# vgl-hub/kreeq

Measured on AMD Instinct MI355X. Metric: distinct+total k-mers/sec at k=21 (count path), higher is better.
Workload: dtype u64

## Files before the change

### include/kreeq_amd.h

```cpp
#ifndef KREEQ_AMD_H
#define KREEQ_AMD_H

#include <stdint.h>

#ifdef __cplusplus
extern "C" {
#endif

#define KQ_ABI_VERSION 4

typedef enum {
    KQ_OK = 0,
    KQ_ERR_INVALID = -1,
    KQ_ERR_NO_DEVICE = -2,
    KQ_ERR_HIP = -3,
    KQ_ERR_NOMEM = -4,
    KQ_ERR_TABLE_FULL = -5,
    KQ_ERR_CAPACITY = -6,
    KQ_ERR_MISMATCH = -7
} kq_status;

typedef struct kq_handle kq_handle;

typedef struct {
    uint64_t key;
    uint32_t fw[4], bw[4], cov;
    uint32_t hc;
} kq_entry;

typedef struct {
    uint32_t fw, bw, cov;
    uint8_t  isFw;
    uint8_t  pad[3];
} kq_dbgbase;

typedef struct {
    uint64_t total;
    uint64_t unique;
    uint64_t distinct;
    uint64_t missing;
    uint64_t edges;
} kq_stats;

typedef struct {
    uint64_t kmers_counted;
    uint64_t slots_used;
    uint64_t slots_total;
    uint64_t hc_used;
    uint64_t hc_total;
    uint64_t table_bytes;
    uint64_t table_passes;
} kq_info;


int  kq_create(kq_handle** out, int device, int k, int map_count, uint64_t capacity_hint);
void kq_destroy(kq_handle* h);
int  kq_clear(kq_handle* h);
int  kq_set_stream(kq_handle* h, void* hip_stream);
void* kq_get_stream(kq_handle* h);
enum { KQ_OPT_TRUST_CAPACITY = 1, KQ_OPT_COUNT_PATH = 2, KQ_OPT_SLICE_KMERS = 3, KQ_OPT_COUNT_MAP_RANGE = 4, KQ_OPT_PROFILE = 5,
       KQ_OPT_LOOKUP_PATH = 6, KQ_OPT_MERGE_PATH = 7, KQ_OPT_NARROW_MID = 8, KQ_OPT_PENDING_BYTES = 9, KQ_OPT_BUCKET_WINDOW = 10, KQ_OPT_OVERLAP = 11, KQ_OPT_COUNT_MAP_PASSES = 12, KQ_OPT_KERNEL_SET = 13,
       KQ_OPT_TEST_FAIL_PLAN = 100  };
int  kq_set_option(kq_handle* h, int option, int64_t value);
int  kq_get_profile(kq_handle* h, char* buf, uint64_t cap);
int  kq_sync(kq_handle* h);
int  kq_flush(kq_handle* h);
int  kq_get_info(kq_handle* h, kq_info* out);
const char* kq_last_error(void);
int  kq_abi_version(void);
int  kq_device_available(void);
int  kq_device_memory(int device, uint64_t* free_bytes, uint64_t* total_bytes);


int  kq_count_batch(kq_handle* h, const char* bases, uint64_t len);
int  kq_count_batch_dev(kq_handle* h, const char* d_bases, uint64_t len);

void* kq_host_alloc(uint64_t bytes);
void  kq_host_free(void* p);
int  kq_count_batch_async(kq_handle* h, const char* bases, uint64_t len, uint64_t* ticket);
int  kq_host_wait(kq_handle* h, uint64_t ticket);

void kq_pack_bases(const char* bases, uint64_t len, uint32_t* codes, uint16_t* inv);
int  kq_count_packed_dev(kq_handle* h, const uint32_t* d_codes, const uint16_t* d_inv, uint64_t n_bases);
int  kq_count_packed_async(kq_handle* h, const uint32_t* codes, const uint16_t* inv, uint64_t n_bases, uint64_t* ticket);

int  kq_pack_bases_dev(kq_handle* h, const char* d_bases, uint64_t len, uint32_t* d_codes, uint16_t* d_inv);

enum { KQ_FASTX_FASTQ = 1, KQ_FASTX_FASTA = 2 };
int  kq_parse_fastx_dev(kq_handle* h, const char* d_text, uint64_t len, int format, char* d_bases, uint64_t cap, uint64_t* n_bases);
int  kq_count_fastx_dev(kq_handle* h, const char* d_text, uint64_t len, int format);
int  kq_count_fastx_async(kq_handle* h, const char* text, uint64_t len, int format, uint64_t* ticket);

int  kq_emit_records(kq_handle* h, const char* bases, uint64_t len,
                     uint64_t* keys, uint8_t* edges, uint64_t cap, uint64_t* n_out);
int  kq_emit_partitioned_dev(kq_handle* h, const char* d_bases, uint64_t len, int n_parts,
                             uint64_t* d_keys, uint8_t* d_edges, uint64_t cap,
                             uint64_t* part_counts);

int  kq_emit_packed_dev(kq_handle* h, const char* d_bases, uint64_t len, int n_parts,
                        uint64_t* d_recs, uint64_t cap, uint64_t* part_counts);
int  kq_insert_packed_dev(kq_handle* h, const uint64_t* d_recs, uint64_t n);

int  kq_emit_sharded_dev(kq_handle* h, const char* d_bases, uint64_t len, int n_parts, uint32_t* d_recs, uint8_t* d_aux, uint64_t cap,
                         uint64_t* d_bucket_counts, uint64_t* part_counts);
int  kq_insert_sharded_dev(kq_handle* h, const uint32_t* d_recs, const uint8_t* d_aux, uint64_t n, int n_peers, const uint64_t* d_bucket_counts);

int  kq_insert_records(kq_handle* h, const uint64_t* keys, const uint8_t* edges, uint64_t n);
int  kq_insert_records_dev(kq_handle* h, const uint64_t* d_keys, const uint8_t* d_edges, uint64_t n);


int  kq_summary(kq_handle* h, kq_stats* out);
int  kq_histogram(kq_handle* h, uint64_t* cov, uint64_t* cnt, uint64_t cap, uint64_t* n_out);


int  kq_lookup_sequence(kq_handle* h, const char* bases, uint64_t len, uint32_t cov_cutoff,
                        uint16_t map_lo, uint16_t map_hi, kq_dbgbase* per_base,
                        uint64_t counters[3]);
int  kq_lookup_sequence_dev(kq_handle* h, const char* d_bases, uint64_t len, uint32_t cov_cutoff,
                            uint16_t map_lo, uint16_t map_hi, kq_dbgbase* d_per_base,
                            uint64_t* d_counters);


int  kq_lookup_keys(kq_handle* h, const uint64_t* keys, uint64_t n, kq_entry* out);

int  kq_branch_scan(kq_handle* h, const char* bases, uint64_t len, uint32_t cov_cutoff, uint8_t* flags);


int  kq_merge(kq_handle* dst, kq_handle* src);

int  kq_import(kq_handle* h, const kq_entry* entries, uint64_t n);
int  kq_export(kq_handle* h, uint16_t map_lo, uint16_t map_hi, kq_entry* out, uint64_t cap,
               uint64_t* n_out);

#ifdef __cplusplus
}
#endif
#endif
```

### kreeq_amd/build.py

```python
import os
import shutil
import subprocess

PKG = os.path.dirname(os.path.abspath(__file__))
ROOT = os.path.dirname(PKG)
LIB = os.path.join(PKG, "lib", "libkreeq_amd.so")
CLI = os.path.join(PKG, "bin", "kreeq")
HOSTLIB = os.path.join(PKG, "lib", "libkreeq_host.so")

HIP_SOURCES = [os.path.join(PKG, "csrc", "kreeq_amd.hip")]
HIP_DEPS = HIP_SOURCES + [os.path.join(PKG, "csrc", f) for f in ("kq_device.h", "kq_partition.h", "kq_kernels.h", "kq_fastx.h")] + [os.path.join(ROOT, "include", "kreeq_amd.h")]
HOST_DIR = os.path.join(PKG, "host")


def _stale(target, deps):
    if not os.path.exists(target):
        return True
    t = os.path.getmtime(target)
    return any(os.path.getmtime(d) > t for d in deps if os.path.exists(d))


def hipcc():
    for c in (shutil.which("hipcc"), "/opt/rocm/bin/hipcc"):
        if c and os.path.exists(c):
            return c
    raise RuntimeError("hipcc not found: the HIP library cannot be built (there is no CPU fallback)")


def build_lib(force=False, verbose=False, out=None, defines=()):
    target = out or LIB
    if force or _stale(target, HIP_DEPS):
        os.makedirs(os.path.dirname(target), exist_ok=True)
        cmd = [hipcc(), "-O3", "-std=c++17", "--offload-arch=gfx950", "-fPIC", "-shared", "-Wall", "-Wextra",
               "-o", target] + ["-D" + d for d in defines] + HIP_SOURCES
        if verbose:
            print(" ".join(cmd))
        subprocess.check_call(cmd)
    return target


def host_sources():
    if not os.path.isdir(HOST_DIR):
        return []
    return sorted(os.path.join(HOST_DIR, f) for f in os.listdir(HOST_DIR) if f.endswith(".cpp") and f != "hostlib.cpp")


def build_hostlib(force=False, verbose=False):
    srcs = [os.path.join(HOST_DIR, f) for f in ("hostlib.cpp", "kreeq_db.cpp")]
    deps = srcs + [os.path.join(HOST_DIR, "kreeq_db.h"), os.path.join(ROOT, "include", "kreeq_amd.h")]
    if force or _stale(HOSTLIB, deps):
        os.makedirs(os.path.dirname(HOSTLIB), exist_ok=True)
        cmd = ["g++", "-O2", "-std=c++17", "-Wall", "-Wextra", "-fPIC", "-shared", "-pthread", "-I", os.path.join(ROOT, "include"), "-o", HOSTLIB] + srcs
        if verbose:
            print(" ".join(cmd))
        subprocess.check_call(cmd)
    return HOSTLIB


def build_cli(force=False, verbose=False):
    srcs = host_sources()
    if not srcs:
        return None
    deps = srcs + [os.path.join(HOST_DIR, f) for f in os.listdir(HOST_DIR) if f.endswith(".h")] + [LIB]
    if force or _stale(CLI, deps):
        os.makedirs(os.path.dirname(CLI), exist_ok=True)
        cmd = ["g++", "-O2", "-std=c++17", "-Wall", "-Wextra", "-pthread", "-I", os.path.join(ROOT, "include"), "-o", CLI] + srcs + \
              ["-L", os.path.dirname(LIB), "-lkreeq_amd", "-lz", "-Wl,-rpath,$ORIGIN/../lib"]
        if verbose:
            print(" ".join(cmd))
        subprocess.check_call(cmd)
    return CLI


def build_all(force=False, verbose=False):
    build_lib(force, verbose)
    build_cli(force, verbose)
    build_hostlib(force, verbose)
```

### kreeq_amd/capi.py

```python
import ctypes as C
import os

import numpy as np

from . import build as _build

ENTRY_DTYPE = np.dtype([("key", "<u8"), ("fw", "<u4", 4), ("bw", "<u4", 4), ("cov", "<u4"), ("hc", "<u4")])
DBGBASE_DTYPE = np.dtype([("fw", "<u4"), ("bw", "<u4"), ("cov", "<u4"), ("isFw", "u1"), ("pad", "u1", 3)])

SYMBOLS = ["kq_create", "kq_destroy", "kq_clear", "kq_set_option", "kq_get_profile", "kq_set_stream", "kq_get_stream", "kq_sync", "kq_flush", "kq_get_info", "kq_last_error",
           "kq_abi_version", "kq_device_available", "kq_device_memory", "kq_count_batch", "kq_count_batch_dev", "kq_host_alloc", "kq_host_free", "kq_count_batch_async", "kq_host_wait", "kq_pack_bases", "kq_count_packed_dev", "kq_count_packed_async",
           "kq_pack_bases_dev", "kq_parse_fastx_dev", "kq_count_fastx_dev", "kq_count_fastx_async", "kq_emit_records",
           "kq_emit_partitioned_dev", "kq_emit_packed_dev", "kq_insert_packed_dev", "kq_emit_sharded_dev", "kq_insert_sharded_dev", "kq_insert_records", "kq_insert_records_dev", "kq_summary", "kq_histogram",
           "kq_lookup_sequence", "kq_lookup_sequence_dev", "kq_lookup_keys", "kq_branch_scan", "kq_merge", "kq_import", "kq_export"]

FASTX_FASTQ, FASTX_FASTA = 1, 2


class KqError(RuntimeError):
    def __init__(self, code, msg):
        super().__init__(f"kreeq_amd error {code}: {msg}")
        self.code = code


class Stats(C.Structure):
    _fields_ = [("total", C.c_uint64), ("unique", C.c_uint64), ("distinct", C.c_uint64), ("missing", C.c_uint64),
                ("edges", C.c_uint64)]


class Info(C.Structure):
    _fields_ = [("kmers_counted", C.c_uint64), ("slots_used", C.c_uint64), ("slots_total", C.c_uint64), ("hc_used", C.c_uint64),
                ("hc_total", C.c_uint64), ("table_bytes", C.c_uint64), ("table_passes", C.c_uint64)]


_lib = None


def lib_path():
    return _build.LIB


def _preload_process_hip_runtime():
    import importlib.util

    try:
        spec = importlib.util.find_spec("torch")
    except (ImportError, ValueError):
        spec = None
    if not spec or not spec.origin:
        return
    d = os.path.join(os.path.dirname(spec.origin), "lib")
    for name in ("libhsa-runtime64.so", "libamdhip64.so"):
        p = os.path.join(d, name)
        if os.path.exists(p):
            try:
                C.CDLL(p, mode=C.RTLD_GLOBAL)
            except OSError:
                return


def load():
    global _lib
    if _lib is not None:
        return _lib
    path = os.environ.get("KQ_LIB") or _build.LIB
    if not os.path.exists(path):
        raise KqError(-2, f"{path} is missing: build it with `python -c 'import __graft_entry__ as g; g.build()'` "
                          "(the product has no CPU fallback)")
    _preload_process_hip_runtime()
    L = C.CDLL(path)
    vp, u64, u32, u16, ci = C.c_void_p, C.c_uint64, C.c_uint32, C.c_uint16, C.c_int
    L.kq_create.argtypes = [C.POINTER(vp), ci, ci, ci, u64]
    L.kq_destroy.argtypes = [vp]
    L.kq_destroy.restype = None
    L.kq_clear.argtypes = [vp]
    L.kq_set_stream.argtypes = [vp, vp]
    L.kq_set_option.argtypes = [vp, ci, C.c_int64]
    L.kq_get_profile.argtypes = [vp, C.c_char_p, u64]
    L.kq_get_stream.argtypes = [vp]
    L.kq_get_stream.restype = vp
    L.kq_sync.argtypes = [vp]
    L.kq_flush.argtypes = [vp]
    L.kq_get_info.argtypes = [vp, C.POINTER(Info)]
    L.kq_last_error.restype = C.c_char_p
    L.kq_device_memory.argtypes = [ci, C.POINTER(u64), C.POINTER(u64)]
    L.kq_count_batch.argtypes = [vp, vp, u64]
    L.kq_count_batch_dev.argtypes = [vp, vp, u64]
    L.kq_host_alloc.argtypes = [u64]
    L.kq_host_alloc.restype = vp
    L.kq_host_free.argtypes = [vp]
    L.kq_host_free.restype = None
    L.kq_count_batch_async.argtypes = [vp, vp, u64, C.POINTER(u64)]
    L.kq_host_wait.argtypes = [vp, u64]
    L.kq_pack_bases.argtypes = [vp, u64, vp, vp]
    L.kq_pack_bases.restype = None
    L.kq_count_packed_dev.argtypes = [vp, vp, vp, u64]
    L.kq_count_packed_async.argtypes = [vp, vp, vp, u64, C.POINTER(u64)]
    L.kq_pack_bases_dev.argtypes = [vp, vp, u64, vp, vp]
    L.kq_parse_fastx_dev.argtypes = [vp, vp, u64, ci, vp, u64, C.POINTER(u64)]
    L.kq_count_fastx_dev.argtypes = [vp, vp, u64, ci]
    L.kq_count_fastx_async.argtypes = [vp, vp, u64, ci, C.POINTER(u64)]
    L.kq_emit_records.argtypes = [vp, vp, u64, vp, vp, u64, C.POINTER(u64)]
    L.kq_emit_partitioned_dev.argtypes = [vp, vp, u64, ci, vp, vp, u64, vp]
    L.kq_emit_packed_dev.argtypes = [vp, vp, u64, ci, vp, u64, vp]
    L.kq_insert_packed_dev.argtypes = [vp, vp, u64]
    L.kq_emit_sharded_dev.argtypes = [vp, vp, u64, ci, vp, vp, u64, vp, vp]
    L.kq_insert_sharded_dev.argtypes = [vp, vp, vp, u64, ci, vp]
    L.kq_insert_records.argtypes = [vp, vp, vp, u64]
    L.kq_insert_records_dev.argtypes = [vp, vp, vp, u64]
    L.kq_summary.argtypes = [vp, C.POINTER(Stats)]
    L.kq_histogram.argtypes = [vp, vp, vp, u64, C.POINTER(u64)]
    L.kq_lookup_sequence.argtypes = [vp, vp, u64, u32, u16, u16, vp, vp]
    L.kq_lookup_sequence_dev.argtypes = [vp, vp, u64, u32, u16, u16, vp, vp]
    L.kq_lookup_keys.argtypes = [vp, vp, u64, vp]
    L.kq_branch_scan.argtypes = [vp, vp, u64, u32, vp]
    L.kq_merge.argtypes = [vp, vp]
    L.kq_import.argtypes = [vp, vp, u64]
    L.kq_export.argtypes = [vp, u16, u16, vp, u64, C.POINTER(u64)]
    _lib = L
    return L


def _check(rc):
    if rc != 0:
        raise KqError(rc, load().kq_last_error().decode(errors="replace"))


def _p(a):
    return a.ctypes.data_as(C.c_void_p) if a is not None else None


def pack_bases(bases: bytes):
    buf = np.frombuffer(bases, dtype=np.uint8)
    units = (len(buf) + 15) // 16
    codes, inv = np.zeros(max(units, 1), dtype=np.uint32), np.zeros(max(units, 1), dtype=np.uint16)
    load().kq_pack_bases(_p(buf) if len(buf) else None, len(buf), _p(codes), _p(inv))
    return codes[:units], inv[:units]


def device_available():
    return bool(load().kq_device_available())


def device_memory(device=0):
    f, t = C.c_uint64(0), C.c_uint64(0)
    _check(load().kq_device_memory(device, C.byref(f), C.byref(t)))
    return f.value, t.value


class KreeqDB:

    def __init__(self, k=21, map_count=128, device=0, capacity_hint=0):
        self.k, self.map_count, self.device = k, map_count, device
        self._h = C.c_void_p()
        _check(load().kq_create(C.byref(self._h), device, k, map_count, capacity_hint))

    def close(self, _load=load):
        if getattr(self, "_h", None):
            _load().kq_destroy(self._h)
            self._h = None

    __del__ = close

    @property
    def handle(self):
        return self._h

    def set_stream(self, hip_stream_ptr):
        _check(load().kq_set_stream(self._h, C.c_void_p(hip_stream_ptr)))

    def sync(self):
        _check(load().kq_sync(self._h))

    def flush(self):
        _check(load().kq_flush(self._h))

    def set_option(self, option, value):
        opt = {"trust_capacity": 1, "count_path": 2, "slice_kmers": 3, "count_map_range": 4, "profile": 5, "lookup_path": 6, "merge_path": 7, "narrow_mid": 8, "pending_bytes": 9, "bucket_window": 10, "overlap": 11, "count_map_passes": 12, "kernel_set": 13, "test_fail_plan": 100}[option]
        if option == "count_map_range":
            value = int(value[0]) | (int(value[1]) << 16)
        if option in ("count_path", "lookup_path", "merge_path"):
            value = {"auto": 0, "direct": 1, "partitioned": 2}[value]
        _check(load().kq_set_option(self._h, opt, int(value)))

    def clear(self):
        _check(load().kq_clear(self._h))

    def profile(self):
        buf = C.create_string_buffer(1024)
        _check(load().kq_get_profile(self._h, buf, 1024))
        return {k: float(v) for k, v in (kv.split("=") for kv in buf.value.decode().split(";") if kv)}

    def info(self):
        i = Info()
        _check(load().kq_get_info(self._h, C.byref(i)))
        return {f: getattr(i, f) for f, _ in Info._fields_}

    def count_batch(self, bases: bytes):
        buf = np.frombuffer(bases, dtype=np.uint8)
        _check(load().kq_count_batch(self._h, _p(buf), len(buf)))

    def count_batch_async(self, host_ptr, n):
        t = C.c_uint64(0)
        _check(load().kq_count_batch_async(self._h, C.c_void_p(host_ptr), n, C.byref(t)))
        return t.value

    def count_packed_dev(self, codes_ptr, inv_ptr, n_bases):
        _check(load().kq_count_packed_dev(self._h, C.c_void_p(codes_ptr), C.c_void_p(inv_ptr), n_bases))

    def count_packed_async(self, codes_ptr, inv_ptr, n_bases):
        t = C.c_uint64(0)
        _check(load().kq_count_packed_async(self._h, C.c_void_p(codes_ptr), C.c_void_p(inv_ptr), n_bases, C.byref(t)))
        return t.value

    def pack_bases_dev(self, bases_ptr, n, codes_ptr, inv_ptr):
        _check(load().kq_pack_bases_dev(self._h, C.c_void_p(bases_ptr), n, C.c_void_p(codes_ptr), C.c_void_p(inv_ptr)))

    def parse_fastx_dev(self, text_ptr, n, fmt, out_ptr, cap):
        nb = C.c_uint64(0)
        rc = load().kq_parse_fastx_dev(self._h, C.c_void_p(text_ptr), n, fmt, C.c_void_p(out_ptr) if out_ptr else None, cap, C.byref(nb))
        if rc != 0:
            e = KqError(rc, load().kq_last_error().decode(errors="replace"))
            e.needed = nb.value
            raise e
        return nb.value

    def count_fastx_dev(self, text_ptr, n, fmt):
        _check(load().kq_count_fastx_dev(self._h, C.c_void_p(text_ptr), n, fmt))

    def count_fastx_async(self, host_ptr, n, fmt):
        t = C.c_uint64(0)
        _check(load().kq_count_fastx_async(self._h, C.c_void_p(host_ptr), n, fmt, C.byref(t)))
        return t.value

    def host_wait(self, ticket):
        _check(load().kq_host_wait(self._h, ticket))

    def count_batch_dev(self, ptr, n):
        _check(load().kq_count_batch_dev(self._h, C.c_void_p(ptr), n))

    def emit_records(self, bases: bytes):
        buf = np.frombuffer(bases, dtype=np.uint8)
        n = C.c_uint64(0)
        _check(load().kq_emit_records(self._h, _p(buf), len(buf), None, None, 0, C.byref(n)))
        keys = np.empty(n.value, dtype=np.uint64)
        edges = np.empty(n.value, dtype=np.uint8)
        if n.value:
            _check(load().kq_emit_records(self._h, _p(buf), len(buf), _p(keys), _p(edges), n.value, C.byref(n)))
        return keys, edges

    def emit_partitioned_dev(self, bases_ptr, n, n_parts, keys_ptr, edges_ptr, cap):
        counts = np.zeros(n_parts, dtype=np.uint64)
        _check(load().kq_emit_partitioned_dev(self._h, C.c_void_p(bases_ptr), n, n_parts, C.c_void_p(keys_ptr), C.c_void_p(edges_ptr),
                                              cap, _p(counts)))
        return counts

    def emit_packed_dev(self, bases_ptr, n, n_parts, recs_ptr, cap):
        counts = np.zeros(n_parts, dtype=np.uint64)
        _check(load().kq_emit_packed_dev(self._h, C.c_void_p(bases_ptr), n, n_parts, C.c_void_p(recs_ptr), cap, _p(counts)))
        return counts

    def insert_packed_dev(self, recs_ptr, n):
        _check(load().kq_insert_packed_dev(self._h, C.c_void_p(recs_ptr), n))

    def emit_sharded_dev(self, bases_ptr, n, n_parts, recs_ptr, aux_ptr, cap, bucket_counts_ptr, sync=True):
        counts = np.zeros(n_parts, dtype=np.uint64) if sync else None
        _check(load().kq_emit_sharded_dev(self._h, C.c_void_p(bases_ptr), n, n_parts, C.c_void_p(recs_ptr), C.c_void_p(aux_ptr), cap,
                                          C.c_void_p(bucket_counts_ptr), _p(counts)))
        return counts

    def insert_sharded_dev(self, recs_ptr, aux_ptr, n, n_peers, bucket_counts_ptr):
        _check(load().kq_insert_sharded_dev(self._h, C.c_void_p(recs_ptr), C.c_void_p(aux_ptr), n, n_peers, C.c_void_p(bucket_counts_ptr)))

    def insert_records(self, keys, edges):
        keys = np.ascontiguousarray(keys, dtype=np.uint64)
        edges = np.ascontiguousarray(edges, dtype=np.uint8)
        assert len(keys) == len(edges)
        _check(load().kq_insert_records(self._h, _p(keys), _p(edges), len(keys)))

    def insert_records_dev(self, keys_ptr, edges_ptr, n):
        _check(load().kq_insert_records_dev(self._h, C.c_void_p(keys_ptr), C.c_void_p(edges_ptr), n))

    def summary(self, with_hist=False):
        st = Stats()
        _check(load().kq_summary(self._h, C.byref(st)))
        d = {f: getattr(st, f) for f, _ in Stats._fields_}
        if with_hist:
            n = C.c_uint64(0)
            _check(load().kq_histogram(self._h, None, None, 0, C.byref(n)))
            cov = np.zeros(n.value, dtype=np.uint64)
            cnt = np.zeros(n.value, dtype=np.uint64)
            _check(load().kq_histogram(self._h, _p(cov), _p(cnt), n.value, C.byref(n)))
            d["hist"] = dict(zip(cov.tolist(), cnt.tolist()))
        return d

    def lookup_sequence(self, bases: bytes, cov_cutoff=0, map_lo=0, map_hi=None, per_base=False, per_base_buf=None):
        if map_hi is None:
            map_hi = self.map_count
        buf = np.frombuffer(bases, dtype=np.uint8)
        ctr = np.zeros(3, dtype=np.uint64)
        pb = per_base_buf if per_base_buf is not None else (np.zeros(len(buf), dtype=DBGBASE_DTYPE) if per_base else None)
        _check(load().kq_lookup_sequence(self._h, _p(buf), len(buf), cov_cutoff, map_lo, map_hi, _p(pb), _p(ctr)))
        return ctr, pb

    def lookup_sequence_dev(self, bases_ptr, n, counters_ptr, cov_cutoff=0, map_lo=0, map_hi=None, per_base_ptr=None):
        if map_hi is None:
            map_hi = self.map_count
        _check(load().kq_lookup_sequence_dev(self._h, C.c_void_p(bases_ptr), n, cov_cutoff, map_lo, map_hi,
                                             C.c_void_p(per_base_ptr) if per_base_ptr else None, C.c_void_p(counters_ptr)))

    def lookup_keys(self, keys):
        keys = np.ascontiguousarray(keys, dtype=np.uint64)
        out = np.zeros(len(keys), dtype=ENTRY_DTYPE)
        _check(load().kq_lookup_keys(self._h, _p(keys), len(keys), _p(out)))
        return out

    def branch_scan(self, bases: bytes, cov_cutoff=0):
        buf = np.frombuffer(bases, dtype=np.uint8)
        flags = np.zeros(len(buf), dtype=np.uint8)
        _check(load().kq_branch_scan(self._h, _p(buf), len(buf), cov_cutoff, _p(flags)))
        return flags

    def merge(self, other):
        _check(load().kq_merge(self._h, other._h))

    def import_entries(self, entries):
        entries = np.ascontiguousarray(entries, dtype=ENTRY_DTYPE)
        _check(load().kq_import(self._h, _p(entries), len(entries)))

    def export(self, map_lo=0, map_hi=None):
        if map_hi is None:
# ... 8 lines not shown
```

### kreeq_amd/csrc/kq_kernels.h

```cpp
#pragma once

#include <hip/hip_runtime.h>

#include <type_traits>

#include "../../include/kreeq_amd.h"
#include "kq_device.h"
#include "kq_partition.h"

using namespace kq;


__global__ __launch_bounds__(TILE_THREADS) void k_count_direct(TableView t, const uint8_t* __restrict__ ab,
                                                                uint64_t lead, uint64_t len, int k, EmitRange er, PartCfg filt,
                                                                const uint16_t* __restrict__ pinv ) {
    uint32_t n_new = 0;
    uint64_t n_kmers = 0;
    scan_tiles(ab, lead, len, k, [&](uint64_t pos, uint64_t fw, uint64_t rv, uint32_t prev, uint32_t next) {
        if (pos < er.lo || pos >= er.hi) return;
        const bool is_fw = fw < rv;
        const uint64_t key = is_fw ? fw : rv;
        if (filt.filt_lo != 0 || filt.filt_hi != filt.map_count) {
            const uint32_t m = map_index(key, filt.map_count, filt.map_mask);
            if (m < filt.filt_lo || m >= filt.filt_hi) return;
// ... 240 lines not shown
        for (int it = 0; it < 16; ++it) { const uint32_t b = TOP8 ? wb[TOP8 ? it : 0] : narrow_word_bin(w[it]); pl[it] = b != NB ? atomicAdd(&s_hist[b], 1u) : ~0u; }
#pragma unroll
        for (int it = 0; it < 16; ++it) if (pl[it] != ~0u) { s_buf[pl[it]] = w[it]; if (TOP8) s_bin[pl[it]] = (uint16_t)wb[TOP8 ? it : 0]; }
        __syncthreads();
        const uint32_t total = s_loff[NB];
        uint64_t cv[16];
        uint32_t cg[16];
#pragma unroll
        for (int it = 0; it < 16; ++it) cv[it] = s_buf[tid + it * THREADS];
#pragma unroll
        for (int it = 0; it < 16; ++it) cg[it] = s_grel[(uint32_t)(tid + it * THREADS) < total ? (TOP8 ? (uint32_t)s_bin[TOP8 ? tid + it * THREADS : 0] : narrow_word_bin(cv[it])) : 0u] + (tid + it * THREADS);
        if (bin_owner) s_hist[tid] = 0;
        landed(nxt.x); landed(nxt.y); landed(nxt.z); landed(nxt.w);
#pragma unroll
        for (int it = 0; it < 16; ++it) {
            if ((uint32_t)(tid + it * THREADS) < total) {
                if (TOP8) reinterpret_cast<uint64_t*>(recs)[cg[it]] = cv[it];
                else { recs[cg[it]] = (uint32_t)cv[it]; recs_aux[cg[it]] = (uint8_t)(cv[it] >> 48); }
            }
        }
    }
}

__global__ __launch_bounds__(1024) void k_lv_units(const unsigned long long* __restrict__ seg_off, const unsigned long long* __restrict__ seg_hi, LevelCfg lv,
                                                   unsigned long long* __restrict__ unit_base) {
    __shared__ unsigned long long s_part[1024];
    const uint32_t tid = threadIdx.x, per = (lv.n_seg + 1023) / 1024;
    const uint32_t lo = min(tid * per, lv.n_seg), hi = min(lo + per, lv.n_seg);
    unsigned long long sum = 0;
    for (uint32_t b = lo; b < hi; ++b) sum += (seg_hi[b] - seg_off[b] + P2_UNIT - 1) / P2_UNIT;
    s_part[tid] = sum;
    __syncthreads();
    if (tid < 64) {
        unsigned long long loc[16], tot = 0;
#pragma unroll
        for (int j = 0; j < 16; ++j) { loc[j] = s_part[tid * 16 + j]; tot += loc[j]; }
        unsigned long long incl = tot;
#pragma unroll
        for (int o = 1; o < 64; o <<= 1) { unsigned long long nn = __shfl_up(incl, o, 64); if ((int)tid >= o) incl += nn; }
        unsigned long long run = incl - tot;
#pragma unroll
        for (int j = 0; j < 16; ++j) { s_part[tid * 16 + j] = run; run += loc[j]; }
        if (tid == 63) unit_base[lv.n_seg] = incl;
    }
    __syncthreads();
    unsigned long long run = s_part[tid];
    for (uint32_t b = lo; b < hi; ++b) { unit_base[b] = run; run += (seg_hi[b] - seg_off[b] + P2_UNIT - 1) / P2_UNIT; }
}
__device__ __forceinline__ uint32_t seg_of_unit(const unsigned long long* unit_base, uint32_t n_seg, uint64_t u) {
    uint32_t lo = 0, hi = n_seg;
    while (hi - lo > 1) { uint32_t mid = (lo + hi) >> 1; if (unit_base[mid] <= u) lo = mid; else hi = mid; }
    return lo;
}
template <int FMT>
__global__ __launch_bounds__(MS_THREADS) void k_lv_hist(const uint64_t* __restrict__ recs, const uint8_t* __restrict__ , LevelCfg lv,
                                                        const unsigned long long* __restrict__ seg_off, const unsigned long long* __restrict__ seg_hi,
                                                        const unsigned long long* __restrict__ unit_base, uint32_t* __restrict__ m2) {
    __shared__ uint32_t s_hist[NB_MAX];
    const uint64_t n_units = unit_base[lv.n_seg];
    for (uint64_t u = blockIdx.x; u < n_units; u += gridDim.x) {
        const uint32_t b_in = seg_of_unit(unit_base, lv.n_seg, u);
        const uint32_t b = lv.spb > 1 ? b_in / lv.spb : b_in;
        const uint64_t lo = seg_off[b_in] + (u - unit_base[b_in]) * P2_UNIT;
        const uint64_t hi = lo + P2_UNIT < seg_hi[b_in] ? lo + P2_UNIT : seg_hi[b_in];
        for (uint32_t i = threadIdx.x; i < lv.nb; i += MS_THREADS) s_hist[i] = 0;
        __syncthreads();
        const uint64_t last = hi - 1;
        if (FMT == FMT_NARROW) {
            const uint4* v4 = reinterpret_cast<const uint4*>(recs);
            const uint64_t q0 = lo >> 2, q1 = (hi + 3) >> 2;
            for (uint64_t qb = q0; qb < q1; qb += 4ull * MS_THREADS) {
                uint4 q[4];
#pragma unroll
                for (int j = 0; j < 4; ++j) q[j] = v4[min(qb + (uint64_t)j * MS_THREADS + threadIdx.x, q1 - 1)];
#pragma unroll
                for (int j = 0; j < 4; ++j) {
                    const uint64_t qi = qb + (uint64_t)j * MS_THREADS + threadIdx.x;
                    const uint32_t e[4] = {q[j].x, q[j].y, q[j].z, q[j].w};
#pragma unroll
                    for (int c = 0; c < 4; ++c) {
                        const uint64_t ri = 4 * qi + c;
                        if (qi < q1 && ri >= lo && ri < hi) atomicAdd(&s_hist[narrow_bin(lv, b, e[c])], 1u);
                    }
                }
            }
        } else
        for (uint64_t base = lo; base < hi; base += 8ull * MS_THREADS) {
            uint64_t r[8];
#pragma unroll
            for (int j = 0; j < 8; ++j) {
                const uint64_t i = min(base + (uint64_t)j * MS_THREADS + threadIdx.x, last);
                r[j] = FMT == FMT_NARROW ? (uint64_t)reinterpret_cast<const uint32_t*>(recs)[i] : recs[i];
            }
#pragma unroll
            for (int j = 0; j < 8; ++j)
                if (base + (uint64_t)j * MS_THREADS + threadIdx.x < hi) {
                    const uint32_t bin = FMT == FMT_NARROW ? narrow_bin(lv, b, (uint32_t)r[j])
                        : FMT == FMT_TOP8 ? narrow_bin(lv, b, (uint32_t)(r[j] >> 32))
                        : (FMT == FMT_PACK8 && lv.top8) ? (uint32_t)(rec_hash<false>(r[j]) >> (64 - NARROW_CBITS))
                        : level_bin(lv, b, hash_region(lv.in_raw ? table_hash(r[j], lv.k) : rec_hash<FMT == FMT_WIDE>(r[j]), lv.n_regions));
                    atomicAdd(&s_hist[bin], 1u);
                }
        }
        __syncthreads();
        for (uint32_t i = threadIdx.x; i < lv.nb; i += MS_THREADS) m2[u * lv.nb + i] = s_hist[i];
        __syncthreads();
    }
}
__global__ __launch_bounds__(256) void k_lv_offsets(uint32_t* __restrict__ m2, LevelCfg lv, const unsigned long long* __restrict__ unit_base,
                                                    unsigned long long* __restrict__ group_count) {
    const uint64_t r = ((uint64_t)blockIdx.x * blockDim.x + threadIdx.x) >> 6;
    const uint32_t lane = threadIdx.x & 63;
    const uint32_t n_lseg = lv.n_seg / lv.spb;
    if (r >= (uint64_t)n_lseg * lv.nb) return;
    const uint32_t b = (uint32_t)(r / lv.nb), bin = (uint32_t)(r % lv.nb);
    const uint64_t u0 = unit_base[b * lv.spb], u1 = unit_base[(b + 1) * lv.spb];
    unsigned long long run = 0;
    for (uint64_t base = u0; base < u1; base += 64) {
        const uint64_t u = base + lane;
        const uint32_t c = u < u1 ? m2[u * lv.nb + bin] : 0u;
        unsigned long long incl = c;
#pragma unroll
        for (int o = 1; o < 64; o <<= 1) { const unsigned long long n = __shfl_up(incl, o, 64); if ((int)lane >= o) incl += n; }
        if (u < u1) m2[u * lv.nb + bin] = (uint32_t)(run + incl - c);
        run += __shfl(incl, 63, 64);
    }
    if (lane == 0) group_count[r] = run;
}
__global__ __launch_bounds__(256) void k_lv_offsets_thread(uint32_t* __restrict__ m2, LevelCfg lv, const unsigned long long* __restrict__ unit_base,
                                                           unsigned long long* __restrict__ group_count) {
    const uint64_t r = (uint64_t)blockIdx.x * blockDim.x + threadIdx.x;
    const uint32_t n_lseg = lv.n_seg / lv.spb;
    if (r >= (uint64_t)n_lseg * lv.nb) return;
    const uint32_t b = (uint32_t)(r / lv.nb), bin = (uint32_t)(r % lv.nb);
    const uint64_t u0 = unit_base[b * lv.spb], u1 = unit_base[(b + 1) * lv.spb];
    unsigned long long run = 0;
    for (uint64_t u = u0; u < u1; ++u) {
        const uint32_t c = m2[u * lv.nb + bin];
        m2[u * lv.nb + bin] = (uint32_t)run;
        run += c;
    }
    group_count[r] = run;
}
#ifndef KQ_LV_THREADS
#define KQ_LV_THREADS 512
#define KQ_LV_ITEMS 8
#define KQ_LV_OCC 4
#endif
constexpr int LV_THREADS = KQ_LV_THREADS, LV_ITEMS = KQ_LV_ITEMS, LV_TILE = LV_THREADS * LV_ITEMS;
template <int FMT, int NBC>
__global__ __launch_bounds__(LV_THREADS, KQ_LV_OCC) void k_lv_scatter(const uint64_t* __restrict__ recs, const uint8_t* __restrict__ recs_aux, LevelCfg lv,
                                                           const unsigned long long* __restrict__ seg_off, const unsigned long long* __restrict__ seg_hi,
                                                           const unsigned long long* __restrict__ unit_base, const uint32_t* __restrict__ m2,
                                                           const unsigned long long* __restrict__ group_base, uint64_t* __restrict__ out,
                                                           uint8_t* __restrict__ out_aux) {
    constexpr bool WIDE = FMT == FMT_WIDE, TIGHT = FMT == FMT_NARROW_TO_TIGHT, NARROW = FMT == FMT_NARROW || TIGHT, CONVERT = FMT == FMT_PACK8_TO_NARROW,
                   TOP8 = FMT == FMT_TOP8, HAS_AUX = WIDE || NARROW;
    constexpr int MS_FMT = (CONVERT || TIGHT) ? FMT_NARROW : TOP8 ? FMT_PACK8 : FMT;
    const uint32_t* recs32 = reinterpret_cast<const uint32_t*>(recs);
    __shared__ MsShared<NBC, MS_FMT, LV_TILE> s;
    __shared__ uint32_t s_rst[TIGHT ? NBC : 1];
    const uint32_t nb = lv.nb;
    const uint64_t n_units = unit_base[lv.n_seg];
    for (uint64_t u = blockIdx.x; u < n_units; u += gridDim.x) {
        const uint32_t b_in = seg_of_unit(unit_base, lv.n_seg, u);
        const uint32_t b = lv.spb > 1 ? b_in / lv.spb : b_in;
        const uint64_t lo = seg_off[b_in] + (u - unit_base[b_in]) * P2_UNIT;
        const uint64_t hi = lo + P2_UNIT < seg_hi[b_in] ? lo + P2_UNIT : seg_hi[b_in];
        for (uint32_t i = threadIdx.x; i < nb; i += LV_THREADS)
            s.gbase[i] = (uint32_t)(group_base[(uint64_t)b * nb + i] + m2[u * nb + i]);
        if (TIGHT) {
            const uint32_t first = (b >> lv.nr_shift) * lv.nr_rps + (b & ((1u << lv.nr_shift) - 1u)) * lv.nr_sub;
            for (uint32_t i = threadIdx.x; i < nb; i += LV_THREADS) s_rst[i] = lv.rstart[first + i];
        }
        __syncthreads();
        uint64_t nxt[LV_ITEMS];
        uint32_t nxt_aux[LV_ITEMS];
        const uint64_t last = hi - 1;
#pragma unroll
        for (int j = 0; j < LV_ITEMS; ++j) {
            const uint64_t i = min(lo + (uint64_t)j * LV_THREADS + threadIdx.x, last);
            nxt[j] = NARROW ? (uint64_t)recs32[i] : recs[i];
            nxt_aux[j] = HAS_AUX ? recs_aux[i] : 0;
        }
#pragma unroll
        for (int j = 0; j < LV_ITEMS; ++j) { landed(nxt[j]); if (HAS_AUX) landed(nxt_aux[j]); }
        for (uint64_t pos = lo; pos < hi; pos += LV_TILE) {
            uint64_t rec[LV_ITEMS];
            uint32_t aux[LV_ITEMS], bin[LV_ITEMS];
#pragma unroll
            for (int j = 0; j < LV_ITEMS; ++j) {
                const uint64_t i = pos + (uint64_t)j * LV_THREADS + threadIdx.x;
                rec[j] = (WIDE && lv.in_raw) ? table_hash(nxt[j], lv.k) : nxt[j];
                aux[j] = nxt_aux[j];
                if (TIGHT) {
                    const uint32_t bn = i >= hi ? nb : narrow_bin(lv, b, (uint32_t)rec[j]);
                    rec[j] = narrow_word(tight_rec(b >> lv.nr_shift, (uint32_t)rec[j], aux[j], s_rst[bn < nb ? bn : 0u]), 0u, bn);
                }
                else if (NARROW) rec[j] = narrow_word((uint32_t)rec[j], aux[j], i >= hi ? nb : narrow_bin(lv, b, (uint32_t)rec[j]));
                else if (CONVERT) {
                    const uint64_t hh = rec_hash<false>(rec[j]);
                    rec[j] = narrow_word(narrow_main(hh), narrow_aux(hh, (uint32_t)(rec[j] >> REC_EDGE_SHIFT) & 63u), i >= hi ? nb : (uint32_t)(hh >> (64 - NARROW_CBITS)));
                }
                else if (TOP8) bin[j] = i >= hi ? nb : narrow_bin(lv, b, (uint32_t)(rec[j] >> 32));
                else bin[j] = i >= hi ? nb : level_bin(lv, b, hash_region(rec_hash<WIDE>(rec[j]), lv.n_regions));
            }
#pragma unroll
            for (int j = 0; j < LV_ITEMS; ++j) {
                const uint64_t i = min(pos + LV_TILE + (uint64_t)j * LV_THREADS + threadIdx.x, last);
                nxt[j] = NARROW ? (uint64_t)recs32[i] : recs[i];
                nxt_aux[j] = HAS_AUX ? recs_aux[i] : 0;
            }
            block_multisplit<MS_FMT, LV_THREADS, LV_ITEMS>(s, rec, aux, bin, nb, out, out_aux, [&] {
#pragma unroll
                for (int j = 0; j < LV_ITEMS; ++j) { landed(nxt[j]); if (HAS_AUX) landed(nxt_aux[j]); }
            }, NBC <= 512 ? lv.rep_shift : 0u);
        }
    }
}
#ifndef KQ_LVS_OCC
#define KQ_LVS_OCC 4
#define KQ_LVS_OCC_TIGHT 4
#endif
template <bool TIGHT>
__global__ __launch_bounds__(LV_THREADS, TIGHT ? KQ_LVS_OCC_TIGHT : KQ_LVS_OCC) void k_lv_scatter_s(const uint32_t* __restrict__ recs32, const uint8_t* __restrict__ recs_aux, LevelCfg lv,
                                                           const unsigned long long* __restrict__ seg_off, const unsigned long long* __restrict__ seg_hi,
                                                           const unsigned long long* __restrict__ unit_base, const uint32_t* __restrict__ m2,
                                                           const unsigned long long* __restrict__ group_base, uint32_t* __restrict__ out,
                                                           uint8_t* __restrict__ out_aux) {
    constexpr int NC = 512;
    static_assert(LV_THREADS == NC && LV_ITEMS == 8, "one counter per thread");
    __shared__ uint64_t s_buf[LV_TILE];
    __shared__ uint32_t s_hist[2][NC], s_loff[NC + 1], s_grel[NC], s_wave[LV_THREADS / 64];
    __shared__ uint32_t s_rst[TIGHT ? NC : 1];
    const int tid = threadIdx.x;
    const uint32_t nb = lv.nb, rs = lv.rep_shift, n_ctr = (nb + 1) << rs;
    const uint32_t sub = (uint32_t)tid & ((1u << rs) - 1u), my_bin = (uint32_t)tid >> rs;
    const bool own_bin = sub == 0 && my_bin < nb;
    const uint64_t n_units = unit_base[lv.n_seg];
    for (uint64_t u = blockIdx.x; u < n_units; u += gridDim.x) {
        const uint32_t b_in = seg_of_unit(unit_base, lv.n_seg, u);
        const uint32_t b = lv.spb > 1 ? b_in / lv.spb : b_in;
        const uint64_t lo = seg_off[b_in] + (u - unit_base[b_in]) * P2_UNIT;
        const uint64_t hi = lo + P2_UNIT < seg_hi[b_in] ? lo + P2_UNIT : seg_hi[b_in];
        uint32_t gabs = own_bin ? (uint32_t)(group_base[(uint64_t)b * nb + my_bin] + m2[u * nb + my_bin]) : 0u;
        if (TIGHT) {
            const uint32_t first = (b >> lv.nr_shift) * lv.nr_rps + (b & ((1u << lv.nr_shift) - 1u)) * lv.nr_sub;
            if ((uint32_t)tid < nb) s_rst[tid] = lv.rstart[first + tid];
        }
        s_hist[0][tid] = 0;
        __syncthreads();
        uint32_t nxt[LV_ITEMS], nxt_aux[LV_ITEMS];
        const uint64_t last = hi - 1;
#pragma unroll
        for (int j = 0; j < LV_ITEMS; ++j) {
            const uint64_t i = min(lo + (uint64_t)j * LV_THREADS + tid, last);
            nxt[j] = recs32[i];
            nxt_aux[j] = recs_aux[i];
        }
#pragma unroll
        for (int j = 0; j < LV_ITEMS; ++j) { landed(nxt[j]); landed(nxt_aux[j]); }
        uint32_t par = 0;
        for (uint64_t pos = lo; pos < hi; pos += LV_TILE, par ^= 1u) {
            uint32_t* hist = s_hist[par];
            uint64_t w[LV_ITEMS];
#pragma unroll
            for (int j = 0; j < LV_ITEMS; ++j) {
                const uint64_t i = pos + (uint64_t)j * LV_THREADS + tid;
                const uint32_t bn = i >= hi ? nb : narrow_bin(lv, b, nxt[j]);
                w[j] = TIGHT ? narrow_word(tight_rec(b >> lv.nr_shift, nxt[j], nxt_aux[j], s_rst[bn < nb ? bn : 0u]), 0u, bn) : narrow_word(nxt[j], nxt_aux[j], bn);
                if (bn != nb) atomicAdd(&hist[(bn << rs) | sub], 1u);
            }
#pragma unroll
            for (int j = 0; j < LV_ITEMS; ++j) {
                const uint64_t i = min(pos + LV_TILE + (uint64_t)j * LV_THREADS + tid, last);
                nxt[j] = recs32[i];
                nxt_aux[j] = recs_aux[i];
            }
            __syncthreads();
            const uint32_t cnt = (uint32_t)tid < n_ctr ? hist[tid] : 0u;
            uint32_t incl = cnt;
#pragma unroll
            for (int o = 1; o < 64; o <<= 1) { const uint32_t n = __shfl_up(incl, o, 64); if ((tid & 63) >= o) incl += n; }
            if ((tid & 63) == 63) s_wave[tid >> 6] = incl;
            s_hist[par ^ 1u][tid] = 0;
            __syncthreads();
            uint32_t excl = incl - cnt;
            for (int v = 0; v < (tid >> 6); ++v) excl += s_wave[v];
            s_loff[tid] = excl;
            hist[tid] = excl;
            if (own_bin) s_grel[my_bin] = gabs - excl;
            __syncthreads();
            if (own_bin) gabs += s_loff[(my_bin + 1) << rs] - excl;
#pragma unroll
            for (int j = 0; j < LV_ITEMS; ++j) {
                const uint32_t bn = narrow_word_bin(w[j]);
                if (bn != nb) s_buf[atomicAdd(&hist[(bn << rs) | sub], 1u)] = w[j];
            }
            __syncthreads();
            const uint32_t total = s_loff[nb << rs];
            uint64_t cv[LV_ITEMS];
            uint32_t cg[LV_ITEMS];
#pragma unroll
            for (int it = 0; it < LV_ITEMS; ++it) cv[it] = s_buf[tid + it * LV_THREADS];
#pragma unroll
            for (int it = 0; it < LV_ITEMS; ++it) cg[it] = s_grel[(uint32_t)(tid + it * LV_THREADS) < total ? narrow_word_bin(cv[it]) : 0u] + (tid + it * LV_THREADS);
#pragma unroll
            for (int j = 0; j < LV_ITEMS; ++j) { landed(nxt[j]); landed(nxt_aux[j]); }
#pragma unroll
            for (int it = 0; it < LV_ITEMS; ++it) {
                if ((uint32_t)(tid + it * LV_THREADS) < total) {
                    out[cg[it]] = (uint32_t)cv[it];
                    if (!TIGHT) out_aux[cg[it]] = (uint8_t)(cv[it] >> 48);
                }
            }
        }
    }
}
__global__ void k_set2(unsigned long long* p, unsigned long long a, unsigned long long b) { p[0] = a; p[1] = b; }

constexpr uint32_t SCAN_CHUNK = 16384;
__global__ __launch_bounds__(1024) void k_scan_sums(const unsigned long long* __restrict__ a, uint64_t n, unsigned long long* __restrict__ sums) {
    const uint64_t lo = (uint64_t)blockIdx.x * SCAN_CHUNK, hi = lo + SCAN_CHUNK < n ? lo + SCAN_CHUNK : n;
    unsigned long long v = 0;
    for (uint64_t i = lo + threadIdx.x; i < hi; i += 1024) v += a[i];
    uint64_t t = block_sum(v);
    if (threadIdx.x == 0) sums[blockIdx.x] = t;
}
__global__ __launch_bounds__(1024) void k_scan_apply(unsigned long long* __restrict__ a, uint64_t n, const unsigned long long* __restrict__ sums) {
    __shared__ unsigned long long s_part[1024];
    const uint64_t lo = (uint64_t)blockIdx.x * SCAN_CHUNK + (uint64_t)threadIdx.x * (SCAN_CHUNK / 1024);
    unsigned long long v[SCAN_CHUNK / 1024], sum = 0;
#pragma unroll
    for (uint32_t j = 0; j < SCAN_CHUNK / 1024; ++j) { v[j] = lo + j < n ? a[lo + j] : 0; sum += v[j]; }
    s_part[threadIdx.x] = sum;
    __syncthreads();
    if (threadIdx.x < 64) {
        unsigned long long loc[16], tot = 0;
#pragma unroll
        for (int j = 0; j < 16; ++j) { loc[j] = s_part[threadIdx.x * 16 + j]; tot += loc[j]; }
        unsigned long long incl = tot;
#pragma unroll
        for (int o = 1; o < 64; o <<= 1) { unsigned long long nn = __shfl_up(incl, o, 64); if ((int)threadIdx.x >= o) incl += nn; }
        unsigned long long run = incl - tot;
#pragma unroll
        for (int j = 0; j < 16; ++j) { s_part[threadIdx.x * 16 + j] = run; run += loc[j]; }
    }
    __syncthreads();
    unsigned long long run = sums[blockIdx.x] + s_part[threadIdx.x];
#pragma unroll
    for (uint32_t j = 0; j < SCAN_CHUNK / 1024; ++j) { if (lo + j < n) a[lo + j] = run; run += v[j]; }
}


template <class T> __device__ __forceinline__ T ld_global(const T* p) { return *(const __attribute__((address_space(1))) T*)p; }

template <uint32_t GRP>
struct SetTickets {
    uint64_t lo; uint32_t cnt, first, n_grp;
    __device__ __forceinline__ void build(const P3Set* __restrict__ sets, uint32_t n_sets, uint64_t r, uint32_t lane) {
        lo = 0; cnt = 0;
        if (lane < n_sets) { const unsigned long long* b = ld_global(&sets[lane].base); lo = ld_global(b + r); cnt = (uint32_t)(ld_global(b + r + 1) - lo); }
        const uint32_t mine = (cnt + GRP - 1) / GRP;
        uint32_t incl = mine;
#pragma unroll
        for (int o = 1; o < P3_MAX_SETS; o <<= 1) { const uint32_t v = __shfl_up(incl, o, 64); if ((int)lane >= o) incl += v; }
        first = incl - mine;
        n_grp = __builtin_amdgcn_readlane(incl, 63);
    }
    __device__ __forceinline__ void locate(uint32_t g, uint32_t& q, uint32_t& off, uint32_t& q_cnt, uint64_t& q_lo) const {
        const uint64_t nonempty = __ballot(cnt != 0);
        const uint64_t m = __ballot(cnt != 0 && first <= g);
        q = (g < n_grp && m) ? 63u - (uint32_t)__clzll((unsigned long long)m) : (uint32_t)__ffsll((unsigned long long)nonempty) - 1u;
        const uint32_t f = __builtin_amdgcn_readlane(first, q);
        q_cnt = __builtin_amdgcn_readlane(cnt, q);
        q_lo = ((uint64_t)__builtin_amdgcn_readlane((uint32_t)(lo >> 32), q) << 32) | __builtin_amdgcn_readlane((uint32_t)lo, q);
        off = (g < n_grp ? g - f : 0u) * GRP;
    }
};

template <int THREADS, bool HOT, uint32_t GRP>
__device__ __forceinline__ bool region_gate(SetTickets<GRP>& tk, const TableView& t, const P3Set* __restrict__ sets, uint32_t n_sets, uint64_t r,
                                            int table_is_empty, unsigned long long* __restrict__ hot_list ) {
    const int tid = threadIdx.x;
    tk.build(sets, n_sets, r, (uint32_t)tid & 63u);
    uint64_t n_recs = tk.cnt;
#pragma unroll
    for (int o = 32; o > 0; o >>= 1) n_recs += __shfl_xor(n_recs, o, 64);
    if (n_recs == 0) {
        if (!HOT && table_is_empty == 2) {
            ulonglong2* g2 = reinterpret_cast<ulonglong2*>(t.slots + (r << REGION_SHIFT));
            for (int i = tid; i < (int)REGION_SLOTS; i += THREADS) g2[i] = make_ulonglong2(0ull, 0ull);
        }
        return false;
    }
    if (!HOT && n_recs > 32ull * REGION_SLOTS) {
        if (tid == 0) hot_list[1 + atomicAdd(&hot_list[0], 1ull)] = r;
        return false;
    }
    return true;
}
constexpr int HC_LDS = 64;
__device__ __forceinline__ void hc_lds_reset(uint64_t (&hckey)[HC_LDS], uint32_t (&hccnt)[HC_LDS][8]) {
    const int tid = threadIdx.x;
    if (tid < HC_LDS) {
        hckey[tid] = EMPTY_KEY;
#pragma unroll
        for (int e = 0; e < 8; ++e) hccnt[tid][e] = 0;
    }
}
__device__ __forceinline__ void hc_lds_add(const TableView& t, uint64_t (&hckey)[HC_LDS], uint32_t (&hccnt)[HC_LDS][8], uint64_t h, const uint32_t (&e)[8]) {
    const uint64_t key = key_of_hash(h, t.k);
    int hslot = -1;
    uint32_t hp = (uint32_t)(h >> 40) & (HC_LDS - 1);
    for (int probe = 0; probe < HC_LDS; ++probe, hp = (hp + 1) & (HC_LDS - 1)) {
        uint64_t cur = __hip_atomic_load(&hckey[hp], __ATOMIC_RELAXED, __HIP_MEMORY_SCOPE_WORKGROUP);
        if (cur == EMPTY_KEY) cur = atomicCAS((unsigned long long*)&hckey[hp], (unsigned long long)EMPTY_KEY, (unsigned long long)key);
        if (cur == EMPTY_KEY || cur == key) { hslot = (int)hp; break; }
    }
    if (hslot >= 0) {
#pragma unroll
        for (int w = 0; w < 8; ++w) if (e[w]) atomicAdd(&hccnt[hslot][w], e[w]);
    } else {
        hc_add(t, h, 0, 0, e);
    }
}
__device__ __forceinline__ void hc_lds_flush(const TableView& t, uint64_t (&hckey)[HC_LDS], uint32_t (&hccnt)[HC_LDS][8]) {
    const int tid = threadIdx.x;
    if (tid < HC_LDS && hckey[tid] != EMPTY_KEY) {
        HcSlot* hs = hc_upsert(t, hckey[tid]);
        if (!hs) atomicOr(&t.st->err_hc_full, 1u);
        else {
#pragma unroll
            for (int e = 0; e < 8; ++e) if (hccnt[tid][e]) atomicAdd((unsigned long long*)&hs->cnt[e], (unsigned long long)hccnt[tid][e]);
        }
    }
}
template <class C>
__device__ __forceinline__ void region_totals_wave(uint32_t n_new, uint32_t n_ok, C& s_new, C& s_kmers) {
#pragma unroll
    for (int o = 32; o > 0; o >>= 1) { n_new += __shfl_down(n_new, o, 64); n_ok += __shfl_down(n_ok, o, 64); }
    if ((threadIdx.x & 63) == 0) { if (n_new) atomicAdd(&s_new, (C)n_new); if (n_ok) atomicAdd(&s_kmers, (C)n_ok); }
}
template <class C>
__device__ __forceinline__ void region_totals_store(const TableView& t, const C& s_new, const C& s_kmers) {
    if (threadIdx.x == 0) {
        if (s_new) atomicAdd(&t.st->slots_used, (unsigned long long)s_new);
        if (s_kmers) atomicAdd(&t.st->kmers_added, (unsigned long long)s_kmers);
    }
}

#ifndef KQ_P3_THREADS
#define KQ_P3_THREADS 512
#define KQ_P3_OCC 6
#define KQ_P3_PF 2
#endif
constexpr int P3_THREADS = KQ_P3_THREADS;
template <int FMT, bool HOT>
__global__ __launch_bounds__(P3_THREADS, HOT ? 4 : KQ_P3_OCC) void k_count_regions(TableView t, const P3Set* __restrict__ sets, uint32_t n_sets,
                                                              int aux_fmt, int table_is_empty,
                                                              unsigned long long* __restrict__ hot_list ,
                                                              uint32_t narrow_rps ) {
    constexpr bool WIDE = FMT == FMT_WIDE, NARROW = FMT == FMT_NARROW, TOP8 = FMT == FMT_TOP8, HAS_AUX = WIDE || NARROW;
    constexpr int PF = KQ_P3_PF;
    constexpr uint64_t GRP = 64ull * PF;
    __shared__ uint64_t s_img[REGION_SLOTS * 3];
    __shared__ uint64_t s_lut[64];
    if (threadIdx.x < 64) s_lut[threadIdx.x] = idx6_to_pack(threadIdx.x);
    __shared__ unsigned long long s_new, s_kmers;
    __shared__ unsigned int s_grp;
    __shared__ uint64_t s_hckey[HC_LDS];
    __shared__ uint32_t s_hccnt[HC_LDS][8];
// ... 837 lines not shown
```

### kreeq_amd/csrc/kq_partition.h

```cpp
#pragma once
#include "kq_device.h"

namespace kq {

constexpr int MS_THREADS = 256;
constexpr int MS_ITEMS = 16;
constexpr int MS_TILE = MS_THREADS * MS_ITEMS;
constexpr int NB_MAX = 2048;
constexpr int SEG_MAX = 65536;
constexpr uint32_t SUB_BITS_MAX = 8;
constexpr int REC_EDGE_SHIFT = 56;
constexpr int PART_MAX_K = 28;
constexpr int AUX_IDX6 = 0, AUX_EDGE_BYTE = 1, AUX_TIGHT = 2;

struct PartCfg {
    uint64_t n_regions;
    uint32_t g_shift;
    uint32_t n_coarse;
    uint32_t mode;
    uint32_t map_count;
    uint32_t map_mask;
    uint32_t filt_lo, filt_hi;
    uint32_t raw_out;
    uint32_t narrow;
    uint32_t owner_sub;
    uint32_t sub_bits;
    uint32_t win_lo, win_hi;
    uint32_t n_rng;
};

constexpr int P3_MAX_SETS = 64;
struct P3Set { const uint64_t* recs; const uint8_t* aux; const unsigned long long* base; uint64_t n_max; };

struct LevelCfg {
    uint64_t n_regions;
    uint32_t n_seg, nb, seg_shift, out_shift;
    uint32_t in_raw;
    uint32_t k;
    uint32_t narrow;
    uint32_t top8;
    uint32_t nr_shift, nr_rps, nr_sub, nr_div, nr_inv;
    uint32_t nr_mid, nr_fshift, nr_fmask, nr_f24;
    uint32_t spb;
    uint32_t rep_shift;
    const uint32_t* rstart = nullptr;
};
__device__ __forceinline__ uint32_t level_bin(const LevelCfg& lv, uint32_t b, uint64_t region) {
    return (uint32_t)(region >> lv.out_shift) - (lv.seg_shift >= 32 ? 0u : (b << (lv.seg_shift - lv.out_shift)));
}

__device__ __forceinline__ uint32_t edge_idx6(bool is_fw, uint32_t prev, uint32_t next) {
    uint32_t f, b;
    if (is_fw) { f = next < 4 ? next : 7u; b = prev < 4 ? prev : 7u; }
    else       { f = prev < 4 ? 3u - prev : 7u; b = next < 4 ? 3u - next : 7u; }
    return f | (b << 3);
}
__device__ __forceinline__ uint32_t edge_idx6_any(bool is_fw, uint32_t prev, uint32_t next) {
    const uint32_t f = is_fw ? next : prev, b = is_fw ? prev : next, m = is_fw ? 0u : 0x1Bu;
    return (f | (b << 3)) ^ m;
}
__device__ __forceinline__ uint64_t rec_pack(uint64_t key, bool is_fw, uint32_t prev, uint32_t next) {
    return key | ((uint64_t)edge_idx6(is_fw, prev, next) << REC_EDGE_SHIFT);
}
__device__ __forceinline__ uint64_t idx6_to_pack(uint32_t v) {
    const uint32_t f = v & 7u, b = (v >> 3) & 7u;
    return (f < 4 ? 1ull << (8 * f) : 0ull) | (b < 4 ? 1ull << (8 * (4 + b)) : 0ull);
}
__device__ __forceinline__ uint32_t idx6_to_edge_byte(uint32_t v) {
    const uint32_t f = v & 7u, b = (v >> 3) & 7u;
    return (f < 4 ? 1u << (7 - f) : 0u) | (b < 4 ? 1u << (7 - (4 + b)) : 0u);
}
__device__ __forceinline__ uint64_t rec_key(uint64_t rec) { return rec & ((1ull << REC_EDGE_SHIFT) - 1); }
__device__ __forceinline__ uint64_t rec_edge_pack(uint64_t rec) {
    const uint32_t f = (uint32_t)(rec >> REC_EDGE_SHIFT) & 7u, b = (uint32_t)(rec >> (REC_EDGE_SHIFT + 3)) & 7u;
    return (f < 4 ? 1ull << (8 * f) : 0ull) | (b < 4 ? 1ull << (8 * (4 + b)) : 0ull);
}
template <bool WIDE>
__device__ __forceinline__ uint64_t rec_hash(uint64_t rec) { return WIDE ? rec : rec << 8; }
__device__ __forceinline__ uint64_t rec_pack_hash(uint64_t h, bool is_fw, uint32_t prev, uint32_t next) {
    return (h >> 8) | ((uint64_t)edge_idx6(is_fw, prev, next) << REC_EDGE_SHIFT);
}

constexpr int FMT_PACK8 = 0, FMT_WIDE = 1, FMT_NARROW = 2;
constexpr int FMT_PACK8_TO_NARROW = 3;
constexpr uint32_t NARROW_CBITS = 8, NARROW_MAX_K = 21;
constexpr int FMT_TOP8 = 4;
constexpr int FMT_TIGHT = 5;
constexpr int FMT_NARROW_TO_TIGHT = 6;
constexpr uint64_t TIGHT_MIN_REGIONS = 1ull << 16;
__device__ __forceinline__ uint32_t tight_rec(uint32_t bucket, uint32_t main32, uint32_t aux, uint32_t rstart_r) {
    const uint32_t d = ((bucket << (32 - NARROW_CBITS)) | (main32 >> NARROW_CBITS)) - rstart_r;
    return (d << 16) | ((main32 & 0xFFu) << 8) | ((aux & 3u) << 6) | (aux >> 2);
}
__device__ __forceinline__ uint64_t tight_hash(uint32_t t, uint32_t rstart_r) { return ((uint64_t)((t >> 16) + rstart_r) << 32) | ((uint64_t)((t >> 6) & 1023u) << 22); }
__device__ __forceinline__ uint64_t top8_rec(uint64_t h, uint32_t idx6) { return ((h << NARROW_CBITS) & ~63ull) | idx6; }
__device__ __forceinline__ uint64_t top8_hash(uint32_t bucket, uint64_t rec) { return ((uint64_t)bucket << (64 - NARROW_CBITS)) | ((rec & ~63ull) >> NARROW_CBITS); }
__device__ __forceinline__ uint32_t narrow_main(uint64_t h) { return (uint32_t)(h >> (32 - NARROW_CBITS)); }
__device__ __forceinline__ uint32_t narrow_aux(uint64_t h, uint32_t idx6) { return ((uint32_t)(h >> (30 - NARROW_CBITS)) & 3u) | (idx6 << 2); }
__device__ __forceinline__ uint64_t narrow_hash(uint32_t bucket, uint32_t main32, uint32_t aux) {
    return ((uint64_t)bucket << (64 - NARROW_CBITS)) | ((uint64_t)main32 << (32 - NARROW_CBITS)) | ((uint64_t)(aux & 3u) << (30 - NARROW_CBITS));
}
__device__ __forceinline__ uint64_t narrow_word(uint32_t main32, uint32_t aux, uint32_t bin) { return (uint64_t)main32 | ((uint64_t)(bin | (aux << 16)) << 32); }
__device__ __forceinline__ uint32_t narrow_word_bin(uint64_t w) { return (uint32_t)(w >> 32) & 0xFFFFu; }
__device__ __forceinline__ uint32_t narrow_region(uint32_t bucket, uint32_t main32, uint64_t n_regions) {
    return __umulhi((bucket << (32 - NARROW_CBITS)) | (main32 >> NARROW_CBITS), (uint32_t)n_regions);
}
__device__ __forceinline__ uint32_t narrow_bin(const LevelCfg& lv, uint32_t , uint32_t main32) {
    const uint32_t f = main32 >> NARROW_CBITS;
    if (lv.nr_mid) return f >> lv.nr_fshift;
    const uint32_t fs = f & lv.nr_fmask;
    return lv.nr_f24 ? umul24u(fs, lv.nr_sub) >> lv.nr_fshift : (uint32_t)(((uint64_t)fs * lv.nr_sub) >> lv.nr_fshift);
}

template <int NBC, int FMT, int TILE = MS_TILE>
struct MsShared {
    static constexpr int tile = TILE;
    uint64_t stage[TILE];
    uint16_t sbin[FMT != FMT_NARROW ? TILE : 4];
    uint8_t  saux[FMT == FMT_WIDE ? TILE : 8];
    uint32_t hist[NBC];
    uint32_t loff[NBC];
    uint32_t gbase[NBC];
    uint32_t wave_sum[16];
};

template <int THREADS, class S>
__device__ __forceinline__ void ms_scan(S& s, uint32_t nb) {
    constexpr int NBC = (int)(sizeof(s.hist) / sizeof(uint32_t));
    constexpr int MS_BINS_PER_THREAD = (NBC + THREADS - 1) / THREADS;
    const int tid = threadIdx.x;
    uint32_t v[MS_BINS_PER_THREAD], sum = 0;
#pragma unroll
    for (int j = 0; j < MS_BINS_PER_THREAD; ++j) { uint32_t b = MS_BINS_PER_THREAD * tid + j; v[j] = (b < nb) ? s.hist[b] : 0; sum += v[j]; }
    uint32_t incl = sum;
#pragma unroll
    for (int o = 1; o < 64; o <<= 1) { uint32_t n = __shfl_up(incl, o, 64); if ((tid & 63) >= o) incl += n; }
    if ((tid & 63) == 63) s.wave_sum[tid >> 6] = incl;
    __syncthreads();
    uint32_t base = 0;
    for (int w = 0; w < (tid >> 6); ++w) base += s.wave_sum[w];
    uint32_t run = base + incl - sum;
#pragma unroll
    for (int j = 0; j < MS_BINS_PER_THREAD; ++j) { uint32_t b = MS_BINS_PER_THREAD * tid + j; if (b < nb) s.loff[b] = run; run += v[j]; }
    __syncthreads();
}

__device__ __forceinline__ void landed(uint32_t& v) { asm volatile("" : "+v"(v)); }
__device__ __forceinline__ void landed(uint64_t& v) { asm volatile("" : "+v"(v)); }
struct NoHook { __device__ __forceinline__ void operator()() const {} };
template <int FMT, int THREADS = MS_THREADS, int ITEMS = MS_ITEMS, class S, class F = NoHook>
__device__ __forceinline__ void block_multisplit(S& s, const uint64_t (&rec)[ITEMS], const uint32_t (&aux)[ITEMS],
                                                 const uint32_t (&bin)[ITEMS], uint32_t nb,
                                                 uint64_t* __restrict__ out, uint8_t* __restrict__ out_aux, F pre_store = F(), uint32_t rs = 0) {
    const int tid = threadIdx.x;
    const uint32_t sub = (uint32_t)tid & ((1u << rs) - 1u), n_ctr = (nb + 1) << rs;
    for (uint32_t b = tid; b < n_ctr; b += THREADS) s.hist[b] = 0;
    __syncthreads();
    static_assert(THREADS * ITEMS <= S::tile, "round size");
    uint32_t rank[ITEMS];
#pragma unroll
    for (int i = 0; i < ITEMS; ++i) {
        const uint32_t b = FMT == FMT_NARROW ? narrow_word_bin(rec[i]) : bin[i];
        rank[i] = 0;
        if (b != nb) rank[i] = atomicAdd(&s.hist[(b << rs) | sub], 1u);
    }
    __syncthreads();
    ms_scan<THREADS>(s, n_ctr);
    for (uint32_t b = tid; b < nb; b += THREADS) s.gbase[b] -= s.loff[b << rs];
#pragma unroll
    for (int i = 0; i < ITEMS; ++i) {
        const uint32_t b = FMT == FMT_NARROW ? narrow_word_bin(rec[i]) : bin[i];
        if (b == nb) continue;
        const uint32_t p = s.loff[(b << rs) | sub] + rank[i];
        if (FMT == FMT_NARROW) {
            s.stage[p] = rec[i];
        } else {
            s.stage[p] = rec[i];
            s.sbin[p] = (uint16_t)bin[i];
            if (FMT == FMT_WIDE) s.saux[p] = (uint8_t)aux[i];
        }
    }
    __syncthreads();
    const uint32_t total = s.loff[nb << rs];
    uint32_t cb[ITEMS];
    uint32_t cg[ITEMS];
    uint64_t cv[ITEMS];
// ... 46 lines not shown
```

### kreeq_amd/csrc/kreeq_amd.hip

```cpp
#include <hip/hip_runtime.h>
#include <hipcub/hipcub.hpp>

#include <algorithm>
#include <cstdarg>
#include <cstdio>
#include <cstdlib>
#include <cstring>
#include <mutex>
#include <new>
#include <numeric>
#include <string>
#include <thread>
#include <type_traits>
#include <vector>

#include "../../include/kreeq_amd.h"
#include "kq_device.h"
#include "kq_partition.h"

using namespace kq;

#include "kq_kernels.h"
#include "kq_fastx.h"


static thread_local std::string g_err;
static int fail(int code, const char* fmt, ...) {
    char buf[512];
    va_list ap; va_start(ap, fmt); vsnprintf(buf, sizeof buf, fmt, ap); va_end(ap);
    g_err = buf;
    return code;
}
#define HIPC(expr)                                                                                   \
    do {                                                                                             \
        hipError_t e_ = (expr);                                                                      \
        if (e_ != hipSuccess)                                                                        \
            return fail(e_ == hipErrorOutOfMemory ? KQ_ERR_NOMEM : KQ_ERR_HIP, "%s: %s (%s:%d)", #expr, \
                        hipGetErrorString(e_), __FILE__, __LINE__);                                  \
    } while (0)

struct Scrambled {
    void* p = nullptr; size_t bytes = 0, chunk = 0;
    std::vector<hipMemGenericAllocationHandle_t> hs;
    bool vmm = false;
};
static void scr_free(Scrambled& b) {
    if (!b.p) return;
    (void)hipDeviceSynchronize();
    if (b.vmm) {
        (void)hipMemUnmap(b.p, b.hs.size() * b.chunk);
        for (auto& hnd : b.hs) (void)hipMemRelease(hnd);
        (void)hipMemAddressFree(b.p, b.hs.size() * b.chunk);
    } else (void)hipFree(b.p);
    b = Scrambled();
}
static bool scr_try_vmm(Scrambled& b, size_t bytes, int device) {
    static const size_t chunk_mb = getenv("KQ_SCRAMBLE_MB") ? (size_t)atoi(getenv("KQ_SCRAMBLE_MB")) : 2;
    if (!chunk_mb) return false;
    hipMemAllocationProp prop = {};
    prop.type = hipMemAllocationTypePinned; prop.location.type = hipMemLocationTypeDevice; prop.location.id = device;
    size_t gran = 0;
    if (hipMemGetAllocationGranularity(&gran, &prop, hipMemAllocationGranularityMinimum) != hipSuccess || !gran) { (void)hipGetLastError(); return false; }
    const size_t chunk = ((chunk_mb << 20) + gran - 1) / gran * gran, n = (bytes + chunk - 1) / chunk;
    void* base = nullptr;
    if (hipMemAddressReserve(&base, n * chunk, 0, nullptr, 0) != hipSuccess) { (void)hipGetLastError(); return false; }
    std::vector<hipMemGenericAllocationHandle_t> hs;
    hs.reserve(n);
    bool ok = true;
    for (size_t i = 0; i < n && ok; ++i) { hipMemGenericAllocationHandle_t hnd; ok = hipMemCreate(&hnd, chunk, &prop, 0) == hipSuccess; if (ok) hs.push_back(hnd); }
    size_t mapped = 0;
    if (ok) {
        size_t mul = 7919;
        while (std::gcd(mul, n) != 1) ++mul;
        for (; mapped < n && ok; ++mapped) ok = hipMemMap((char*)base + mapped * chunk, chunk, 0, hs[(mapped * mul + 13) % n], 0) == hipSuccess;
        if (!ok) --mapped;
    }
    if (ok) {
        hipMemAccessDesc acc = {};
        acc.location = prop.location; acc.flags = hipMemAccessFlagsProtReadWrite;
        ok = hipMemSetAccess(base, n * chunk, &acc, 1) == hipSuccess;
    }
    if (!ok) {
        (void)hipGetLastError();
        if (mapped) (void)hipMemUnmap(base, mapped * chunk);
        for (auto& hnd : hs) (void)hipMemRelease(hnd);
        (void)hipMemAddressFree(base, n * chunk);
        return false;
    }
    b.p = base; b.bytes = n * chunk; b.chunk = chunk; b.hs.swap(hs); b.vmm = true;
    return true;
}
static int scr_ensure(Scrambled& b, size_t need, int device) {
    if (b.bytes >= need) return KQ_OK;
    scr_free(b);
    const size_t sz = need + std::min<size_t>(need / 4, (size_t)256 << 20) + 4096;
    if (scr_try_vmm(b, sz, device)) return KQ_OK;
    if (hipMalloc(&b.p, sz) != hipSuccess) { (void)hipGetLastError(); b.p = nullptr; return fail(KQ_ERR_NOMEM, "partition scratch allocation failed"); }
    b.bytes = sz; b.vmm = false;
    return KQ_OK;
}

struct kq_handle;
static void arena_release(kq_handle* h);
struct kq_handle {
    int device = 0, k = 0, map_count = 0;
    hipStream_t own_stream = nullptr, stream = nullptr;
    int n_cu = 256;
    Slot* slots = nullptr;
    uint64_t n_regions = 0;
    uint32_t win_lo = 0, win_hi = 256;
    bool windowed = false;
    HcSlot* hc = nullptr;
    uint64_t hc_cap = 0;
    uint32_t* rstart = nullptr;
    DevState* st = nullptr;
    DevState* st_host = nullptr;
    void* scratch = nullptr; size_t scratch_bytes = 0;
    void* stage = nullptr; size_t stage_bytes = 0;
    uint64_t kmers_bound = 0;
    uint64_t used_bound = 0;
    uint64_t hc_check_at = 0;
    bool table_empty = true;
    uint32_t mid_rps = 2048;
    int merge_path = 0;
    int lookup_path = 0;
    bool slots_dirty = false;
    bool trust_capacity = false;
    int count_path = 0;
    uint64_t slice_kmers = 1ull << 28;
    bool slice_user = false;
    uint32_t filt_lo = 0, filt_hi = 0;
    bool profile = false;
    std::vector<std::pair<const char*, hipEvent_t>> marks;
    void* part = nullptr; size_t part_bytes = 0;
    Scrambled part2, fork_part2;
    hipStream_t base = nullptr;
    hipStream_t fork_stream[2] = {nullptr, nullptr};
    void* fork_part[2] = {nullptr, nullptr}; size_t fork_part_bytes[2] = {0, 0};
    bool fork_busy[2] = {false, false};
    bool fork_stale[2] = {false, false};
    static constexpr int EV_RING = 64;
    hipEvent_t ev_ring[EV_RING] = {};
    uint64_t ev_next = 0;
    hipEvent_t ev_pass = nullptr;
    int overlap = 1;
    int kernel_set = 0;
    struct HistKey { const void* ab; const void* pinv; uint64_t lead, len, er_lo, er_hi; uint32_t g1, n_rng; int k;
                     bool operator==(const HistKey& o) const { return ab == o.ab && pinv == o.pinv && lead == o.lead && len == o.len && er_lo == o.er_lo && er_hi == o.er_hi && g1 == o.g1 && n_rng == o.n_rng && k == o.k; } };
    struct HistEntry { HistKey key; unsigned long long* m1_all; size_t bytes; };
    std::vector<HistEntry> hist_cache;
    size_t hist_cache_bytes = 0;
    int map_passes = 1;
    void* arena = nullptr; size_t arena_bytes = 0, arena_used = 0;
    Scrambled arena_scr;
    P3Set* d_sets = nullptr;
    int n_pend = 0, pend_fmt = -1, pend_aux_fmt = 0;
    uint64_t pend_records = 0;
    int64_t pend_budget = -1;
    uint64_t table_passes = 0;
    static constexpr int IN_SLOTS = 3, IN_TICKETS = 512;
    hipStream_t copy_stream = nullptr;
    void* in_buf[IN_SLOTS] = {nullptr, nullptr, nullptr}; size_t in_bytes[IN_SLOTS] = {0, 0, 0};
    hipEvent_t in_consumed[IN_SLOTS] = {nullptr, nullptr, nullptr};
    std::vector<hipEvent_t> in_copied;
    uint64_t in_next = 0;
    std::mutex in_m;
    uint8_t in_bad[IN_TICKETS] = {};
    void* fx_units = nullptr; size_t fx_units_bytes = 0;
    void* fx_out = nullptr; size_t fx_out_bytes = 0;
    void* in_cmp[IN_SLOTS] = {nullptr, nullptr, nullptr}; size_t in_cmp_bytes[IN_SLOTS] = {0, 0, 0};
    FxResult* fx_res = nullptr;
    FxResult* fx_res_host = nullptr;
    int fx_bad = 0;
    bool hist_cache_off = false;
    bool test_fail_plan = false;
    void* hot = nullptr; size_t hot_bytes = 0;

    TableView view() const {
        TableView v; v.slots = slots - (reg_lo() << REGION_SHIFT); v.n_regions = n_regions; v.hc = hc; v.hc_mask = hc_cap - 1; v.st = st; v.k = (uint32_t)k;
        v.reg_lo = reg_lo(); v.reg_hi = reg_hi();
        v.rps = k >= HI_K ? (uint32_t)(n_regions >> 8) : 0u;
        v.rstart = rstart;
        return v;
    }
    uint64_t reg_lo() const { return windowed ? (uint64_t)win_lo * (n_regions >> 8) : 0; }
    uint64_t reg_hi() const { return windowed ? (uint64_t)win_hi * (n_regions >> 8) : n_regions; }
    uint64_t n_alloc_regions() const { return reg_hi() - reg_lo(); }
    uint64_t n_slots() const { return n_alloc_regions() << REGION_SHIFT; }
};

static void marks_reset(kq_handle* h);
static int flush_pending(kq_handle* h);

static int ev_get(kq_handle* h, hipEvent_t* out) {
    hipEvent_t& e = h->ev_ring[h->ev_next++ % kq_handle::EV_RING];
    if (!e) HIPC(hipEventCreateWithFlags(&e, hipEventDisableTiming));
    else HIPC(hipEventSynchronize(e));
    *out = e;
    return KQ_OK;
}
static int join_forks(kq_handle* h) {
    for (int w = 0; w < 2; ++w) {
        if (!h->fork_busy[w]) continue;
        hipEvent_t e; int rc = ev_get(h, &e); if (rc) return rc;
        HIPC(hipEventRecord(e, h->fork_stream[w]));
        HIPC(hipStreamWaitEvent(h->base, e, 0));
        h->fork_busy[w] = false;
    }
    return KQ_OK;
}

static int grid_for(const kq_handle* h, uint64_t work_items, int per_block, int per_cu = 8) {
    uint64_t blocks = (work_items + per_block - 1) / per_block;
    uint64_t cap = (uint64_t)h->n_cu * per_cu;
    if (blocks > cap) blocks = cap;
    if (blocks < 1) blocks = 1;
    return (int)blocks;
}

static void arena_release(kq_handle* h) {
    if (!h->arena) return;
    if (h->arena_scr.p) scr_free(h->arena_scr); else (void)hipFree(h->arena);
    h->arena = nullptr; h->arena_bytes = 0;
}
static int ensure_buf(void** p, size_t* have, size_t need) {
    if (*have >= need) return KQ_OK;
    if (*p) { HIPC(hipFree(*p)); *p = nullptr; *have = 0; }
    size_t sz = need + std::min<size_t>(need / 4, (size_t)256 << 20) + 4096;
    HIPC(hipMalloc(p, sz));
    *have = sz;
    return KQ_OK;
}

static void clear_words(kq_handle* h, void* p, uint32_t words_per_slot, uint64_t n_slots) {
    const uint64_t n_pairs = n_slots * words_per_slot / 2;
    hipLaunchKernelGGL(k_clear_slots, dim3(grid_for(h, n_pairs, 256)), dim3(256), 0, h->stream, (ulonglong2*)p, words_per_slot, n_pairs);
}
static void clear_main(kq_handle* h, Slot* p, uint64_t n_slots) { (void)hipMemsetAsync(p, 0, (size_t)n_slots * sizeof(Slot), h->stream); }
static void materialize(kq_handle* h) {
    if (!h->slots_dirty) return;
    clear_main(h, h->slots, h->n_slots());
    h->slots_dirty = false;
}
static int alloc_main(kq_handle* h, uint64_t n_regions, uint64_t alloc_regions, Slot** out, uint32_t** rstart_out) {
    Slot* p = nullptr;
    uint32_t* rs = nullptr;
    size_t bytes = (size_t)(alloc_regions << REGION_SHIFT) * sizeof(Slot);
    HIPC(hipMalloc((void**)&p, bytes));
    if (hipMalloc((void**)&rs, (size_t)(n_regions + 1) * sizeof(uint32_t)) != hipSuccess) { (void)hipFree(p); return fail(KQ_ERR_NOMEM, "region index allocation failed"); }
    clear_main(h, p, alloc_regions << REGION_SHIFT);
    hipLaunchKernelGGL(k_region_starts, dim3(grid_for(h, n_regions + 1, 256)), dim3(256), 0, h->stream, rs, n_regions);
    *out = p; *rstart_out = rs;
    return KQ_OK;
}
static int alloc_hc(kq_handle* h, uint64_t cap, HcSlot** out) {
    HcSlot* p = nullptr;
    size_t bytes = (size_t)cap * sizeof(HcSlot);
    HIPC(hipMalloc((void**)&p, bytes));
    clear_words(h, p, sizeof(HcSlot) / 8, cap);
    *out = p;
    return KQ_OK;
}

static int read_state_raw(kq_handle* h) {
    HIPC(hipMemcpyAsync(h->st_host, h->st, sizeof(DevState), hipMemcpyDeviceToHost, h->stream));
    HIPC(hipStreamSynchronize(h->stream));
    return KQ_OK;
}
static int read_state(kq_handle* h) {
    int frc = flush_pending(h);
    if (frc) return frc;
    return read_state_raw(h);
}
static int check_errors(kq_handle* h) {
    int rc = read_state(h);
    if (rc) return rc;
    if (h->st_host->err_table_full) return fail(KQ_ERR_TABLE_FULL, "k-mer table region overflow (slots %llu / %llu)",
                                                 (unsigned long long)h->st_host->slots_used, (unsigned long long)h->n_slots());
    if (h->st_host->err_hc_full) return fail(KQ_ERR_TABLE_FULL, "high-copy side table overflow (%llu / %llu)",
                                              (unsigned long long)h->st_host->hc_used, (unsigned long long)h->hc_cap);
    return KQ_OK;
}

static int grow_main(kq_handle* h, uint64_t need_slots) {
    int frc = flush_pending(h);
    if (frc) return frc;
    uint64_t want = h->n_slots(), new_regions = h->n_regions;
    while (want < need_slots) { want *= 2; new_regions *= 2; }
    if (new_regions >= (1ull << 32)) return fail(KQ_ERR_TABLE_FULL, "cannot grow k-mer table to %llu slots: region index overflow", (unsigned long long)want);
    Slot* fresh = nullptr;
    uint32_t* fresh_rs = nullptr;
    int rc = alloc_main(h, new_regions, want >> REGION_SHIFT, &fresh, &fresh_rs);
    if (rc) return rc == KQ_ERR_NOMEM ? fail(KQ_ERR_TABLE_FULL, "cannot grow k-mer table to %llu slots: out of device memory",
                                             (unsigned long long)want) : rc;
    Slot* old = h->slots; const uint64_t n_old = h->n_slots();
    const TableView old_view = h->view();
    uint32_t* old_rs = h->rstart;
    h->slots = fresh; h->n_regions = new_regions; h->rstart = fresh_rs;
    if (h->slots_dirty) h->slots_dirty = false;
    else hipLaunchKernelGGL(k_rehash, dim3(grid_for(h, n_old, 256)), dim3(256), 0, h->stream, h->view(), old_view);
    HIPC(hipStreamSynchronize(h->stream));
    HIPC(hipFree(old));
    if (old_rs) HIPC(hipFree(old_rs));
    return KQ_OK;
}
static int grow_hc(kq_handle* h, uint64_t need) {
    uint64_t want = h->hc_cap;
    while (want < need) want *= 2;
    HcSlot* fresh = nullptr;
    int rc = alloc_hc(h, want, &fresh);
    if (rc) return rc;
    HcSlot* old = h->hc; const uint64_t n_old = h->hc_cap;
    h->hc = fresh; h->hc_cap = want;
    HIPC(hipMemsetAsync(&h->st->hc_used, 0, sizeof(unsigned long long), h->stream));
    hipLaunchKernelGGL(k_rehash_hc, dim3(grid_for(h, n_old, 256)), dim3(256), 0, h->stream, h->view(), old, n_old);
    HIPC(hipStreamSynchronize(h->stream));
    HIPC(hipFree(old));
    return KQ_OK;
}

constexpr uint64_t HC_CAP_BIG = 1ull << 25;
static int reserve(kq_handle* h, uint64_t extra, uint64_t extra_instances) {
    int rc;
    bool state_read = false;
    if (!h->trust_capacity) {
        uint64_t need = (uint64_t)((double)(h->used_bound + extra) / 0.85) + REGION_SLOTS;
        if (need > h->n_slots()) {
            rc = read_state(h); if (rc) return rc;
            state_read = true;
            h->used_bound = h->st_host->slots_used;
            need = (uint64_t)((double)(h->used_bound + extra) / 0.85) + REGION_SLOTS;
            if (need > h->n_slots()) { rc = grow_main(h, need); if (rc) return rc; }
        }
    }
    h->used_bound += extra;
    h->kmers_bound += extra_instances;
    const uint64_t bound = h->kmers_bound / 255 + 1;
    uint64_t need_hc = 2 * std::min<uint64_t>(bound, 1ull << 23);
    if (bound > (1ull << 23)) need_hc = HC_CAP_BIG;
    if (bound > (1ull << 23) && h->kmers_bound >= h->hc_check_at && h->n_pend == 0) {
        if (!state_read) { rc = read_state_raw(h); if (rc) return rc; }
        need_hc = std::max<uint64_t>(need_hc, 8 * h->st_host->hc_used);
        h->hc_check_at = 2 * h->kmers_bound;
    }
    if (need_hc > h->hc_cap) { rc = grow_hc(h, need_hc); if (rc) return rc; }
    return KQ_OK;
}

static inline void aligned_view(const char* d, const uint8_t** ab, uint64_t* lead) {
    uintptr_t p = (uintptr_t)d;
    *lead = p & 15;
    *ab = (const uint8_t*)(p - *lead);
}

static int stage_in(kq_handle* h, const void* host, size_t bytes, void** dev) {
    int rc = ensure_buf(&h->stage, &h->stage_bytes, bytes + 64);
    if (rc) return rc;
    if (bytes) HIPC(hipMemcpyAsync(h->stage, host, bytes, hipMemcpyHostToDevice, h->stream));
    *dev = h->stage;
    return KQ_OK;
}

static void parallel_sort_entries(kq_entry* a, uint64_t n) {
    auto less = [](const kq_entry& x, const kq_entry& y) { return x.key < y.key; };
    unsigned hw = std::thread::hardware_concurrency();
    unsigned t = std::max(1u, std::min(16u, hw ? hw : 1u));
    while (t > 1 && n / t < (1u << 16)) t /= 2;
    if (t <= 1) { std::sort(a, a + n, less); return; }
    std::vector<uint64_t> cut(t + 1);
    for (unsigned i = 0; i <= t; ++i) cut[i] = n * i / t;
    {
        std::vector<std::thread> th;
        for (unsigned i = 0; i < t; ++i) th.emplace_back([&, i] { std::sort(a + cut[i], a + cut[i + 1], less); });
        for (auto& x : th) x.join();
    }
    for (unsigned width = 1; width < t; width *= 2) {
        std::vector<std::thread> th;
        for (unsigned i = 0; i + width < t; i += 2 * width) {
            const uint64_t lo = cut[i], mid = cut[i + width], hi = cut[std::min(i + 2 * width, t)];
            th.emplace_back([=] { std::inplace_merge(a + lo, a + mid, a + hi, less); });
        }
        for (auto& x : th) x.join();
    }
}

extern "C" {

const char* kq_last_error(void) { return g_err.c_str(); }
int kq_abi_version(void) { return KQ_ABI_VERSION; }

int kq_device_available(void) {
    int n = 0;
    if (hipGetDeviceCount(&n) != hipSuccess || n <= 0) return 0;
    hipDeviceProp_t p;
    if (hipGetDeviceProperties(&p, 0) != hipSuccess) return 0;
    return strncmp(p.gcnArchName, "gfx950", 6) == 0 ? 1 : 0;
}

int kq_device_memory(int device, uint64_t* free_bytes, uint64_t* total_bytes) {
    if (!free_bytes || !total_bytes) return fail(KQ_ERR_INVALID, "null argument");
    int n = 0;
    if (hipGetDeviceCount(&n) != hipSuccess || n <= 0) return fail(KQ_ERR_NO_DEVICE, "no HIP device visible (this library has no CPU path)");
    if (device < 0 || device >= n) return fail(KQ_ERR_NO_DEVICE, "device %d out of range (%d visible)", device, n);
    HIPC(hipSetDevice(device));
    size_t f = 0, t = 0;
    HIPC(hipMemGetInfo(&f, &t));
    *free_bytes = f; *total_bytes = t;
    return KQ_OK;
}

static uint64_t round_regions(uint64_t regions, int k) {
    if (regions < 16) regions = 16;
    if (regions >= (uint64_t)NB_MAX || k >= HI_K) regions = (regions + 255) / 256 * 256;
    if (regions >= (1ull << 19)) {
        uint32_t sbits = 3;
        while (sbits < SUB_BITS_MAX && (((regions + 255) / 256) >> sbits) > 256) ++sbits;
        const uint64_t unit = 256ull << sbits;
        regions = (regions + unit - 1) / unit * unit;
    }
    return regions;
}
static int set_window(kq_handle* h, uint32_t lo, uint32_t hi) {
    if (lo >= hi || hi > 256) return fail(KQ_ERR_INVALID, "bucket window [%u, %u) is not a range of the 256 hash-prefix buckets", lo, hi);
    if (h->k > (int)NARROW_MAX_K) return fail(KQ_ERR_INVALID, "bucket windows need k <= %u (5-byte records)", NARROW_MAX_K);
    if (!h->table_empty || h->n_pend || h->kmers_bound) return fail(KQ_ERR_INVALID, "the bucket window is chosen before anything is counted");
    if (h->windowed && hi - lo == h->win_hi - h->win_lo && !(lo == 0 && hi == 256)) {
        HIPC(hipStreamSynchronize(h->stream));
        h->win_lo = lo; h->win_hi = hi;
        return KQ_OK;
    }
    const uint64_t nb = hi - lo;
    const uint64_t alloc_now = h->n_alloc_regions();
    uint64_t virt = round_regions(std::max<uint64_t>((alloc_now + nb - 1) / nb * 256, (uint64_t)NB_MAX), h->k);
    if (virt >= (1ull << 32)) return fail(KQ_ERR_INVALID, "bucket window too narrow for a table of %llu regions", (unsigned long long)alloc_now);
    HIPC(hipStreamSynchronize(h->stream));
    const bool windowed = !(lo == 0 && hi == 256);
    const uint64_t alloc_new = windowed ? (uint64_t)(hi - lo) * (virt >> 8) : virt;
    Slot* fresh = nullptr;
    uint32_t* fresh_rs = nullptr;
    int rc = alloc_main(h, virt, alloc_new, &fresh, &fresh_rs);
    if (rc) return rc;
    HIPC(hipStreamSynchronize(h->stream));
    if (h->slots) (void)hipFree(h->slots);
    if (h->rstart) (void)hipFree(h->rstart);
    h->slots = fresh; h->rstart = fresh_rs;
    h->n_regions = virt; h->win_lo = lo; h->win_hi = hi; h->windowed = windowed;
    h->slots_dirty = false;
    return KQ_OK;
}

int kq_create(kq_handle** out, int device, int k, int map_count, uint64_t capacity_hint) {
    if (!out) return fail(KQ_ERR_INVALID, "out is null");
    *out = nullptr;
    if (k < 2 || k > 32) return fail(KQ_ERR_INVALID, "k must be in 2..32 (got %d)", k);
    if (map_count < 1 || map_count > 65535) return fail(KQ_ERR_INVALID, "map_count must be in 1..65535 (got %d)", map_count);
    int n = 0;
    if (hipGetDeviceCount(&n) != hipSuccess || n <= 0) return fail(KQ_ERR_NO_DEVICE, "no HIP device visible (this library has no CPU path)");
    if (device < 0 || device >= n) return fail(KQ_ERR_NO_DEVICE, "device %d out of range (%d visible)", device, n);
    HIPC(hipSetDevice(device));
    hipDeviceProp_t prop;
    HIPC(hipGetDeviceProperties(&prop, device));
    if (strncmp(prop.gcnArchName, "gfx950", 6) != 0)
        return fail(KQ_ERR_NO_DEVICE, "device %d is %s; this library carries gfx950 code only", device, prop.gcnArchName);
    kq_handle* h = new (std::nothrow) kq_handle();
    if (!h) return fail(KQ_ERR_NOMEM, "host allocation failed");
    h->device = device; h->k = k; h->map_count = map_count; h->n_cu = prop.multiProcessorCount;
    h->filt_hi = (uint32_t)map_count;
    hipError_t e = hipStreamCreateWithFlags(&h->own_stream, hipStreamNonBlocking);
    if (e != hipSuccess) { delete h; return fail(KQ_ERR_HIP, "hipStreamCreate: %s", hipGetErrorString(e)); }
    h->stream = h->base = h->own_stream;
    int rc = KQ_OK;
    do {
        if (hipMalloc((void**)&h->st, sizeof(DevState)) != hipSuccess || hipHostMalloc((void**)&h->st_host, sizeof(DevState)) != hipSuccess) {
            rc = fail(KQ_ERR_NOMEM, "state allocation failed"); break;
        }
        (void)hipMemsetAsync(h->st, 0, sizeof(DevState), h->stream);
        uint64_t slots = (uint64_t)((double)(capacity_hint ? capacity_hint : (1u << 20)) / 0.7);
        const uint64_t regions = round_regions((slots + REGION_SLOTS - 1) >> REGION_SHIFT, k);
        rc = alloc_main(h, regions, regions, &h->slots, &h->rstart); if (rc) break;
        h->n_regions = regions;
        uint64_t hc = 1u << 16;
        rc = alloc_hc(h, hc, &h->hc); if (rc) break;
        h->hc_cap = hc;
        if (hipStreamSynchronize(h->stream) != hipSuccess) { rc = fail(KQ_ERR_HIP, "table initialisation failed"); break; }
    } while (0);
    if (rc) { kq_destroy(h); return rc; }
    *out = h;
    return KQ_OK;
}

void kq_destroy(kq_handle* h) {
    if (!h) return;
    (void)hipSetDevice(h->device);
    if (h->stream) (void)hipStreamSynchronize(h->stream);
    if (h->slots) (void)hipFree(h->slots);
    if (h->rstart) (void)hipFree(h->rstart);
    if (h->hc) (void)hipFree(h->hc);
    if (h->st) (void)hipFree(h->st);
    if (h->st_host) (void)hipHostFree(h->st_host);
    if (h->scratch) (void)hipFree(h->scratch);
    if (h->stage) (void)hipFree(h->stage);
    if (h->part) (void)hipFree(h->part);
    scr_free(h->part2); scr_free(h->fork_part2);
    for (auto& e : h->hist_cache) (void)hipFree(e.m1_all);
    for (int w = 0; w < 2; ++w) { if (h->fork_stream[w]) { (void)hipStreamSynchronize(h->fork_stream[w]); (void)hipStreamDestroy(h->fork_stream[w]); } }
    if (h->fork_part[1]) (void)hipFree(h->fork_part[1]);
    for (auto e : h->ev_ring) if (e) (void)hipEventDestroy(e);
    if (h->ev_pass) (void)hipEventDestroy(h->ev_pass);
    for (int i = 0; i < kq_handle::IN_SLOTS; ++i) { if (h->in_buf[i]) (void)hipFree(h->in_buf[i]); if (h->in_consumed[i]) (void)hipEventDestroy(h->in_consumed[i]); }
    for (auto e : h->in_copied) (void)hipEventDestroy(e);
    for (int i = 0; i < kq_handle::IN_SLOTS; ++i) if (h->in_cmp[i]) (void)hipFree(h->in_cmp[i]);
    if (h->fx_units) (void)hipFree(h->fx_units);
    if (h->fx_out) (void)hipFree(h->fx_out);
    if (h->fx_res) (void)hipFree(h->fx_res);
    if (h->fx_res_host) (void)hipHostFree(h->fx_res_host);
    if (h->copy_stream) (void)hipStreamDestroy(h->copy_stream);
    arena_release(h);
    if (h->d_sets) (void)hipFree(h->d_sets);
    if (h->hot) (void)hipFree(h->hot);
    marks_reset(h);
    if (h->own_stream) (void)hipStreamDestroy(h->own_stream);
    delete h;
}

int kq_clear(kq_handle* h) {
    if (!h) return fail(KQ_ERR_INVALID, "null handle");
    HIPC(hipSetDevice(h->device));
    h->slots_dirty = true;
    clear_words(h, h->hc, sizeof(HcSlot) / 8, h->hc_cap);
    HIPC(hipMemsetAsync(h->st, 0, sizeof(DevState), h->stream));
    h->kmers_bound = 0;
    h->used_bound = 0;
    h->hc_check_at = 0;
    h->table_empty = true;
    h->n_pend = 0; h->arena_used = 0; h->pend_records = 0;
    h->fx_bad = 0;
    return KQ_OK;
}

int kq_set_stream(kq_handle* h, void* s) {
    if (!h) return fail(KQ_ERR_INVALID, "null handle");
    HIPC(hipStreamSynchronize(h->stream));
    h->stream = h->base = s ? (hipStream_t)s : h->own_stream;
    return KQ_OK;
}
int kq_set_option(kq_handle* h, int option, int64_t value) {
    if (!h) return fail(KQ_ERR_INVALID, "null handle");
    switch (option) {
        case KQ_OPT_TRUST_CAPACITY: h->trust_capacity = value != 0; return KQ_OK;
        case KQ_OPT_COUNT_PATH:
            if (value < 0 || value > 2) return fail(KQ_ERR_INVALID, "KQ_OPT_COUNT_PATH must be 0, 1 or 2");
            h->count_path = (int)value; return KQ_OK;
        case KQ_OPT_COUNT_MAP_RANGE: {
            const int64_t lo = value & 0xFFFF, hi = (value >> 16) & 0xFFFF;
            if (lo >= hi || hi > h->map_count) return fail(KQ_ERR_INVALID, "map range [%lld,%lld) outside [0,%d]", (long long)lo, (long long)hi, h->map_count);
            h->filt_lo = (uint32_t)lo; h->filt_hi = (uint32_t)hi; return KQ_OK;
        }
        case KQ_OPT_NARROW_MID:
            if (value < 2 || value > (1 << 14)) return fail(KQ_ERR_INVALID, "KQ_OPT_NARROW_MID must be in [2, 16384]");
            h->mid_rps = (uint32_t)value; return KQ_OK;
        case KQ_OPT_MERGE_PATH:
            if (value < 0 || value > 2) return fail(KQ_ERR_INVALID, "KQ_OPT_MERGE_PATH must be 0, 1 or 2");
            h->merge_path = (int)value; return KQ_OK;
        case KQ_OPT_LOOKUP_PATH:
            if (value < 0 || value > 2) return fail(KQ_ERR_INVALID, "KQ_OPT_LOOKUP_PATH must be 0, 1 or 2");
            h->lookup_path = (int)value; return KQ_OK;
        case KQ_OPT_PROFILE: h->profile = value != 0; if (!h->profile) marks_reset(h); return KQ_OK;
        case KQ_OPT_TEST_FAIL_PLAN: h->test_fail_plan = value != 0; return KQ_OK;
        case KQ_OPT_COUNT_MAP_PASSES: {
            if (value != 1 && value != 2 && value != 4 && value != 8) return fail(KQ_ERR_INVALID, "KQ_OPT_COUNT_MAP_PASSES must be 1, 2, 4 or 8");
            if ((h->map_count & (h->map_count - 1)) != 0 || value > h->map_count) return fail(KQ_ERR_INVALID, "KQ_OPT_COUNT_MAP_PASSES needs a power-of-two map count");
            HIPC(hipStreamSynchronize(h->stream));
            for (auto& e : h->hist_cache) (void)hipFree(e.m1_all);
            h->hist_cache.clear(); h->hist_cache_bytes = 0;
            h->map_passes = (int)value; return KQ_OK;
        }
        case KQ_OPT_KERNEL_SET:
            if (value < 0 || value > 7) return fail(KQ_ERR_INVALID, "KQ_OPT_KERNEL_SET is a mask of bits 1, 2, 4");
            h->kernel_set = (int)value; return KQ_OK;
        case KQ_OPT_OVERLAP:
            if (value < 0 || value > 2) return fail(KQ_ERR_INVALID, "KQ_OPT_OVERLAP must be 0, 1 or 2");
            h->overlap = (int)value; return KQ_OK;
        case KQ_OPT_PENDING_BYTES: {
            if (value < -1) return fail(KQ_ERR_INVALID, "KQ_OPT_PENDING_BYTES must be -1 (auto), 0 (off) or a byte count");
            int rc = flush_pending(h);
            if (rc) return rc;
            if (h->arena && value != h->pend_budget) { HIPC(hipStreamSynchronize(h->stream)); arena_release(h); }
            h->pend_budget = value; return KQ_OK;
        }
        case KQ_OPT_BUCKET_WINDOW:
            HIPC(hipSetDevice(h->device));
            return set_window(h, (uint32_t)(value & 0xFFFF), (uint32_t)((value >> 16) & 0xFFFF));
        case KQ_OPT_SLICE_KMERS:
            if (value < 1) return fail(KQ_ERR_INVALID, "KQ_OPT_SLICE_KMERS must be positive");
            h->slice_kmers = (uint64_t)value; h->slice_user = true; return KQ_OK;
        default: return fail(KQ_ERR_INVALID, "unknown option %d", option);
    }
}
int kq_get_profile(kq_handle* h, char* buf, uint64_t cap) {
    if (!h || !buf || !cap) return fail(KQ_ERR_INVALID, "null argument");
    HIPC(hipSetDevice(h->device));
    HIPC(hipStreamSynchronize(h->stream));
    std::string out;
    for (size_t i = 1; i < h->marks.size(); ++i) {
        float ms = 0;
        HIPC(hipEventElapsedTime(&ms, h->marks[i - 1].second, h->marks[i].second));
        char tmp[96];
        snprintf(tmp, sizeof tmp, "%s%s=%.4f", out.empty() ? "" : ";", h->marks[i].first, ms);
        out += tmp;
    }
    if (out.size() + 1 > cap) return fail(KQ_ERR_CAPACITY, "profile buffer too small: need %zu", out.size() + 1);
    memcpy(buf, out.c_str(), out.size() + 1);
    return KQ_OK;
}
void* kq_get_stream(kq_handle* h) { return h ? (void*)h->stream : nullptr; }
int kq_sync(kq_handle* h) {
    if (!h) return fail(KQ_ERR_INVALID, "null handle");
    HIPC(hipSetDevice(h->device));
    HIPC(hipStreamSynchronize(h->stream));
    const int rc = check_errors(h);
    if (h->fx_bad) return fail(KQ_ERR_INVALID, "malformed %s text was submitted for counting and skipped (kq_clear resets this)", h->fx_bad == KQ_FASTX_FASTQ ? "FASTQ" : "FASTA");
    return rc;
}
int kq_flush(kq_handle* h) {
    if (!h) return fail(KQ_ERR_INVALID, "null handle");
    HIPC(hipSetDevice(h->device));
    return flush_pending(h);
}
int kq_get_info(kq_handle* h, kq_info* out) {
    if (!h || !out) return fail(KQ_ERR_INVALID, "null argument");
    HIPC(hipSetDevice(h->device));
    int rc = read_state(h);
    if (rc) return rc;
    out->kmers_counted = h->st_host->kmers_added;
    out->slots_used = h->st_host->slots_used;
    out->slots_total = h->n_slots();
    out->hc_used = h->st_host->hc_used;
    out->hc_total = h->hc_cap;
    out->table_bytes = h->n_slots() * sizeof(Slot) + h->hc_cap * sizeof(HcSlot);
    out->table_passes = h->table_passes;
    return KQ_OK;
}

struct PartPlan {
    PartCfg cfg;
    bool two_level;
    int fmt;
    uint64_t n_max, R;
    uint32_t g1;
    uint64_t m1_n, m2_n, sums_n, groups_n;
    uint64_t *recs1, *recs2;
    uint8_t *aux1, *aux2;
    unsigned long long *m1, *seg_off, *unit_base, *group_base, *sums, *total, *hot;
    uint32_t* m2;
};
static void plan_cfg(const kq_handle* h, PartCfg* cfg, bool allow_narrow = false) {
    cfg->n_regions = h->n_regions;
    uint32_t g = 1;
    while (((cfg->n_regions + (1ull << g) - 1) >> g) > 512 && g < 10) ++g;
    while (((cfg->n_regions + (1ull << g) - 1) >> g) >= (uint64_t)NB_MAX) ++g;
    cfg->g_shift = cfg->n_regions < (uint64_t)NB_MAX ? 0 : g;
    cfg->n_coarse = (uint32_t)((cfg->n_regions + (1ull << cfg->g_shift) - 1) >> cfg->g_shift);
    cfg->mode = 0; cfg->map_count = (uint32_t)h->map_count;
    cfg->map_mask = (h->map_count & (h->map_count - 1)) == 0 ? (uint32_t)h->map_count - 1 : 0;
    cfg->filt_lo = 0; cfg->filt_hi = (uint32_t)h->map_count;
    cfg->raw_out = 0;
    cfg->narrow = 0; cfg->sub_bits = 0; cfg->owner_sub = 0; cfg->n_rng = 0; cfg->win_lo = 0; cfg->win_hi = 1u << NARROW_CBITS;
    if (allow_narrow && (h->k <= (int)NARROW_MAX_K || h->k > PART_MAX_K) && cfg->n_regions >= (uint64_t)NB_MAX && cfg->n_regions % (1u << NARROW_CBITS) == 0) {
        const uint64_t rps = cfg->n_regions >> NARROW_CBITS;
        uint32_t sb = 0;
        if (rps >= h->mid_rps) {
            const uint64_t target_nb = std::max<uint64_t>(1, std::min<uint64_t>(256, h->mid_rps / 8));
            while ((rps >> sb) > target_nb && sb < SUB_BITS_MAX && rps % (2ull << sb) == 0) ++sb;
        }
        if ((rps >> sb) < (uint64_t)NB_MAX && (sb > 0 || rps < (uint64_t)NB_MAX)) { cfg->narrow = 1; cfg->sub_bits = sb; }
    }
    if (cfg->narrow) { cfg->n_coarse = 1u << NARROW_CBITS; if (cfg->g_shift == 0) cfg->g_shift = 1; }
}
static int plan_alloc(kq_handle* h, PartPlan* p, uint64_t n_max, uint64_t n_tiles, uint32_t p1_bins, bool allow_narrow = false,
                      uint64_t min_segs = 0 ) {
    if (h->test_fail_plan) { h->test_fail_plan = false; return fail(KQ_ERR_NOMEM, "partition scratch allocation failed (injected by KQ_OPT_TEST_FAIL_PLAN)"); }
    if (n_max >= (1ull << 32) - 16) return fail(KQ_ERR_INVALID, "a partition pass handles fewer than 2^32 records (got %llu): slice the input", (unsigned long long)n_max);
    plan_cfg(h, &p->cfg, allow_narrow);
    n_max = (n_max + 7) & ~7ull;
    p->two_level = p->cfg.g_shift != 0;
    p->fmt = !p->cfg.narrow ? FMT_PACK8 : h->k > PART_MAX_K ? FMT_TOP8 : FMT_NARROW;
    p->n_max = n_max; p->R = p->cfg.n_regions;
    p->g1 = (uint32_t)std::max<uint64_t>(1, std::min<uint64_t>(n_tiles, (uint64_t)h->n_cu * (p1_bins < 512 ? 18 : 12)));
    p->m1_n = (uint64_t)p1_bins * p->g1 * P1_F;
    const uint64_t nb_max = std::max<uint64_t>(std::max<uint64_t>(1ull << p->cfg.g_shift, p->cfg.n_coarse), p->cfg.narrow ? (p->cfg.n_regions >> NARROW_CBITS) >> p->cfg.sub_bits : 0);
    const uint64_t seg_max = std::max<uint64_t>(min_segs, p->cfg.narrow ? ((uint64_t)1 << NARROW_CBITS) << p->cfg.sub_bits : (uint64_t)NB_MAX);
    p->m2_n = (n_max / P2_UNIT + seg_max + 2) * nb_max;
    p->groups_n = std::max<uint64_t>(std::max<uint64_t>(p->R, (uint64_t)p->cfg.n_coarse << p->cfg.g_shift), min_segs) + 2;
    p->sums_n = std::max(p->m1_n, p->groups_n) / SCAN_CHUNK + 2;
    const uint64_t aux_words = (n_max + 7) / 8 + 1;
    const uint64_t rec_words = p->fmt == FMT_NARROW ? n_max / 2 + 2 : n_max;
    const bool split2 = (rec_words + aux_words) * 8 >= ((size_t)512 << 20);
    if (split2) { int rc2 = scr_ensure(h->part2, (size_t)(rec_words + aux_words) * 8, h->device); if (rc2) return rc2; }
    const size_t words = (size_t)((split2 ? 1 : 2) * (rec_words + aux_words) + p->m1_n + 2 * (seg_max + 2) + p->groups_n + p->sums_n + 4 + (p->R + 2) + (p->m2_n + 1) / 2);
    int rc = ensure_buf(&h->part, &h->part_bytes, words * 8);
    if (rc) return rc;
    p->recs1 = (uint64_t*)h->part;
    p->aux1 = (uint8_t*)(p->recs1 + rec_words);
    uint64_t* rest = (uint64_t*)(p->aux1 + aux_words * 8);
    if (split2) { p->recs2 = (uint64_t*)h->part2.p; p->aux2 = (uint8_t*)(p->recs2 + rec_words); }
    else { p->recs2 = rest; p->aux2 = (uint8_t*)(p->recs2 + rec_words); rest = (uint64_t*)(p->aux2 + aux_words * 8); }
    p->m1 = (unsigned long long*)rest;
    p->seg_off = p->m1 + p->m1_n;
    p->unit_base = p->seg_off + seg_max + 2;
    p->group_base = p->unit_base + seg_max + 2;
    p->sums = p->group_base + p->groups_n;
    p->total = p->sums + p->sums_n;
    p->hot = p->total + 4;
    p->m2 = (uint32_t*)(p->hot + p->R + 2);
    return KQ_OK;
}
static void scan_u64(kq_handle* h, unsigned long long* a, uint64_t n, unsigned long long* sums_scratch, unsigned long long* total) {
    if (n <= 2 * SCAN_CHUNK) {
        hipLaunchKernelGGL(k_exclusive_scan, dim3(1), dim3(1024), 0, h->stream, a, n, total);
        return;
    }
    const uint64_t chunks = (n + SCAN_CHUNK - 1) / SCAN_CHUNK;
    hipLaunchKernelGGL(k_scan_sums, dim3((unsigned)chunks), dim3(1024), 0, h->stream, a, n, sums_scratch);
    hipLaunchKernelGGL(k_exclusive_scan, dim3(1), dim3(1024), 0, h->stream, sums_scratch, chunks, total);
    hipLaunchKernelGGL(k_scan_apply, dim3((unsigned)chunks), dim3(1024), 0, h->stream, a, n, sums_scratch);
}
static void mark(kq_handle* h, const char* name) {
    if (!h->profile) return;
    hipEvent_t e;
    if (hipEventCreate(&e) != hipSuccess) return;
    (void)hipEventRecord(e, h->stream);
    h->marks.emplace_back(name, e);
}
static void marks_reset(kq_handle* h) {
    for (auto& m : h->marks) (void)hipEventDestroy(m.second);
    h->marks.clear();
}

static void run_p1(kq_handle* h, PartPlan* p, const PartCfg& cfg, const uint8_t* ab, uint64_t lead, uint64_t len, EmitRange er, uint64_t* out,
                   uint8_t* out_aux, int aux_fmt, const uint16_t* pinv = nullptr ) {
    const bool plain = cfg.mode == 0 && cfg.filt_lo == 0 && cfg.filt_hi == cfg.map_count;
    const bool owner_plain = cfg.mode == 1 && cfg.map_mask != 0 && cfg.filt_lo == 0 && cfg.filt_hi == cfg.map_count;
    const bool narrow_filt = cfg.mode == 0 && cfg.narrow && !plain && cfg.map_mask != 0 && h->k <= (int)NARROW_MAX_K;
    const bool narrow_win = plain && cfg.narrow && h->k <= (int)NARROW_MAX_K && (cfg.win_lo != 0 || cfg.win_hi != (1u << NARROW_CBITS));
    const int binmode = owner_plain ? 3 : narrow_filt ? 4 : narrow_win ? 6 : !plain ? 0 : cfg.narrow ? 2 : 1;
    auto cached_hist = [&](const kq_handle::HistKey& key, size_t bytes, auto launch) -> kq_handle::HistEntry* {
        for (auto& e : h->hist_cache) if (e.key == key) return &e;
        if (h->hist_cache_bytes + bytes > ((size_t)4 << 30)) return nullptr;
        unsigned long long* buf = nullptr;
        if (hipMalloc((void**)&buf, bytes) != hipSuccess) { (void)hipGetLastError(); return nullptr; }
        launch(buf);
        h->hist_cache.push_back(kq_handle::HistEntry{key, buf, bytes});
        h->hist_cache_bytes += bytes;
        return &h->hist_cache.back();
    };
    bool have_hist = false;
    const size_t row = (size_t)p->g1 * sizeof(unsigned long long), block = row << NARROW_CBITS;
    if (narrow_filt && h->map_passes > 1 && P1_F == 1 && !h->hist_cache_off) {
        const uint32_t n = (uint32_t)h->map_passes, per = cfg.map_count / n, rr = cfg.filt_lo / per;
        if (cfg.filt_lo == rr * per && cfg.filt_hi == (rr + 1) * per) {
            const auto* ent = cached_hist({ab, pinv, lead, len, er.lo, er.hi, p->g1, n, h->k}, n * block, [&](unsigned long long* buf) {
                PartCfg all = cfg;
                all.n_rng = n; all.n_coarse = n << NARROW_CBITS;
                if (h->k == 21) hipLaunchKernelGGL((k_p1_hist<5, 21>), dim3(p->g1), dim3(TILE_THREADS), 0, h->stream, ab, lead, len, h->k, all, er, p->g1, buf, pinv);
                else hipLaunchKernelGGL((k_p1_hist<5, 0>), dim3(p->g1), dim3(TILE_THREADS), 0, h->stream, ab, lead, len, h->k, all, er, p->g1, buf, pinv);
            });
            if (ent) {
                (void)hipMemcpyAsync(p->m1, (const char*)ent->m1_all + rr * block, block, hipMemcpyDeviceToDevice, h->stream);
                have_hist = true;
            }
        }
    }
    if (narrow_win && h->map_passes > 1 && P1_F == 1 && !h->hist_cache_off) {
        const auto* ent = cached_hist({ab, pinv, lead, len, er.lo, er.hi, p->g1, 0xB0C4E7u, h->k}, block, [&](unsigned long long* buf) {
            PartCfg all = cfg;
            all.win_lo = 0; all.win_hi = 1u << NARROW_CBITS;
            if (h->k == 21) hipLaunchKernelGGL((k_p1_hist<2, 21>), dim3(p->g1), dim3(TILE_THREADS), 0, h->stream, ab, lead, len, h->k, all, er, p->g1, buf, pinv);
            else hipLaunchKernelGGL((k_p1_hist<2, 0>), dim3(p->g1), dim3(TILE_THREADS), 0, h->stream, ab, lead, len, h->k, all, er, p->g1, buf, pinv);
        });
        if (ent) {
            (void)hipMemcpyAsync(p->m1, ent->m1_all, block, hipMemcpyDeviceToDevice, h->stream);
            if (cfg.win_lo) (void)hipMemsetAsync(p->m1, 0, (size_t)cfg.win_lo * row, h->stream);
            if (cfg.win_hi < (1u << NARROW_CBITS)) (void)hipMemsetAsync((char*)p->m1 + (size_t)cfg.win_hi * row, 0, (size_t)((1u << NARROW_CBITS) - cfg.win_hi) * row, h->stream);
            have_hist = true;
        }
    }
#define KQ_P1H(B, K) hipLaunchKernelGGL((k_p1_hist<B, K>), dim3(p->g1 * P1_F), dim3(TILE_THREADS), 0, h->stream, ab, lead, len, h->k, cfg, er, p->g1, p->m1, pinv)
    if (have_hist) { }
    else if (binmode == 6) { if (h->k == 21) KQ_P1H(6, 21); else KQ_P1H(6, 0); }
    else if (binmode == 2) { if (h->k == 21) KQ_P1H(2, 21); else KQ_P1H(2, 0); }
    else if (binmode == 1) { if (h->k == 31) KQ_P1H(1, 31); else KQ_P1H(1, 0); }
    else if (binmode == 3) { if (h->k == 21) KQ_P1H(3, 21); else KQ_P1H(3, 0); }
    else if (binmode == 4) { if (h->k == 21) KQ_P1H(4, 21); else KQ_P1H(4, 0); }
    else KQ_P1H(0, 0);
#undef KQ_P1H
    scan_u64(h, p->m1, (uint64_t)cfg.n_coarse * p->g1 * P1_F, p->sums, p->total);
    hipLaunchKernelGGL(k_p1_offsets, dim3((cfg.n_coarse + 256) / 256), dim3(256), 0, h->stream, p->m1, p->total, cfg, p->g1, p->seg_off);
    mark(h, "k_p1_hist+scan");
    const bool small = cfg.n_coarse < 512;
#define KQ_P1S(W, N, B, K) hipLaunchKernelGGL((k_p1_scatter<W, N, B, K>), dim3(p->g1), dim3(TILE_THREADS), 0, h->stream, ab, lead, len, h->k, cfg, er, p->m1, out, out_aux, aux_fmt, pinv)
#define KQ_P1T(B, K) do { if (h->kernel_set & 1) KQ_P1S(FMT_TOP8, 512, B, K); else \
        hipLaunchKernelGGL((k_p1_scatter_s<B, K, 1, true>), dim3(p->g1), dim3(TILE_THREADS), 0, h->stream, ab, lead, len, h->k, cfg, er, p->m1, (uint32_t*)out, out_aux, pinv); } while (0)
    if (cfg.narrow && h->k > PART_MAX_K) { if (plain && h->k == 31) KQ_P1T(2, 31); else if (plain) KQ_P1T(2, 0); else KQ_P1T(0, 0); }
#define KQ_P1N(B, K, T) do { if (h->kernel_set & 1) KQ_P1S(FMT_NARROW, 512, B, K); else \
        hipLaunchKernelGGL((k_p1_scatter_s<B, K, T>), dim3(p->g1), dim3(TILE_THREADS * T), 0, h->stream, ab, lead, len, h->k, cfg, er, p->m1, (uint32_t*)out, out_aux, pinv); } while (0)
    else if (narrow_filt)  { if (h->k == 21) KQ_P1N(4, 21, 1); else KQ_P1N(4, 0, 1); }
    else if (narrow_win)   { if (h->k == 21) KQ_P1N(6, 21, 1); else KQ_P1N(6, 0, 1); }
    else if (cfg.narrow)   { if (plain && h->k == 21) KQ_P1N(2, 21, KQ_P1S_TPR); else if (plain) KQ_P1N(2, 0, KQ_P1S_TPR); else KQ_P1N(0, 0, 1); }
    else if (out_aux && plain && h->k == 31) { if (small) KQ_P1S(FMT_WIDE, 512, 1, 31); else KQ_P1S(FMT_WIDE, NB_MAX, 1, 31); }
    else if (out_aux) { if (small) KQ_P1S(FMT_WIDE, 512, 0, 0); else KQ_P1S(FMT_WIDE, NB_MAX, 0, 0); }
    else if (owner_plain && !out_aux && small) { if (h->k == 21) KQ_P1S(FMT_PACK8, 512, 3, 21); else KQ_P1S(FMT_PACK8, 512, 3, 0); }
    else if (plain)   { if (small) KQ_P1S(FMT_PACK8, 512, 1, 0); else KQ_P1S(FMT_PACK8, NB_MAX, 1, 0); }
    else              { if (small) KQ_P1S(FMT_PACK8, 512, 0, 0); else KQ_P1S(FMT_PACK8, NB_MAX, 0, 0); }
#undef KQ_P1S
#undef KQ_P1N
#undef KQ_P1T
    mark(h, "k_p1_scatter");
}
static void run_level(kq_handle* h, PartPlan* p, const LevelCfg& lv, const uint64_t* in, const uint8_t* in_aux, uint64_t* out, uint8_t* out_aux,
                      unsigned long long* gb = nullptr ,
                      const unsigned long long* seg_hi = nullptr ) {
    if (!gb) gb = p->group_base;
    if (!seg_hi) seg_hi = p->seg_off + 1;
    LevelCfg lvr = lv;
    lvr.rep_shift = 0;
    while (lvr.rep_shift < 6 && (((uint64_t)lv.nb + 1) << (lvr.rep_shift + 1)) <= 512) ++lvr.rep_shift;
    const LevelCfg& lv_ = lvr;
    const int fmt = lv.narrow == 2 ? FMT_TOP8 : lv.narrow ? FMT_NARROW : in_aux != nullptr ? FMT_WIDE : FMT_PACK8;
    const uint64_t groups = (uint64_t)(lv.n_seg / lv.spb) * lv.nb;
    hipLaunchKernelGGL(k_lv_units, dim3(1), dim3(1024), 0, h->stream, p->seg_off, seg_hi, lv_, p->unit_base);
    const unsigned unit_grid = (unsigned)std::min<uint64_t>(p->n_max / P2_UNIT + lv.n_seg + 1, 1u << 30);
    if (fmt == FMT_TOP8) hipLaunchKernelGGL(k_lv_hist<FMT_TOP8>, dim3(unit_grid), dim3(MS_THREADS), 0, h->stream, in, in_aux, lv_, p->seg_off, seg_hi, p->unit_base, p->m2);
    else if (fmt == FMT_NARROW) hipLaunchKernelGGL(k_lv_hist<FMT_NARROW>, dim3(unit_grid), dim3(MS_THREADS), 0, h->stream, in, in_aux, lv_, p->seg_off, seg_hi, p->unit_base, p->m2);
    else if (fmt == FMT_WIDE) hipLaunchKernelGGL(k_lv_hist<FMT_WIDE>, dim3(unit_grid), dim3(MS_THREADS), 0, h->stream, in, in_aux, lv_, p->seg_off, seg_hi, p->unit_base, p->m2);
    else hipLaunchKernelGGL(k_lv_hist<FMT_PACK8>, dim3(unit_grid), dim3(MS_THREADS), 0, h->stream, in, in_aux, lv_, p->seg_off, seg_hi, p->unit_base, p->m2);
    if (p->n_max / P2_UNIT + 1 <= 8 * (uint64_t)(lv.n_seg / lv.spb))
        hipLaunchKernelGGL(k_lv_offsets_thread, dim3((unsigned)((groups + 255) / 256)), dim3(256), 0, h->stream, p->m2, lv_, p->unit_base, gb);
    else
        hipLaunchKernelGGL(k_lv_offsets, dim3((unsigned)((groups * 64 + 255) / 256)), dim3(256), 0, h->stream, p->m2, lv_, p->unit_base, gb);
    (void)hipMemsetAsync(gb + groups, 0, 8, h->stream);
    scan_u64(h, gb, groups + 1, p->sums, p->total + 1);
    mark(h, "k_lv_hist+offsets+scan");
    const bool small = lv.nb < 512;
#define KQ_LVS(W, N) hipLaunchKernelGGL((k_lv_scatter<W, N>), dim3(unit_grid), dim3(LV_THREADS), 0, h->stream, in, in_aux, lv_, \
                                        p->seg_off, seg_hi, p->unit_base, p->m2, gb, out, out_aux)
    if (lv.top8)              { KQ_LVS(FMT_PACK8_TO_NARROW, 512); }
    else if (fmt == FMT_TOP8) { if (small) KQ_LVS(FMT_TOP8, 512); else KQ_LVS(FMT_TOP8, NB_MAX); }
#define KQ_LVN(T) hipLaunchKernelGGL((k_lv_scatter_s<T>), dim3(unit_grid), dim3(LV_THREADS), 0, h->stream, (const uint32_t*)in, in_aux, lv_, \
                                      p->seg_off, seg_hi, p->unit_base, p->m2, gb, (uint32_t*)out, out_aux)
    else if (fmt == FMT_NARROW && small && lv.rstart && !(h->kernel_set & 4)) { KQ_LVN(true); }
    else if (fmt == FMT_NARROW && small && !lv.rstart && (h->kernel_set & 2)) { KQ_LVN(false); }
#undef KQ_LVN
    else if (fmt == FMT_NARROW && lv.rstart) { if (small) KQ_LVS(FMT_NARROW_TO_TIGHT, 512); else KQ_LVS(FMT_NARROW_TO_TIGHT, NB_MAX); }
    else if (fmt == FMT_NARROW) { if (small) KQ_LVS(FMT_NARROW, 512); else KQ_LVS(FMT_NARROW, NB_MAX); }
    else if (fmt == FMT_WIDE) { if (small) KQ_LVS(FMT_WIDE, 512); else KQ_LVS(FMT_WIDE, NB_MAX); }
    else                      { if (small) KQ_LVS(FMT_PACK8, 512); else KQ_LVS(FMT_PACK8, NB_MAX); }
#undef KQ_LVS
    mark(h, "k_lv_scatter");
}
static LevelCfg level_coarse_to_regions(const PartCfg& cfg) {
    LevelCfg lv; lv.n_regions = cfg.n_regions; lv.n_seg = cfg.n_coarse; lv.nb = 1u << cfg.g_shift; lv.seg_shift = cfg.g_shift; lv.out_shift = 0; lv.in_raw = 0; lv.k = 0; lv.narrow = 0; lv.top8 = 0;
    lv.nr_shift = lv.nr_rps = lv.nr_sub = lv.nr_inv = 0; lv.nr_div = 1;
    lv.nr_mid = 0; lv.nr_fshift = 24; lv.nr_fmask = 0xFFFFFFu; lv.nr_f24 = 0;
    lv.spb = 1;
    return lv;
}
static LevelCfg level_narrow(const PartCfg& cfg, uint32_t sub_bits = 0, bool middle = false, bool top8_records = false) {
    LevelCfg lv; lv.n_regions = cfg.n_regions;
    const uint32_t rps = (uint32_t)(cfg.n_regions >> NARROW_CBITS), subsz = rps >> sub_bits;
    lv.seg_shift = 0; lv.out_shift = 0; lv.in_raw = 0; lv.k = 0; lv.narrow = top8_records ? 2 : 1; lv.top8 = 0;
    lv.nr_rps = rps; lv.nr_sub = subsz;
    if (middle) { lv.n_seg = 1u << NARROW_CBITS; lv.nb = 1u << sub_bits; lv.nr_shift = 0; lv.nr_div = subsz; }
    else        { lv.n_seg = (1u << NARROW_CBITS) << sub_bits; lv.nb = subsz; lv.nr_shift = sub_bits; lv.nr_div = 1; }
    lv.nr_inv = lv.nr_div > 1 ? (uint32_t)(((1ull << 32) + lv.nr_div - 1) / lv.nr_div) : 0;
    lv.nr_mid = middle ? 1u : 0u; lv.nr_fshift = 24 - sub_bits; lv.nr_fmask = (1u << (24 - sub_bits)) - 1u;
    lv.nr_f24 = ((uint64_t)subsz << (24 - sub_bits)) <= (1ull << 32) && subsz < (1u << 24) ? 1u : 0u;
    lv.spb = 1;
    return lv;
}
static void run_narrow_levels(kq_handle* h, PartPlan* p, const uint64_t** sorted, const uint8_t** sorted_aux, const P3Set* dst = nullptr, bool tight = false);
static bool tight_ok(const kq_handle* h, const PartPlan& p) { return p.fmt == FMT_NARROW && p.R >= TIGHT_MIN_REGIONS && h->rstart != nullptr; }
static LevelCfg level_flat_to_coarse(const PartCfg& cfg) {
    LevelCfg lv; lv.n_regions = cfg.n_regions; lv.n_seg = 1; lv.nb = cfg.n_coarse; lv.seg_shift = 32; lv.out_shift = cfg.g_shift; lv.in_raw = 0; lv.k = 0; lv.narrow = 0; lv.top8 = 0;
    lv.nr_shift = lv.nr_rps = lv.nr_sub = lv.nr_inv = 0; lv.nr_div = 1;
    lv.nr_mid = 0; lv.nr_fshift = 24; lv.nr_fmask = 0xFFFFFFu; lv.nr_f24 = 0;
    lv.spb = 1;
    return lv;
}
__global__ void k_p3set(P3Set* sets, int i, P3Set v) { sets[i] = v; }

static size_t set_bytes(uint64_t n_max, int fmt, uint64_t R) {
    const size_t rec = (fmt == FMT_NARROW || fmt == FMT_TIGHT) ? 4 : 8;
    const bool aux = fmt == FMT_NARROW || fmt == FMT_WIDE;
    return ((((size_t)n_max * rec + 63) & ~(size_t)63) + (aux ? (((size_t)n_max + 63) & ~(size_t)63) : 0) + (size_t)(R + 2) * 8 + 255) & ~(size_t)255;
}
static int arena_take(kq_handle* h, uint64_t n_max, int fmt, uint64_t R, P3Set* out, bool* ok) {
    *ok = false;
    if (h->pend_budget == 0) return KQ_OK;
    const size_t need = set_bytes(n_max, fmt, R);
    bool was_full = false;
    if (h->n_pend && (h->n_pend >= P3_MAX_SETS || h->pend_fmt != fmt || h->arena_used + need > h->arena_bytes)) {
        was_full = h->pend_fmt == fmt && h->n_pend < P3_MAX_SETS;
        int rc = flush_pending(h);
        if (rc) return rc;
    }
    size_t want = h->arena_bytes;
    if (need > want) want = h->pend_budget > 0 ? (size_t)h->pend_budget : std::max<size_t>(4 * need, (size_t)64 << 20);
    else if (was_full && h->pend_budget < 0) want = 2 * h->arena_bytes;
    if (want > h->arena_bytes) {
        size_t free_b = 0, total_b = 0;
        if (hipMemGetInfo(&free_b, &total_b) != hipSuccess) return KQ_OK;
        size_t budget = want;
        const size_t avail = free_b + h->arena_bytes, reserve = std::max<size_t>(total_b / 8, (size_t)8 << 30);
        const size_t ceiling = avail > 2 * reserve ? avail - reserve : avail / 2;
        if (h->pend_budget < 0) budget = std::min<size_t>(want, std::min<size_t>(ceiling, std::max<size_t>(4 * need, 4 * (size_t)h->n_slots() * sizeof(Slot))));
        if (budget <= h->arena_bytes && need <= h->arena_bytes) budget = 0;
        if (budget && budget < need) return KQ_OK;
        if (budget) {
            if (h->arena) { HIPC(hipStreamSynchronize(h->stream)); HIPC(hipStreamSynchronize(h->base)); arena_release(h); }
            static const bool scramble_arena = !getenv("KQ_SCRAMBLE_ARENA") || atoi(getenv("KQ_SCRAMBLE_ARENA")) != 0;
            if (scramble_arena && budget >= ((size_t)1 << 30) && scr_try_vmm(h->arena_scr, budget, h->device)) h->arena = h->arena_scr.p;
            else
            if (hipMalloc(&h->arena, budget) != hipSuccess) { (void)hipGetLastError(); h->arena = nullptr; return KQ_OK; }
            h->arena_bytes = budget; h->arena_used = 0;
        }
    }
    uint8_t* base = (uint8_t*)h->arena + h->arena_used;
    const size_t rec = (fmt == FMT_NARROW || fmt == FMT_TIGHT) ? 4 : 8;
    const bool aux = fmt == FMT_NARROW || fmt == FMT_WIDE;
    out->recs = (const uint64_t*)base;
    base += ((size_t)n_max * rec + 63) & ~(size_t)63;
    out->aux = aux ? base : nullptr;
    if (aux) base += ((size_t)n_max + 63) & ~(size_t)63;
    out->base = (const unsigned long long*)base;
    out->n_max = n_max;
    h->arena_used += need;
    *ok = true;
    return KQ_OK;
}
static int pend_add(kq_handle* h, const P3Set& set, int fmt, int aux_fmt) {
    if (h->n_pend && (h->n_pend >= P3_MAX_SETS || h->pend_fmt != fmt || h->pend_aux_fmt != aux_fmt)) {
        int rc = flush_pending(h);
        if (rc) return rc;
    }
    if (!h->d_sets) HIPC(hipMalloc((void**)&h->d_sets, sizeof(P3Set) * P3_MAX_SETS));
    hipLaunchKernelGGL(k_p3set, dim3(1), dim3(1), 0, h->stream, h->d_sets, h->n_pend, set);
    h->pend_fmt = fmt; h->pend_aux_fmt = aux_fmt;
    ++h->n_pend;
    h->pend_records += set.n_max;
    return KQ_OK;
}
static int flush_pending_base(kq_handle* h);
static int flush_pending(kq_handle* h) {
    if (!h->n_pend) return KQ_OK;
    hipStream_t work = h->stream;
    h->stream = h->base;
    int rc = join_forks(h);
    if (!rc) rc = flush_pending_base(h);
    if (!rc && h->fork_stream[0]) {
        hipEvent_t e; rc = ev_get(h, &e);
        if (!rc && hipEventRecord(e, h->base) != hipSuccess) rc = fail(KQ_ERR_HIP, "hipEventRecord failed");
        for (int w = 0; w < 2 && !rc; ++w) if (hipStreamWaitEvent(h->fork_stream[w], e, 0) != hipSuccess) rc = fail(KQ_ERR_HIP, "hipStreamWaitEvent failed");
    }
    h->stream = work;
    return rc;
}
static int flush_pending_base(kq_handle* h) {
    const uint64_t R = h->n_regions;
    int rc = ensure_buf(&h->hot, &h->hot_bytes, (size_t)(R + 2) * 8);
    if (rc) return rc;
    if (h->kmers_bound / 255 + 1 > (1ull << 23)) {
        rc = read_state_raw(h); if (rc) return rc;
        const uint64_t need_hc = std::max<uint64_t>(HC_CAP_BIG, 8 * h->st_host->hc_used);
        if (need_hc > h->hc_cap) { rc = grow_hc(h, need_hc); if (rc) return rc; }
    }
    unsigned long long* hot = (unsigned long long*)h->hot;
    HIPC(hipMemsetAsync(hot, 0, 8, h->stream));
    const dim3 grid((unsigned)std::min<uint64_t>(h->n_alloc_regions(), 1u << 30)), grid_hot(h->n_cu), block(P3_THREADS);
    const int empty = h->slots_dirty ? 2 : h->table_empty ? 1 : 0;
    const int fmt = h->pend_fmt;
    const uint32_t rps = (fmt == FMT_NARROW || fmt == FMT_TIGHT || fmt == FMT_TOP8) ? (uint32_t)(R >> NARROW_CBITS) : 1u;
#define KQ_HOT(F) hipLaunchKernelGGL((k_count_regions<F, true>), grid_hot, block, 0, h->stream, h->view(), h->d_sets, (uint32_t)h->n_pend, h->pend_aux_fmt, empty, hot, rps)
#define KQ_P3(F) do { \
        hipLaunchKernelGGL((k_count_regions<F, false>), grid, block, 0, h->stream, h->view(), h->d_sets, (uint32_t)h->n_pend, h->pend_aux_fmt, empty, hot, rps); \
        KQ_HOT(F); } while (0)
#define KQ_Q4(KC, T) do { \
        hipLaunchKernelGGL((k_count_regions_q4<KC, T>), grid, dim3(Q4_THREADS), 0, h->stream, h->view(), h->d_sets, (uint32_t)h->n_pend, empty, hot, rps); \
        KQ_HOT(FMT_NARROW); } while (0)
    if (fmt == FMT_TIGHT)       { if (h->k == 21) KQ_Q4(21, true); else KQ_Q4(0, true); }
    else if (fmt == FMT_NARROW) { if (h->k == 21) KQ_Q4(21, false); else KQ_Q4(0, false); }
    else if (fmt == FMT_TOP8) KQ_P3(FMT_TOP8);
    else if (fmt == FMT_WIDE) KQ_P3(FMT_WIDE);
    else KQ_P3(FMT_PACK8);
#undef KQ_Q4
#undef KQ_P3
#undef KQ_HOT
    h->n_pend = 0; h->arena_used = 0; h->pend_records = 0;
    ++h->table_passes;
    h->slots_dirty = false;
    h->table_empty = false;
    mark(h, "k_count_regions");
    HIPC(hipGetLastError());
    return KQ_OK;
}

static bool part_table_ok(const kq_handle* h, bool narrow_possible) {
    if (h->n_regions <= (1ull << 20)) return true;
    if (!narrow_possible) return false;
    PartCfg c; plan_cfg(h, &c, true);
    return c.narrow != 0;
}
static void run_narrow_levels(kq_handle* h, PartPlan* p, const uint64_t** sorted, const uint8_t** sorted_aux, const P3Set* dst, bool tight) {
    const uint32_t sb = p->cfg.sub_bits;
    const bool t8 = p->fmt == FMT_TOP8;
    uint8_t* a1 = t8 ? nullptr : p->aux1;
    uint8_t* a2 = t8 ? nullptr : p->aux2;
    uint64_t* fin = dst ? const_cast<uint64_t*>(dst->recs) : (sb == 0 ? p->recs2 : p->recs1);
    uint8_t* fin_aux = (t8 || tight) ? nullptr : dst ? const_cast<uint8_t*>(dst->aux) : (sb == 0 ? a2 : a1);
    unsigned long long* fin_base = dst ? const_cast<unsigned long long*>(dst->base) : p->group_base;
    LevelCfg last = level_narrow(p->cfg, sb, false, t8);
    if (tight) last.rstart = h->rstart;
    if (sb == 0) {
        run_level(h, p, last, p->recs1, a1, fin, fin_aux, fin_base);
    } else {
        run_level(h, p, level_narrow(p->cfg, sb, true, t8), p->recs1, a1, p->recs2, a2);
        (void)hipMemcpyAsync(p->seg_off, p->group_base, (size_t)(((1u << NARROW_CBITS) << sb) + 1) * 8, hipMemcpyDeviceToDevice, h->stream);
        run_level(h, p, last, p->recs2, a2, fin, fin_aux, fin_base);
    }
    *sorted = fin; *sorted_aux = fin_aux;
}

static int pend_or_apply(kq_handle* h, const P3Set& set, int fmt, int aux_fmt, bool in_arena) {
    int rc = pend_add(h, set, fmt, aux_fmt);
    if (rc) return rc;
    return in_arena ? KQ_OK : flush_pending(h);
}

static int count_partitioned(kq_handle* h, const uint8_t* ab, uint64_t lead, uint64_t len, EmitRange er, const uint16_t* pinv = nullptr) {
    PartPlan p;
    PartCfg c0; plan_cfg(h, &c0, true);
    int rc = plan_alloc(h, &p, len, n_tiles_of(lead, len), c0.n_coarse, true);
    if (rc) return rc;
    if (h->k > PART_MAX_K && p.fmt != FMT_TOP8) p.fmt = FMT_WIDE;
    const bool has_aux = p.fmt == FMT_WIDE || p.fmt == FMT_NARROW;
    uint8_t* a1 = has_aux ? p.aux1 : nullptr;
    uint8_t* a2 = has_aux ? p.aux2 : nullptr;
    p.cfg.filt_lo = h->filt_lo; p.cfg.filt_hi = h->filt_hi;
    if (h->windowed) { p.cfg.win_lo = h->win_lo; p.cfg.win_hi = h->win_hi; }
    const bool leveled = p.fmt == FMT_NARROW || p.fmt == FMT_TOP8 || p.two_level;
    P3Set set; bool in_arena = false;
    const bool tight = tight_ok(h, p);
    const int set_fmt = tight ? FMT_TIGHT : p.fmt;
    const bool filtered = p.cfg.filt_lo != 0 || p.cfg.filt_hi != p.cfg.map_count || h->windowed;
    if (leveled && !filtered) { rc = arena_take(h, p.n_max, set_fmt, p.R, &set, &in_arena); if (rc) return rc; }
    marks_reset(h);
    mark(h, "start");
    run_p1(h, &p, p.cfg, ab, lead, len, er, p.recs1, a1, AUX_IDX6, pinv);
    if (leveled && filtered) {
        unsigned long long n_recs = 0;
        HIPC(hipMemcpyAsync(&n_recs, p.total, sizeof n_recs, hipMemcpyDeviceToHost, h->stream));
        HIPC(hipStreamSynchronize(h->stream));
        rc = arena_take(h, std::min<uint64_t>(p.n_max, ((uint64_t)n_recs + 15) & ~7ull), set_fmt, p.R, &set, &in_arena); if (rc) return rc;
    }
    if (p.fmt == FMT_NARROW || p.fmt == FMT_TOP8) {
        const uint64_t* sorted; const uint8_t* sorted_aux;
        run_narrow_levels(h, &p, &sorted, &sorted_aux, in_arena ? &set : nullptr, tight);
        if (!in_arena) set = P3Set{sorted, sorted_aux, p.group_base, p.n_max};
    } else if (p.two_level) {
        if (in_arena) run_level(h, &p, level_coarse_to_regions(p.cfg), p.recs1, a1, const_cast<uint64_t*>(set.recs), const_cast<uint8_t*>(set.aux), const_cast<unsigned long long*>(set.base));
        else { run_level(h, &p, level_coarse_to_regions(p.cfg), p.recs1, a1, p.recs2, a2); set = P3Set{p.recs2, a2, p.group_base, p.n_max}; }
    } else {
        set = P3Set{p.recs1, a1, p.seg_off, p.n_max};
    }
    HIPC(hipGetLastError());
    return pend_or_apply(h, set, set_fmt, tight ? AUX_TIGHT : AUX_IDX6, in_arena);
}
static int count_partitioned_records(kq_handle* h, const uint64_t* d_recs, const uint8_t* d_aux, int aux_fmt, uint64_t n, bool raw) {
    PartPlan p;
    int rc = plan_alloc(h, &p, n, 0, 1, !d_aux && !raw);
    if (rc) return rc;
    P3Set set; bool in_arena = false;
    if (p.fmt == FMT_NARROW) {
        const bool tight = tight_ok(h, p);
        rc = arena_take(h, p.n_max, tight ? FMT_TIGHT : p.fmt, p.R, &set, &in_arena); if (rc) return rc;
        hipLaunchKernelGGL(k_set2, dim3(1), dim3(1), 0, h->stream, p.seg_off, 0ull, (unsigned long long)n);
        LevelCfg first = level_flat_to_coarse(p.cfg);
        first.top8 = 1; first.nb = 1u << NARROW_CBITS;
        run_level(h, &p, first, d_recs, nullptr, p.recs1, p.aux1);
        HIPC(hipMemcpyAsync(p.seg_off, p.group_base, (size_t)((1u << NARROW_CBITS) + 1) * 8, hipMemcpyDeviceToDevice, h->stream));
        const uint64_t* sorted; const uint8_t* sorted_aux;
        run_narrow_levels(h, &p, &sorted, &sorted_aux, in_arena ? &set : nullptr, tight);
        if (!in_arena) set = P3Set{sorted, sorted_aux, p.group_base, p.n_max};
        HIPC(hipGetLastError());
        return pend_or_apply(h, set, tight ? FMT_TIGHT : FMT_NARROW, tight ? AUX_TIGHT : AUX_IDX6, in_arena);
    }
    if (d_aux) p.fmt = FMT_WIDE;
    uint8_t* a1 = d_aux ? p.aux1 : nullptr;
    uint8_t* a2 = d_aux ? p.aux2 : nullptr;
    hipLaunchKernelGGL(k_set2, dim3(1), dim3(1), 0, h->stream, p.seg_off, 0ull, (unsigned long long)n);
    LevelCfg first = level_flat_to_coarse(p.cfg);
    first.in_raw = raw ? 1 : 0; first.k = (uint32_t)h->k;
    run_level(h, &p, first, d_recs, d_aux, p.recs1, a1);
    if (p.two_level) {
        HIPC(hipMemcpyAsync(p.seg_off, p.group_base, (size_t)(p.cfg.n_coarse + 1) * 8, hipMemcpyDeviceToDevice, h->stream));
        run_level(h, &p, level_coarse_to_regions(p.cfg), p.recs1, a1, p.recs2, a2);
        set = P3Set{p.recs2, a2, p.group_base, p.n_max};
    } else {
        set = P3Set{p.recs1, a1, p.group_base, p.n_max};
    }
    HIPC(hipGetLastError());
    return pend_or_apply(h, set, p.fmt, aux_fmt, false);
}

static int count_seq_dev(kq_handle* h, const char* d_bases, const uint16_t* d_inv, uint64_t len) {
    if (!h || (!d_bases && len)) return fail(KQ_ERR_INVALID, "null argument");
    HIPC(hipSetDevice(h->device));
    if (len < (uint64_t)h->k) return KQ_OK;
    const uint64_t kmers = len - h->k + 1;
    uint64_t slice = h->slice_kmers;
    if (h->pend_budget != 0 && !h->slice_user && kmers > slice) {
        const uint64_t base_slice = slice;
        for (uint64_t cap : {1ull << 31, 1ull << 30}) {
            slice = std::min<uint64_t>(cap, std::max<uint64_t>(base_slice, h->n_slots() / 4));
            const uint64_t n_slices = (kmers + slice - 1) / slice;
            slice = (kmers + n_slices - 1) / n_slices;
            size_t free_b = 0, total_b = 0;
            if (cap == (1ull << 30) || slice <= (1ull << 30)) break;
            if (hipMemGetInfo(&free_b, &total_b) == hipSuccess && free_b + h->part_bytes >= (size_t)11 * slice + ((size_t)2 << 30)) break;
        }
    }
    if (h->pend_budget == 0 && !h->slice_user && kmers > slice && 2 * h->n_slots() > slice) {
        size_t free_b = 0, total_b = 0;
        if (hipMemGetInfo(&free_b, &total_b) == hipSuccess) {
            const uint64_t by_mem = (uint64_t)((free_b + h->part_bytes) / 24);
            slice = std::max(slice, std::min<uint64_t>(std::min<uint64_t>(2 * h->n_slots(), 1ull << 31), by_mem));
        }
    }
    struct ForkGuard {
        kq_handle* h; bool swapped = false;
        void leave() { if (swapped) { std::swap(h->part, h->fork_part[1]); std::swap(h->part_bytes, h->fork_part_bytes[1]); std::swap(h->part2, h->fork_part2); swapped = false; } h->stream = h->base; }
        ~ForkGuard() { leave(); (void)join_forks(h); }
    } guard{h};
    const bool forked = h->overlap && !h->profile && h->count_path != 1 && (kmers + slice - 1) / slice >= 2 && slice >= (1u << 20) &&
                        (h->overlap == 2 || (h->filt_lo == 0 && h->filt_hi == (uint32_t)h->map_count && !h->windowed));
    if (forked) {
        for (int w = 0; w < 2; ++w) if (!h->fork_stream[w]) HIPC(hipStreamCreateWithFlags(&h->fork_stream[w], hipStreamNonBlocking));
        hipEvent_t e_in; int erc = ev_get(h, &e_in); if (erc) return erc;
        HIPC(hipEventRecord(e_in, h->base));
        for (int w = 0; w < 2; ++w) HIPC(hipStreamWaitEvent(h->fork_stream[w], e_in, 0));
    }
    uint64_t slice_no = 0;
    for (uint64_t a = 0; a < kmers; a += slice, ++slice_no) {
        const uint64_t b = std::min(kmers, a + slice);
        int rc = reserve(h, b - a, b - a);
        if (rc) return rc;
        const uint64_t sub_off = a ? a - 1 : 0;
        const uint64_t sub_len = std::min(len, b + h->k) - sub_off;
        const EmitRange er{a - sub_off, b - sub_off};
        const uint8_t* ab; uint64_t lead;
        const uint16_t* pinv = nullptr;
        if (d_inv) { ab = (const uint8_t*)(reinterpret_cast<const uint32_t*>(d_bases) + sub_off / 16); pinv = d_inv + sub_off / 16; lead = sub_off % 16; }
        else aligned_view(d_bases + sub_off, &ab, &lead);
        double pass_records = (double)(b - a);
        if (h->pend_budget != 0) {
            const double per_set = (double)set_bytes(b - a, FMT_PACK8, h->n_regions);
            const double room = h->arena ? (double)h->arena_bytes : 4.0 * (double)h->n_slots() * sizeof(Slot);
            pass_records = (double)h->pend_records + (double)(b - a) * std::max(1.0, std::min(8.0, room / per_set));
        }
        bool part = (b - a) >= (1u << 20) && part_table_ok(h, true) &&
                    (double)h->n_slots() * sizeof(Slot) <= 200.0 * pass_records;
        if (h->count_path == 1) part = false;
        if (h->count_path == 2) {
            if (!part_table_ok(h, true)) return fail(KQ_ERR_INVALID, "table too large for the partitioned path");
            part = true;
        }
        if (part) {
            if (forked) {
                const int w = (int)(slice_no & 1);
                if (w == 1) { std::swap(h->part, h->fork_part[1]); std::swap(h->part_bytes, h->fork_part_bytes[1]); std::swap(h->part2, h->fork_part2); guard.swapped = true; }
                h->stream = h->fork_stream[w];
                h->fork_busy[w] = true;
            }
            rc = count_partitioned(h, ab, lead, sub_len, er, pinv);
            if (forked) h->fork_busy[slice_no & 1] = true;
            guard.leave();
            if (rc) return rc;
            continue;
        }
        if (forked) { rc = join_forks(h); if (rc) return rc; }
        PartCfg filt; plan_cfg(h, &filt);
        filt.filt_lo = h->filt_lo; filt.filt_hi = h->filt_hi;
        materialize(h);
        h->table_empty = false;
        hipLaunchKernelGGL(k_count_direct, dim3(grid_for(h, n_tiles_of(lead, sub_len), 1, 32)), dim3(TILE_THREADS), 0, h->stream,
                           h->view(), ab, lead, sub_len, h->k, er, filt, pinv);
        HIPC(hipGetLastError());
    }
    return KQ_OK;
}
int kq_count_batch_dev(kq_handle* h, const char* d_bases, uint64_t len) { return count_seq_dev(h, d_bases, nullptr, len); }
int kq_count_packed_dev(kq_handle* h, const uint32_t* d_codes, const uint16_t* d_inv, uint64_t n_bases) {
    if (!d_inv && n_bases) return fail(KQ_ERR_INVALID, "null argument");
    return count_seq_dev(h, (const char*)d_codes, d_inv, n_bases);
}
void kq_pack_bases(const char* bases, uint64_t len, uint32_t* codes, uint16_t* inv) {
    static const struct Lut { uint8_t v[256]; Lut() { for (int i = 0; i < 256; ++i) v[i] = 4; v['A'] = v['a'] = 0; v['C'] = v['c'] = 1; v['G'] = v['g'] = 2; v['T'] = v['t'] = 3; } } lut;
    const uint64_t full = len / 16;
    const uint8_t* b = (const uint8_t*)bases;
    for (uint64_t u = 0; u < full; ++u, b += 16) {
        uint32_t c = 0, m = 0;
        for (int i = 0; i < 16; ++i) { const uint32_t x = lut.v[b[i]]; c |= (x & 3u) << (2 * i); m |= (x >> 2) << i; }
        codes[u] = c; inv[u] = (uint16_t)m;
    }
    if (len % 16) {
        uint32_t c = 0, m = 0xFFFFu;
        for (uint64_t i = 0; i < len % 16; ++i) { const uint32_t x = lut.v[b[i]]; c |= (x & 3u) << (2 * i); if (!(x >> 2)) m &= ~(1u << i); }
        codes[full] = c; inv[full] = (uint16_t)m;
    }
}
int kq_count_batch(kq_handle* h, const char* bases, uint64_t len) {
    if (!h || (!bases && len)) return fail(KQ_ERR_INVALID, "null argument");
    HIPC(hipSetDevice(h->device));
    void* d = nullptr;
    int rc = stage_in(h, bases, len, &d);
    if (rc) return rc;
    rc = kq_count_batch_dev(h, (const char*)d, len);
    if (rc) return rc;
    HIPC(hipStreamSynchronize(h->stream));
// ... 773 lines not shown
```

Measured before the change: 51.27 billion.

## Split pending arena into bucket bands and apply table passes per band

Adds a band arena that splits the pending-record arena into per-bucket-range bands. The final narrow scatter writes records directly into per-band destinations, and table count passes can run over just the regions of full bands instead of sweeping the whole table. This is meant to let more batches accumulate before a pass and to cut full-table region visits. In exchange it adds a host sync to read bucket offsets, extra small kernels, and more complex bookkeeping for partially cleared tables.

```diff
diff --git a/include/kreeq_amd.h b/include/kreeq_amd.h
--- a/include/kreeq_amd.h
+++ b/include/kreeq_amd.h
@@ -50,6 +50,8 @@
     uint64_t hc_total;
     uint64_t table_bytes;
     uint64_t table_passes;
+    uint64_t band_passes;
+    uint64_t region_visits;
 } kq_info;
 
 
@@ -59,7 +61,7 @@
 int  kq_set_stream(kq_handle* h, void* hip_stream);
 void* kq_get_stream(kq_handle* h);
 enum { KQ_OPT_TRUST_CAPACITY = 1, KQ_OPT_COUNT_PATH = 2, KQ_OPT_SLICE_KMERS = 3, KQ_OPT_COUNT_MAP_RANGE = 4, KQ_OPT_PROFILE = 5,
-       KQ_OPT_LOOKUP_PATH = 6, KQ_OPT_MERGE_PATH = 7, KQ_OPT_NARROW_MID = 8, KQ_OPT_PENDING_BYTES = 9, KQ_OPT_BUCKET_WINDOW = 10, KQ_OPT_OVERLAP = 11, KQ_OPT_COUNT_MAP_PASSES = 12, KQ_OPT_KERNEL_SET = 13,
+       KQ_OPT_LOOKUP_PATH = 6, KQ_OPT_MERGE_PATH = 7, KQ_OPT_NARROW_MID = 8, KQ_OPT_PENDING_BYTES = 9, KQ_OPT_BUCKET_WINDOW = 10, KQ_OPT_OVERLAP = 11, KQ_OPT_COUNT_MAP_PASSES = 12, KQ_OPT_KERNEL_SET = 13, KQ_OPT_BAND_PASSES = 14,
        KQ_OPT_TEST_FAIL_PLAN = 100  };
 int  kq_set_option(kq_handle* h, int option, int64_t value);
 int  kq_get_profile(kq_handle* h, char* buf, uint64_t cap);
diff --git a/kreeq_amd/build.py b/kreeq_amd/build.py
--- a/kreeq_amd/build.py
+++ b/kreeq_amd/build.py
@@ -9,7 +9,7 @@
 HOSTLIB = os.path.join(PKG, "lib", "libkreeq_host.so")
 
 HIP_SOURCES = [os.path.join(PKG, "csrc", "kreeq_amd.hip")]
-HIP_DEPS = HIP_SOURCES + [os.path.join(PKG, "csrc", f) for f in ("kq_device.h", "kq_partition.h", "kq_kernels.h", "kq_fastx.h")] + [os.path.join(ROOT, "include", "kreeq_amd.h")]
+HIP_DEPS = HIP_SOURCES + [os.path.join(PKG, "csrc", f) for f in ("kq_device.h", "kq_partition.h", "kq_band_arena.h", "kq_kernels.h", "kq_fastx.h")] + [os.path.join(ROOT, "include", "kreeq_amd.h")]
 HOST_DIR = os.path.join(PKG, "host")
 
 
diff --git a/kreeq_amd/capi.py b/kreeq_amd/capi.py
--- a/kreeq_amd/capi.py
+++ b/kreeq_amd/capi.py
@@ -30,7 +30,8 @@
 
 class Info(C.Structure):
     _fields_ = [("kmers_counted", C.c_uint64), ("slots_used", C.c_uint64), ("slots_total", C.c_uint64), ("hc_used", C.c_uint64),
-                ("hc_total", C.c_uint64), ("table_bytes", C.c_uint64), ("table_passes", C.c_uint64)]
+                ("hc_total", C.c_uint64), ("table_bytes", C.c_uint64), ("table_passes", C.c_uint64),
+                ("band_passes", C.c_uint64), ("region_visits", C.c_uint64)]
 
 
 _lib = None
@@ -176,7 +177,7 @@
         _check(load().kq_flush(self._h))
 
     def set_option(self, option, value):
-        opt = {"trust_capacity": 1, "count_path": 2, "slice_kmers": 3, "count_map_range": 4, "profile": 5, "lookup_path": 6, "merge_path": 7, "narrow_mid": 8, "pending_bytes": 9, "bucket_window": 10, "overlap": 11, "count_map_passes": 12, "kernel_set": 13, "test_fail_plan": 100}[option]
+        opt = {"trust_capacity": 1, "count_path": 2, "slice_kmers": 3, "count_map_range": 4, "profile": 5, "lookup_path": 6, "merge_path": 7, "narrow_mid": 8, "pending_bytes": 9, "bucket_window": 10, "overlap": 11, "count_map_passes": 12, "kernel_set": 13, "band_passes": 14, "test_fail_plan": 100}[option]
         if option == "count_map_range":
             value = int(value[0]) | (int(value[1]) << 16)
         if option in ("count_path", "lookup_path", "merge_path"):
diff --git a/kreeq_amd/csrc/kq_band_arena.h b/kreeq_amd/csrc/kq_band_arena.h
--- /dev/null
+++ b/kreeq_amd/csrc/kq_band_arena.h
@@ -0,0 +1,89 @@
+#pragma once
+#include <cstddef>
+#include <cstdint>
+#include <vector>
+
+#ifndef KQ_BANDS
+#define KQ_BANDS 8
+#endif
+
+namespace kq {
+
+constexpr int BANDS = KQ_BANDS;
+
+struct BandArena {
+    static constexpr size_t ALIGN = 256;
+    struct Piece { int band, area; size_t off, len; };
+    size_t lo[BANDS + 1] = {};
+    size_t cur[BANDS] = {};
+    size_t live[BANDS] = {};
+    std::vector<Piece> pieces;
+
+    static size_t align_up(size_t n) { return (n + ALIGN - 1) & ~(ALIGN - 1); }
+    void init(size_t arena_bytes) {
+        const size_t per = arena_bytes / BANDS & ~(ALIGN - 1);
+        for (int a = 0; a <= BANDS; ++a) lo[a] = per * (size_t)a;
+        clear();
+    }
+    void clear() {
+        pieces.clear();
+        for (int a = 0; a < BANDS; ++a) { cur[a] = lo[a]; live[a] = 0; }
+    }
+    bool empty() const { return pieces.empty(); }
+    size_t room(int a) const { return lo[a + 1] - cur[a]; }
+    size_t band_bytes(int band) const {
+        size_t n = 0;
+        for (const Piece& p : pieces) if (p.band == band) n += p.len;
+        return n;
+    }
+    bool place(const size_t (&len)[BANDS], size_t (&off)[BANDS]) {
+        size_t c[BANDS];
+        int area[BANDS];
+        for (int a = 0; a < BANDS; ++a) c[a] = cur[a];
+        for (int j = 0; j < BANDS; ++j) {
+            area[j] = -1;
+            if (!len[j]) continue;
+            const size_t n = align_up(len[j]);
+            int best = j;
+            if (c[j] + n > lo[j + 1]) {
+                best = -1;
+                for (int a = 0; a < BANDS; ++a)
+                    if (c[a] + n <= lo[a + 1] && (best < 0 || lo[a + 1] - c[a] > lo[best + 1] - c[best])) best = a;
+                if (best < 0) return false;
+            }
+            area[j] = best; off[j] = c[best]; c[best] += n;
+        }
+        for (int j = 0; j < BANDS; ++j) {
+            if (area[j] < 0) continue;
+            const size_t n = align_up(len[j]);
+            pieces.push_back(Piece{j, area[j], off[j], n});
+            cur[area[j]] = off[j] + n; live[area[j]] += n;
+        }
+        return true;
+    }
+    void apply_band(int band) {
+        size_t w = 0;
+        for (size_t i = 0; i < pieces.size(); ++i) {
+            const Piece& p = pieces[i];
+            if (p.band == band) { live[p.area] -= p.len; continue; }
+            pieces[w++] = p;
+        }
+        pieces.resize(w);
+        for (int a = 0; a < BANDS; ++a) if (!live[a]) cur[a] = lo[a];
+    }
+    int bands_to_fit(const size_t (&len)[BANDS], int (&order)[BANDS]) const {
+        size_t fill[BANDS], off[BANDS];
+        for (int j = 0; j < BANDS; ++j) { order[j] = j; fill[j] = band_bytes(j); }
+        for (int i = 1; i < BANDS; ++i)
+            for (int q = i; q > 0 && fill[order[q]] > fill[order[q - 1]]; --q) { const int t = order[q]; order[q] = order[q - 1]; order[q - 1] = t; }
+        BandArena trial = *this;
+        for (int n = 0; n <= BANDS; ++n) {
+            BandArena probe = trial;
+            if (probe.place(len, off)) return n;
+            if (n < BANDS) trial.apply_band(order[n]);
+        }
+        return BANDS + 1;
+    }
+};
+
+}
diff --git a/kreeq_amd/csrc/kq_kernels.h b/kreeq_amd/csrc/kq_kernels.h
--- a/kreeq_amd/csrc/kq_kernels.h
+++ b/kreeq_amd/csrc/kq_kernels.h
@@ -416,8 +416,8 @@
 __global__ __launch_bounds__(LV_THREADS, KQ_LV_OCC) void k_lv_scatter(const uint64_t* __restrict__ recs, const uint8_t* __restrict__ recs_aux, LevelCfg lv,
                                                            const unsigned long long* __restrict__ seg_off, const unsigned long long* __restrict__ seg_hi,
                                                            const unsigned long long* __restrict__ unit_base, const uint32_t* __restrict__ m2,
-                                                           const unsigned long long* __restrict__ group_base, uint64_t* __restrict__ out,
-                                                           uint8_t* __restrict__ out_aux) {
+                                                           const unsigned long long* __restrict__ group_base_, uint64_t* __restrict__ out_,
+                                                           uint8_t* __restrict__ out_aux_, const BandSeg* __restrict__ bseg = nullptr ) {
     constexpr bool WIDE = FMT == FMT_WIDE, TIGHT = FMT == FMT_NARROW_TO_TIGHT, NARROW = FMT == FMT_NARROW || TIGHT, CONVERT = FMT == FMT_PACK8_TO_NARROW,
                    TOP8 = FMT == FMT_TOP8, HAS_AUX = WIDE || NARROW;
     constexpr int MS_FMT = (CONVERT || TIGHT) ? FMT_NARROW : TOP8 ? FMT_PACK8 : FMT;
@@ -431,6 +431,13 @@
         const uint32_t b = lv.spb > 1 ? b_in / lv.spb : b_in;
         const uint64_t lo = seg_off[b_in] + (u - unit_base[b_in]) * P2_UNIT;
         const uint64_t hi = lo + P2_UNIT < seg_hi[b_in] ? lo + P2_UNIT : seg_hi[b_in];
+        const unsigned long long* __restrict__ group_base = group_base_;
+        uint64_t* __restrict__ out = out_;
+        uint8_t* __restrict__ out_aux = out_aux_;
+        if (NARROW && bseg) {
+            const BandSeg bs = bseg[b >> lv.nr_shift];
+            group_base = bs.base; out = reinterpret_cast<uint64_t*>(bs.out); out_aux = bs.aux;
+        }
         for (uint32_t i = threadIdx.x; i < nb; i += LV_THREADS)
             s.gbase[i] = (uint32_t)(group_base[(uint64_t)b * nb + i] + m2[u * nb + i]);
         if (TIGHT) {
@@ -490,8 +497,8 @@
 __global__ __launch_bounds__(LV_THREADS, TIGHT ? KQ_LVS_OCC_TIGHT : KQ_LVS_OCC) void k_lv_scatter_s(const uint32_t* __restrict__ recs32, const uint8_t* __restrict__ recs_aux, LevelCfg lv,
                                                            const unsigned long long* __restrict__ seg_off, const unsigned long long* __restrict__ seg_hi,
                                                            const unsigned long long* __restrict__ unit_base, const uint32_t* __restrict__ m2,
-                                                           const unsigned long long* __restrict__ group_base, uint32_t* __restrict__ out,
-                                                           uint8_t* __restrict__ out_aux) {
+                                                           const unsigned long long* __restrict__ group_base_, uint32_t* __restrict__ out_,
+                                                           uint8_t* __restrict__ out_aux_, const BandSeg* __restrict__ bseg = nullptr ) {
     constexpr int NC = 512;
     static_assert(LV_THREADS == NC && LV_ITEMS == 8, "one counter per thread");
     __shared__ uint64_t s_buf[LV_TILE];
@@ -507,6 +514,13 @@
         const uint32_t b = lv.spb > 1 ? b_in / lv.spb : b_in;
         const uint64_t lo = seg_off[b_in] + (u - unit_base[b_in]) * P2_UNIT;
         const uint64_t hi = lo + P2_UNIT < seg_hi[b_in] ? lo + P2_UNIT : seg_hi[b_in];
+        const unsigned long long* __restrict__ group_base = group_base_;
+        uint32_t* __restrict__ out = out_;
+        uint8_t* __restrict__ out_aux = out_aux_;
+        if (bseg) {
+            const BandSeg bs = bseg[b >> lv.nr_shift];
+            group_base = bs.base; out = bs.out; out_aux = bs.aux;
+        }
         uint32_t gabs = own_bin ? (uint32_t)(group_base[(uint64_t)b * nb + my_bin] + m2[u * nb + my_bin]) : 0u;
         if (TIGHT) {
             const uint32_t first = (b >> lv.nr_shift) * lv.nr_rps + (b & ((1u << lv.nr_shift) - 1u)) * lv.nr_sub;
@@ -582,6 +596,29 @@
     }
 }
 __global__ void k_set2(unsigned long long* p, unsigned long long a, unsigned long long b) { p[0] = a; p[1] = b; }
+
+__global__ __launch_bounds__(256) void k_band_segs(BandDst d, BandSeg* __restrict__ seg) {
+    const uint32_t bucket = threadIdx.x;
+    BandSeg v{nullptr, nullptr, nullptr};
+#pragma unroll
+    for (int j = 0; j < BANDS; ++j) if (bucket >= d.edge[j] && bucket < d.edge[j + 1]) v = BandSeg{d.recs[j], d.aux[j], d.base[j]};
+    seg[bucket] = v;
+}
+__global__ __launch_bounds__(256) void k_lv_band_bases(const unsigned long long* __restrict__ scan, BandDst d, uint32_t rps, uint64_t reg_lo, uint64_t reg_hi) {
+    for (uint64_t r = reg_lo + (uint64_t)blockIdx.x * blockDim.x + threadIdx.x; r < reg_hi; r += (uint64_t)gridDim.x * blockDim.x) {
+        const uint32_t bucket = (uint32_t)(r / rps);
+        int band = 0;
+#pragma unroll
+        for (int j = 1; j < BANDS; ++j) if (bucket >= d.edge[j]) band = j;
+        uint64_t first = 0, end = 0;
+        unsigned long long* base = nullptr;
+#pragma unroll
+        for (int j = 0; j < BANDS; ++j) if (band == j) { first = (uint64_t)d.edge[j] * rps; end = (uint64_t)d.edge[j + 1] * rps; base = d.base[j]; }
+        const unsigned long long s0 = scan[first];
+        base[r] = scan[r] - s0;
+        if (r + 1 == end) base[end] = scan[end] - s0;
+    }
+}
 
 constexpr uint32_t SCAN_CHUNK = 16384;
 __global__ __launch_bounds__(1024) void k_scan_sums(const unsigned long long* __restrict__ a, uint64_t n, unsigned long long* __restrict__ sums) {
diff --git a/kreeq_amd/csrc/kq_partition.h b/kreeq_amd/csrc/kq_partition.h
--- a/kreeq_amd/csrc/kq_partition.h
+++ b/kreeq_amd/csrc/kq_partition.h
@@ -1,5 +1,6 @@
 #pragma once
 #include "kq_device.h"
+#include "kq_band_arena.h"
 
 namespace kq {
 
@@ -32,6 +33,12 @@
 constexpr int P3_MAX_SETS = 64;
 struct P3Set { const uint64_t* recs; const uint8_t* aux; const unsigned long long* base; uint64_t n_max; };
 
+struct BandDst {
+    uint32_t* recs[BANDS]; uint8_t* aux[BANDS]; unsigned long long* base[BANDS];
+    uint32_t edge[BANDS + 1];
+};
+struct BandSeg { uint32_t* out; uint8_t* aux; const unsigned long long* base; };
+
 struct LevelCfg {
     uint64_t n_regions;
     uint32_t n_seg, nb, seg_shift, out_shift;
diff --git a/kreeq_amd/csrc/kreeq_amd.hip b/kreeq_amd/csrc/kreeq_amd.hip
--- a/kreeq_amd/csrc/kreeq_amd.hip
+++ b/kreeq_amd/csrc/kreeq_amd.hip
@@ -175,6 +175,14 @@
     bool hist_cache_off = false;
     bool test_fail_plan = false;
     void* hot = nullptr; size_t hot_bytes = 0;
+    bool band_on = true;
+    bool arena_at_ceiling = false;
+    bool pend_banded = false;
+    BandArena bands;
+    P3Set* d_band_sets = nullptr;
+    int band_n[BANDS] = {};
+    uint32_t band_done = 0;
+    uint64_t band_passes = 0, region_visits = 0;
 
     TableView view() const {
         TableView v; v.slots = slots - (reg_lo() << REGION_SHIFT); v.n_regions = n_regions; v.hc = hc; v.hc_mask = hc_cap - 1; v.st = st; v.k = (uint32_t)k;
@@ -187,6 +195,10 @@
     uint64_t reg_hi() const { return windowed ? (uint64_t)win_hi * (n_regions >> 8) : n_regions; }
     uint64_t n_alloc_regions() const { return reg_hi() - reg_lo(); }
     uint64_t n_slots() const { return n_alloc_regions() << REGION_SHIFT; }
+    void band_edges(uint32_t (&edge)[BANDS + 1]) const {
+        const uint32_t lo = windowed ? win_lo : 0u, n = (windowed ? win_hi : 256u) - lo;
+        for (int j = 0; j <= BANDS; ++j) edge[j] = lo + (uint32_t)((uint64_t)n * (uint32_t)j / BANDS);
+    }
 };
 
 static void marks_reset(kq_handle* h);
@@ -221,7 +233,8 @@
 static void arena_release(kq_handle* h) {
     if (!h->arena) return;
     if (h->arena_scr.p) scr_free(h->arena_scr); else (void)hipFree(h->arena);
-    h->arena = nullptr; h->arena_bytes = 0;
+    h->arena = nullptr; h->arena_bytes = 0; h->arena_at_ceiling = false;
+    h->bands.init(0);
 }
 static int ensure_buf(void** p, size_t* have, size_t need) {
     if (*have >= need) return KQ_OK;
@@ -239,7 +252,18 @@
 static void clear_main(kq_handle* h, Slot* p, uint64_t n_slots) { (void)hipMemsetAsync(p, 0, (size_t)n_slots * sizeof(Slot), h->stream); }
 static void materialize(kq_handle* h) {
     if (!h->slots_dirty) return;
-    clear_main(h, h->slots, h->n_slots());
+    if (!h->band_done) clear_main(h, h->slots, h->n_slots());
+    else {
+        uint32_t edge[BANDS + 1];
+        h->band_edges(edge);
+        const uint64_t rps = h->n_regions >> NARROW_CBITS;
+        for (int j = 0; j < BANDS; ++j) {
+            const uint64_t first = edge[j] * rps, n = (edge[j + 1] - edge[j]) * rps;
+            if (n && !(h->band_done >> j & 1u)) clear_main(h, h->slots + ((first - h->reg_lo()) << REGION_SHIFT), n << REGION_SHIFT);
+        }
+        h->table_empty = false;
+        h->band_done = 0;
+    }
     h->slots_dirty = false;
 }
 static int alloc_main(kq_handle* h, uint64_t n_regions, uint64_t alloc_regions, Slot** out, uint32_t** rstart_out) {
@@ -517,6 +541,7 @@
     if (h->copy_stream) (void)hipStreamDestroy(h->copy_stream);
     arena_release(h);
     if (h->d_sets) (void)hipFree(h->d_sets);
+    if (h->d_band_sets) (void)hipFree(h->d_band_sets);
     if (h->hot) (void)hipFree(h->hot);
     marks_reset(h);
     if (h->own_stream) (void)hipStreamDestroy(h->own_stream);
@@ -534,6 +559,8 @@
     h->hc_check_at = 0;
     h->table_empty = true;
     h->n_pend = 0; h->arena_used = 0; h->pend_records = 0;
+    h->bands.clear(); h->pend_banded = false; h->band_done = 0;
+    for (int j = 0; j < BANDS; ++j) h->band_n[j] = 0;
     h->fx_bad = 0;
     return KQ_OK;
 }
@@ -588,6 +615,11 @@
             if (h->arena && value != h->pend_budget) { HIPC(hipStreamSynchronize(h->stream)); arena_release(h); }
             h->pend_budget = value; return KQ_OK;
         }
+        case KQ_OPT_BAND_PASSES: {
+            int rc = flush_pending(h);
+            if (rc) return rc;
+            h->band_on = value != 0; return KQ_OK;
+        }
         case KQ_OPT_BUCKET_WINDOW:
             HIPC(hipSetDevice(h->device));
             return set_window(h, (uint32_t)(value & 0xFFFF), (uint32_t)((value >> 16) & 0xFFFF));
@@ -639,6 +671,8 @@
     out->hc_total = h->hc_cap;
     out->table_bytes = h->n_slots() * sizeof(Slot) + h->hc_cap * sizeof(HcSlot);
     out->table_passes = h->table_passes;
+    out->band_passes = h->band_passes;
+    out->region_visits = h->region_visits;
     return KQ_OK;
 }
 
@@ -652,6 +686,7 @@
     uint64_t *recs1, *recs2;
     uint8_t *aux1, *aux2;
     unsigned long long *m1, *seg_off, *unit_base, *group_base, *sums, *total, *hot;
+    BandSeg* bseg;
     uint32_t* m2;
 };
 static void plan_cfg(const kq_handle* h, PartCfg* cfg, bool allow_narrow = false) {
@@ -697,7 +732,7 @@
     const uint64_t rec_words = p->fmt == FMT_NARROW ? n_max / 2 + 2 : n_max;
     const bool split2 = (rec_words + aux_words) * 8 >= ((size_t)512 << 20);
     if (split2) { int rc2 = scr_ensure(h->part2, (size_t)(rec_words + aux_words) * 8, h->device); if (rc2) return rc2; }
-    const size_t words = (size_t)((split2 ? 1 : 2) * (rec_words + aux_words) + p->m1_n + 2 * (seg_max + 2) + p->groups_n + p->sums_n + 4 + (p->R + 2) + (p->m2_n + 1) / 2);
+    const size_t words = (size_t)((split2 ? 1 : 2) * (rec_words + aux_words) + p->m1_n + 2 * (seg_max + 2) + p->groups_n + p->sums_n + 4 + (p->R + 2) + (sizeof(BandSeg) << NARROW_CBITS) / 8 + (p->m2_n + 1) / 2);
     int rc = ensure_buf(&h->part, &h->part_bytes, words * 8);
     if (rc) return rc;
     p->recs1 = (uint64_t*)h->part;
@@ -712,7 +747,8 @@
     p->sums = p->group_base + p->groups_n;
     p->total = p->sums + p->sums_n;
     p->hot = p->total + 4;
-    p->m2 = (uint32_t*)(p->hot + p->R + 2);
+    p->bseg = (BandSeg*)(p->hot + p->R + 2);
+    p->m2 = (uint32_t*)(p->bseg + (1u << NARROW_CBITS));
     return KQ_OK;
 }
 static void scan_u64(kq_handle* h, unsigned long long* a, uint64_t n, unsigned long long* sums_scratch, unsigned long long* total) {
@@ -819,8 +855,9 @@
 }
 static void run_level(kq_handle* h, PartPlan* p, const LevelCfg& lv, const uint64_t* in, const uint8_t* in_aux, uint64_t* out, uint8_t* out_aux,
                       unsigned long long* gb = nullptr ,
-                      const unsigned long long* seg_hi = nullptr ) {
-    if (!gb) gb = p->group_base;
+                      const unsigned long long* seg_hi = nullptr ,
+                      const BandDst* bd = nullptr ) {
+    if (!gb || bd) gb = p->group_base;
     if (!seg_hi) seg_hi = p->seg_off + 1;
     LevelCfg lvr = lv;
     lvr.rep_shift = 0;
@@ -840,14 +877,20 @@
         hipLaunchKernelGGL(k_lv_offsets, dim3((unsigned)((groups * 64 + 255) / 256)), dim3(256), 0, h->stream, p->m2, lv_, p->unit_base, gb);
     (void)hipMemsetAsync(gb + groups, 0, 8, h->stream);
     scan_u64(h, gb, groups + 1, p->sums, p->total + 1);
+    const BandSeg* bseg = nullptr;
+    if (bd) {
+        hipLaunchKernelGGL(k_band_segs, dim3(1), dim3(1u << NARROW_CBITS), 0, h->stream, *bd, p->bseg);
+        hipLaunchKernelGGL(k_lv_band_bases, dim3(grid_for(h, h->n_alloc_regions(), 256)), dim3(256), 0, h->stream, gb, *bd, (uint32_t)(lv.n_regions >> NARROW_CBITS), h->reg_lo(), h->reg_hi());
+        bseg = p->bseg;
+    }
     mark(h, "k_lv_hist+offsets+scan");
     const bool small = lv.nb < 512;
 #define KQ_LVS(W, N) hipLaunchKernelGGL((k_lv_scatter<W, N>), dim3(unit_grid), dim3(LV_THREADS), 0, h->stream, in, in_aux, lv_, \
-                                        p->seg_off, seg_hi, p->unit_base, p->m2, gb, out, out_aux)
+                                        p->seg_off, seg_hi, p->unit_base, p->m2, gb, out, out_aux, bseg)
     if (lv.top8)              { KQ_LVS(FMT_PACK8_TO_NARROW, 512); }
     else if (fmt == FMT_TOP8) { if (small) KQ_LVS(FMT_TOP8, 512); else KQ_LVS(FMT_TOP8, NB_MAX); }
 #define KQ_LVN(T) hipLaunchKernelGGL((k_lv_scatter_s<T>), dim3(unit_grid), dim3(LV_THREADS), 0, h->stream, (const uint32_t*)in, in_aux, lv_, \
-                                      p->seg_off, seg_hi, p->unit_base, p->m2, gb, (uint32_t*)out, out_aux)
+                                      p->seg_off, seg_hi, p->unit_base, p->m2, gb, (uint32_t*)out, out_aux, bseg)
     else if (fmt == FMT_NARROW && small && lv.rstart && !(h->kernel_set & 4)) { KQ_LVN(true); }
     else if (fmt == FMT_NARROW && small && !lv.rstart && (h->kernel_set & 2)) { KQ_LVN(false); }
 #undef KQ_LVN
@@ -878,7 +921,7 @@
     lv.spb = 1;
     return lv;
 }
-static void run_narrow_levels(kq_handle* h, PartPlan* p, const uint64_t** sorted, const uint8_t** sorted_aux, const P3Set* dst = nullptr, bool tight = false);
+static void run_narrow_levels(kq_handle* h, PartPlan* p, const uint64_t** sorted, const uint8_t** sorted_aux, const P3Set* dst = nullptr, bool tight = false, const BandDst* bd = nullptr);
 static bool tight_ok(const kq_handle* h, const PartPlan& p) { return p.fmt == FMT_NARROW && p.R >= TIGHT_MIN_REGIONS && h->rstart != nullptr; }
 static LevelCfg level_flat_to_coarse(const PartCfg& cfg) {
     LevelCfg lv; lv.n_regions = cfg.n_regions; lv.n_seg = 1; lv.nb = cfg.n_coarse; lv.seg_shift = 32; lv.out_shift = cfg.g_shift; lv.in_raw = 0; lv.k = 0; lv.narrow = 0; lv.top8 = 0;
@@ -894,16 +937,18 @@
     const bool aux = fmt == FMT_NARROW || fmt == FMT_WIDE;
     return ((((size_t)n_max * rec + 63) & ~(size_t)63) + (aux ? (((size_t)n_max + 63) & ~(size_t)63) : 0) + (size_t)(R + 2) * 8 + 255) & ~(size_t)255;
 }
-static int arena_take(kq_handle* h, uint64_t n_max, int fmt, uint64_t R, P3Set* out, bool* ok) {
-    *ok = false;
-    if (h->pend_budget == 0) return KQ_OK;
-    const size_t need = set_bytes(n_max, fmt, R);
-    bool was_full = false;
-    if (h->n_pend && (h->n_pend >= P3_MAX_SETS || h->pend_fmt != fmt || h->arena_used + need > h->arena_bytes)) {
-        was_full = h->pend_fmt == fmt && h->n_pend < P3_MAX_SETS;
-        int rc = flush_pending(h);
-        if (rc) return rc;
-    }
+struct BandedSet { bool on = false; BandDst dst; uint64_t cnt[BANDS]; };
+struct BandSets { P3Set set[BANDS]; int idx[BANDS]; };
+__global__ void k_p3sets_banded(P3Set* tabs, BandSets v) {
+    const int j = threadIdx.x;
+    if (j < BANDS && v.idx[j] >= 0) tabs[j * P3_MAX_SETS + v.idx[j]] = v.set[j];
+}
+static bool band_mode(const kq_handle* h, int fmt) {
+    return h->band_on && (fmt == FMT_TIGHT || fmt == FMT_NARROW) && (h->pend_budget > 0 || (h->pend_budget < 0 && h->arena_at_ceiling));
+}
+static int band_passes_run(kq_handle* h, const int* order, int n);
+
+static int arena_ensure(kq_handle* h, size_t need, bool was_full) {
     size_t want = h->arena_bytes;
     if (need > want) want = h->pend_budget > 0 ? (size_t)h->pend_budget : std::max<size_t>(4 * need, (size_t)64 << 20);
     else if (was_full && h->pend_budget < 0) want = 2 * h->arena_bytes;
@@ -914,7 +959,7 @@
         const size_t avail = free_b + h->arena_bytes, reserve = std::max<size_t>(total_b / 8, (size_t)8 << 30);
         const size_t ceiling = avail > 2 * reserve ? avail - reserve : avail / 2;
         if (h->pend_budget < 0) budget = std::min<size_t>(want, std::min<size_t>(ceiling, std::max<size_t>(4 * need, 4 * (size_t)h->n_slots() * sizeof(Slot))));
-        if (budget <= h->arena_bytes && need <= h->arena_bytes) budget = 0;
+        if (budget <= h->arena_bytes && need <= h->arena_bytes) { budget = 0; if (h->pend_budget < 0) h->arena_at_ceiling = true; }
         if (budget && budget < need) return KQ_OK;
         if (budget) {
             if (h->arena) { HIPC(hipStreamSynchronize(h->stream)); HIPC(hipStreamSynchronize(h->base)); arena_release(h); }
@@ -923,8 +968,73 @@
             else
             if (hipMalloc(&h->arena, budget) != hipSuccess) { (void)hipGetLastError(); h->arena = nullptr; return KQ_OK; }
             h->arena_bytes = budget; h->arena_used = 0;
+            h->bands.init(budget);
         }
     }
+    return KQ_OK;
+}
+static int arena_take_banded(kq_handle* h, int fmt, const unsigned long long* bucket_off, BandedSet* bs, bool* ok) {
+    *ok = false;
+    if (h->n_pend && (h->n_pend >= P3_MAX_SETS || h->pend_fmt != fmt || !h->pend_banded)) { int rc = flush_pending(h); if (rc) return rc; }
+    if (h->arena_used) return KQ_OK;
+    const bool aux = fmt == FMT_NARROW;
+    const uint64_t rps = h->n_regions >> NARROW_CBITS;
+    h->band_edges(bs->dst.edge);
+    size_t len[BANDS], recs_b[BANDS], aux_b[BANDS], total = 0;
+    for (int j = 0; j < BANDS; ++j) {
+        const uint32_t e0 = bs->dst.edge[j], e1 = bs->dst.edge[j + 1];
+        bs->cnt[j] = bucket_off[e1] - bucket_off[e0];
+        const size_t slack = bs->cnt[j] + 16;
+        recs_b[j] = (slack * 4 + 63) & ~(size_t)63;
+        aux_b[j] = aux ? (slack + 63) & ~(size_t)63 : 0;
+        len[j] = e1 > e0 ? BandArena::align_up(recs_b[j] + aux_b[j] + (size_t)((e1 - e0) * rps + 1) * 8) : 0;
+        total += len[j];
+    }
+    if (total > h->arena_bytes) {
+        if (h->n_pend) { int rc = flush_pending(h); if (rc) return rc; }
+        int rc = arena_ensure(h, total, false); if (rc) return rc;
+        if (total > h->arena_bytes || !h->arena) return KQ_OK;
+    }
+    size_t off[BANDS] = {};
+    int order[BANDS];
+    int n = h->bands.bands_to_fit(len, order);
+    if (n > 0 && !h->n_pend) return KQ_OK;
+    if (n > 0 && n < BANDS / 2) {
+        int rc = band_passes_run(h, order, n); if (rc) return rc;
+        n = h->bands.bands_to_fit(len, order);
+    }
+    if (n > 0) { int rc = flush_pending(h); if (rc) return rc; }
+    if (!h->bands.place(len, off)) return KQ_OK;
+    for (int j = 0; j < BANDS; ++j) {
+        bs->dst.recs[j] = nullptr; bs->dst.aux[j] = nullptr; bs->dst.base[j] = nullptr;
+        if (!len[j]) continue;
+        uint8_t* b = (uint8_t*)h->arena + off[j];
+        bs->dst.recs[j] = (uint32_t*)b;
+        if (aux) bs->dst.aux[j] = b + recs_b[j];
+        bs->dst.base[j] = (unsigned long long*)(b + recs_b[j] + aux_b[j]) - (uint64_t)bs->dst.edge[j] * rps;
+    }
+    bs->on = true;
+    *ok = true;
+    return KQ_OK;
+}
+static int arena_take(kq_handle* h, uint64_t n_max, int fmt, uint64_t R, P3Set* out, bool* ok, const unsigned long long* bucket_off = nullptr, BandedSet* bs = nullptr) {
+    *ok = false;
+    if (h->pend_budget == 0) return KQ_OK;
+    if (bucket_off && bs && band_mode(h, fmt)) {
+        int rc = arena_take_banded(h, fmt, bucket_off, bs, ok);
+        if (rc || *ok) { *out = P3Set{nullptr, nullptr, nullptr, n_max}; return rc; }
+    }
+    const size_t need = set_bytes(n_max, fmt, R);
+    bool was_full = false;
+    if (h->n_pend && (h->n_pend >= P3_MAX_SETS || h->pend_fmt != fmt || h->pend_banded || h->arena_used + need > h->arena_bytes)) {
+        was_full = h->pend_fmt == fmt && h->n_pend < P3_MAX_SETS && !h->pend_banded;
+        int rc = flush_pending(h);
+        if (rc) return rc;
+    }
+    if (!h->bands.empty()) return KQ_OK;
+    int rc = arena_ensure(h, need, was_full);
+    if (rc) return rc;
+    if (!h->arena || h->arena_used + need > h->arena_bytes) return KQ_OK;
     uint8_t* base = (uint8_t*)h->arena + h->arena_used;
     const size_t rec = (fmt == FMT_NARROW || fmt == FMT_TIGHT) ? 4 : 8;
     const bool aux = fmt == FMT_NARROW || fmt == FMT_WIDE;
@@ -938,25 +1048,35 @@
     *ok = true;
     return KQ_OK;
 }
-static int pend_add(kq_handle* h, const P3Set& set, int fmt, int aux_fmt) {
-    if (h->n_pend && (h->n_pend >= P3_MAX_SETS || h->pend_fmt != fmt || h->pend_aux_fmt != aux_fmt)) {
+static int pend_add(kq_handle* h, const P3Set& set, int fmt, int aux_fmt, const BandedSet* bs = nullptr) {
+    const bool banded = bs && bs->on;
+    if (h->n_pend && (h->n_pend >= P3_MAX_SETS || h->pend_fmt != fmt || h->pend_aux_fmt != aux_fmt || h->pend_banded != banded)) {
         int rc = flush_pending(h);
         if (rc) return rc;
     }
-    if (!h->d_sets) HIPC(hipMalloc((void**)&h->d_sets, sizeof(P3Set) * P3_MAX_SETS));
-    hipLaunchKernelGGL(k_p3set, dim3(1), dim3(1), 0, h->stream, h->d_sets, h->n_pend, set);
-    h->pend_fmt = fmt; h->pend_aux_fmt = aux_fmt;
+    if (banded) {
+        if (!h->d_band_sets) HIPC(hipMalloc((void**)&h->d_band_sets, sizeof(P3Set) * P3_MAX_SETS * BANDS));
+        BandSets v;
+        for (int j = 0; j < BANDS; ++j) {
+            v.idx[j] = bs->dst.recs[j] ? h->band_n[j]++ : -1;
+            v.set[j] = P3Set{(const uint64_t*)bs->dst.recs[j], bs->dst.aux[j], bs->dst.base[j], bs->cnt[j]};
+        }
+        hipLaunchKernelGGL(k_p3sets_banded, dim3(1), dim3(64), 0, h->stream, h->d_band_sets, v);
+    } else {
+        if (!h->d_sets) HIPC(hipMalloc((void**)&h->d_sets, sizeof(P3Set) * P3_MAX_SETS));
+        hipLaunchKernelGGL(k_p3set, dim3(1), dim3(1), 0, h->stream, h->d_sets, h->n_pend, set);
+    }
+    h->pend_fmt = fmt; h->pend_aux_fmt = aux_fmt; h->pend_banded = banded;
     ++h->n_pend;
     h->pend_records += set.n_max;
     return KQ_OK;
 }
 static int flush_pending_base(kq_handle* h);
-static int flush_pending(kq_handle* h) {
-    if (!h->n_pend) return KQ_OK;
+static int on_base_between_forks(kq_handle* h, int (*pass)(kq_handle*, const int*, int), const int* order, int n) {
     hipStream_t work = h->stream;
     h->stream = h->base;
     int rc = join_forks(h);
-    if (!rc) rc = flush_pending_base(h);
+    if (!rc) rc = pass(h, order, n);
     if (!rc && h->fork_stream[0]) {
         hipEvent_t e; rc = ev_get(h, &e);
         if (!rc && hipEventRecord(e, h->base) != hipSuccess) rc = fail(KQ_ERR_HIP, "hipEventRecord failed");
@@ -965,27 +1085,35 @@
     h->stream = work;
     return rc;
 }
-static int flush_pending_base(kq_handle* h) {
-    const uint64_t R = h->n_regions;
-    int rc = ensure_buf(&h->hot, &h->hot_bytes, (size_t)(R + 2) * 8);
+static int flush_pending(kq_handle* h) {
+    if (!h->n_pend) return KQ_OK;
+    return on_base_between_forks(h, [](kq_handle* hh, const int*, int) { return flush_pending_base(hh); }, nullptr, 0);
+}
+static int pass_prepare(kq_handle* h) {
+    int rc = ensure_buf(&h->hot, &h->hot_bytes, (size_t)(h->n_regions + 2) * 8);
     if (rc) return rc;
     if (h->kmers_bound / 255 + 1 > (1ull << 23)) {
         rc = read_state_raw(h); if (rc) return rc;
         const uint64_t need_hc = std::max<uint64_t>(HC_CAP_BIG, 8 * h->st_host->hc_used);
         if (need_hc > h->hc_cap) { rc = grow_hc(h, need_hc); if (rc) return rc; }
     }
+    return KQ_OK;
+}
+static int pass_launch(kq_handle* h, uint64_t reg_lo, uint64_t reg_hi, const P3Set* sets, uint32_t n_sets, int empty) {
+    const uint64_t R = h->n_regions;
     unsigned long long* hot = (unsigned long long*)h->hot;
     HIPC(hipMemsetAsync(hot, 0, 8, h->stream));
-    const dim3 grid((unsigned)std::min<uint64_t>(h->n_alloc_regions(), 1u << 30)), grid_hot(h->n_cu), block(P3_THREADS);
-    const int empty = h->slots_dirty ? 2 : h->table_empty ? 1 : 0;
+    TableView view = h->view();
+    view.reg_lo = reg_lo; view.reg_hi = reg_hi;
+    const dim3 grid((unsigned)std::min<uint64_t>(reg_hi - reg_lo, 1u << 30)), grid_hot(h->n_cu), block(P3_THREADS);
     const int fmt = h->pend_fmt;
     const uint32_t rps = (fmt == FMT_NARROW || fmt == FMT_TIGHT || fmt == FMT_TOP8) ? (uint32_t)(R >> NARROW_CBITS) : 1u;
-#define KQ_HOT(F) hipLaunchKernelGGL((k_count_regions<F, true>), grid_hot, block, 0, h->stream, h->view(), h->d_sets, (uint32_t)h->n_pend, h->pend_aux_fmt, empty, hot, rps)
+#define KQ_HOT(F) hipLaunchKernelGGL((k_count_regions<F, true>), grid_hot, block, 0, h->stream, view, sets, n_sets, h->pend_aux_fmt, empty, hot, rps)
 #define KQ_P3(F) do { \
-        hipLaunchKernelGGL((k_count_regions<F, false>), grid, block, 0, h->stream, h->view(), h->d_sets, (uint32_t)h->n_pend, h->pend_aux_fmt, empty, hot, rps); \
+        hipLaunchKernelGGL((k_count_regions<F, false>), grid, block, 0, h->stream, view, sets, n_sets, h->pend_aux_fmt, empty, hot, rps); \
         KQ_HOT(F); } while (0)
 #define KQ_Q4(KC, T) do { \
-        hipLaunchKernelGGL((k_count_regions_q4<KC, T>), grid, dim3(Q4_THREADS), 0, h->stream, h->view(), h->d_sets, (uint32_t)h->n_pend, empty, hot, rps); \
+        hipLaunchKernelGGL((k_count_regions_q4<KC, T>), grid, dim3(Q4_THREADS), 0, h->stream, view, sets, n_sets, empty, hot, rps); \
         KQ_HOT(FMT_NARROW); } while (0)
     if (fmt == FMT_TIGHT)       { if (h->k == 21) KQ_Q4(21, true); else KQ_Q4(0, true); }
     else if (fmt == FMT_NARROW) { if (h->k == 21) KQ_Q4(21, false); else KQ_Q4(0, false); }
@@ -995,12 +1123,61 @@
 #undef KQ_Q4
 #undef KQ_P3
 #undef KQ_HOT
+    HIPC(hipGetLastError());
+    h->region_visits += reg_hi - reg_lo;
+    return KQ_OK;
+}
+static int band_empty_flag(const kq_handle* h, int j) {
+    if (h->band_done >> j & 1u) return 0;
+    return h->slots_dirty ? 2 : h->table_empty ? 1 : 0;
+}
+static int band_pass(kq_handle* h, int j, const uint32_t (&edge)[BANDS + 1]) {
+    const uint64_t rps = h->n_regions >> NARROW_CBITS;
+    const int empty = band_empty_flag(h, j);
+    if (edge[j + 1] > edge[j] && (h->band_n[j] || empty == 2)) {
+        int rc = pass_launch(h, edge[j] * rps, edge[j + 1] * rps, h->d_band_sets + (size_t)j * P3_MAX_SETS, (uint32_t)h->band_n[j], empty);
+        if (rc) return rc;
+    }
+    if (h->table_empty || h->slots_dirty) h->band_done |= 1u << j;
+    h->band_n[j] = 0;
+    h->bands.apply_band(j);
+    uint32_t all = 0;
+    for (int q = 0; q < BANDS; ++q) if (edge[q + 1] > edge[q]) all |= 1u << q;
+    if ((h->band_done & all) == all) { h->slots_dirty = false; h->table_empty = false; h->band_done = 0; }
+    return KQ_OK;
+}
+static int band_passes_base(kq_handle* h, const int* order, int n) {
+    int rc = pass_prepare(h);
+    if (rc) return rc;
+    uint32_t edge[BANDS + 1];
+    h->band_edges(edge);
+    for (int i = 0; i < n; ++i) {
+        rc = band_pass(h, order[i], edge); if (rc) return rc;
+        ++h->band_passes;
+    }
+    mark(h, "k_count_regions");
+    return KQ_OK;
+}
+static int band_passes_run(kq_handle* h, const int* order, int n) { return on_base_between_forks(h, band_passes_base, order, n); }
+static int flush_pending_base(kq_handle* h) {
+    int rc = pass_prepare(h);
+    if (rc) return rc;
+    if (h->pend_banded) {
+        uint32_t edge[BANDS + 1];
+        h->band_edges(edge);
+        for (int j = 0; j < BANDS; ++j) { rc = band_pass(h, j, edge); if (rc) return rc; }
+    } else {
+        rc = pass_launch(h, h->reg_lo(), h->reg_hi(), h->d_sets, (uint32_t)h->n_pend, h->slots_dirty ? 2 : h->table_empty ? 1 : 0);
+        if (rc) return rc;
+    }
     h->n_pend = 0; h->arena_used = 0; h->pend_records = 0;
+    h->pend_banded = false; h->bands.clear();
+    for (int j = 0; j < BANDS; ++j) h->band_n[j] = 0;
     ++h->table_passes;
     h->slots_dirty = false;
     h->table_empty = false;
+    h->band_done = 0;
     mark(h, "k_count_regions");
-    HIPC(hipGetLastError());
     return KQ_OK;
 }
 
@@ -1010,7 +1187,7 @@
     PartCfg c; plan_cfg(h, &c, true);
     return c.narrow != 0;
 }
-static void run_narrow_levels(kq_handle* h, PartPlan* p, const uint64_t** sorted, const uint8_t** sorted_aux, const P3Set* dst, bool tight) {
+static void run_narrow_levels(kq_handle* h, PartPlan* p, const uint64_t** sorted, const uint8_t** sorted_aux, const P3Set* dst, bool tight, const BandDst* bd) {
     const uint32_t sb = p->cfg.sub_bits;
     const bool t8 = p->fmt == FMT_TOP8;
     uint8_t* a1 = t8 ? nullptr : p->aux1;
@@ -1021,17 +1198,17 @@
     LevelCfg last = level_narrow(p->cfg, sb, false, t8);
     if (tight) last.rstart = h->rstart;
     if (sb == 0) {
-        run_level(h, p, last, p->recs1, a1, fin, fin_aux, fin_base);
+        run_level(h, p, last, p->recs1, a1, fin, fin_aux, fin_base, nullptr, bd);
     } else {
         run_level(h, p, level_narrow(p->cfg, sb, true, t8), p->recs1, a1, p->recs2, a2);
         (void)hipMemcpyAsync(p->seg_off, p->group_base, (size_t)(((1u << NARROW_CBITS) << sb) + 1) * 8, hipMemcpyDeviceToDevice, h->stream);
-        run_level(h, p, last, p->recs2, a2, fin, fin_aux, fin_base);
+        run_level(h, p, last, p->recs2, a2, fin, fin_aux, fin_base, nullptr, bd);
     }
     *sorted = fin; *sorted_aux = fin_aux;
 }
 
-static int pend_or_apply(kq_handle* h, const P3Set& set, int fmt, int aux_fmt, bool in_arena) {
-    int rc = pend_add(h, set, fmt, aux_fmt);
+static int pend_or_apply(kq_handle* h, const P3Set& set, int fmt, int aux_fmt, bool in_arena, const BandedSet* bs = nullptr) {
+    int rc = pend_add(h, set, fmt, aux_fmt, bs);
     if (rc) return rc;
     return in_arena ? KQ_OK : flush_pending(h);
 }
@@ -1052,19 +1229,25 @@
     const bool tight = tight_ok(h, p);
     const int set_fmt = tight ? FMT_TIGHT : p.fmt;
     const bool filtered = p.cfg.filt_lo != 0 || p.cfg.filt_hi != p.cfg.map_count || h->windowed;
-    if (leveled && !filtered) { rc = arena_take(h, p.n_max, set_fmt, p.R, &set, &in_arena); if (rc) return rc; }
+    const bool band_try = p.fmt == FMT_NARROW && band_mode(h, set_fmt);
+    BandedSet bset;
+    if (leveled && !filtered && !band_try) { rc = arena_take(h, p.n_max, set_fmt, p.R, &set, &in_arena); if (rc) return rc; }
     marks_reset(h);
     mark(h, "start");
     run_p1(h, &p, p.cfg, ab, lead, len, er, p.recs1, a1, AUX_IDX6, pinv);
-    if (leveled && filtered) {
-        unsigned long long n_recs = 0;
-        HIPC(hipMemcpyAsync(&n_recs, p.total, sizeof n_recs, hipMemcpyDeviceToHost, h->stream));
+    if (leveled && (filtered || band_try)) {
+        unsigned long long n_recs = 0, bucket_off[(1u << NARROW_CBITS) + 1];
+        if (band_try) HIPC(hipMemcpyAsync(bucket_off, p.seg_off, sizeof bucket_off, hipMemcpyDeviceToHost, h->stream));
+        else HIPC(hipMemcpyAsync(&n_recs, p.total, sizeof n_recs, hipMemcpyDeviceToHost, h->stream));
         HIPC(hipStreamSynchronize(h->stream));
-        rc = arena_take(h, std::min<uint64_t>(p.n_max, ((uint64_t)n_recs + 15) & ~7ull), set_fmt, p.R, &set, &in_arena); if (rc) return rc;
+        if (band_try) n_recs = bucket_off[1u << NARROW_CBITS];
+        rc = arena_take(h, filtered ? std::min<uint64_t>(p.n_max, ((uint64_t)n_recs + 15) & ~7ull) : p.n_max, set_fmt, p.R, &set, &in_arena,
+                        band_try ? bucket_off : nullptr, &bset);
+        if (rc) return rc;
     }
     if (p.fmt == FMT_NARROW || p.fmt == FMT_TOP8) {
         const uint64_t* sorted; const uint8_t* sorted_aux;
-        run_narrow_levels(h, &p, &sorted, &sorted_aux, in_arena ? &set : nullptr, tight);
+        run_narrow_levels(h, &p, &sorted, &sorted_aux, in_arena && !bset.on ? &set : nullptr, tight, bset.on ? &bset.dst : nullptr);
         if (!in_arena) set = P3Set{sorted, sorted_aux, p.group_base, p.n_max};
     } else if (p.two_level) {
         if (in_arena) run_level(h, &p, level_coarse_to_regions(p.cfg), p.recs1, a1, const_cast<uint64_t*>(set.recs), const_cast<uint8_t*>(set.aux), const_cast<unsigned long long*>(set.base));
@@ -1073,7 +1256,7 @@
         set = P3Set{p.recs1, a1, p.seg_off, p.n_max};
     }
     HIPC(hipGetLastError());
-    return pend_or_apply(h, set, set_fmt, tight ? AUX_TIGHT : AUX_IDX6, in_arena);
+    return pend_or_apply(h, set, set_fmt, tight ? AUX_TIGHT : AUX_IDX6, in_arena, &bset);
 }
 static int count_partitioned_records(kq_handle* h, const uint64_t* d_recs, const uint8_t* d_aux, int aux_fmt, uint64_t n, bool raw) {
     PartPlan p;
```

After: 50.76 billion. 1.0% lower.
